# levymsn/CQA-CRCT

Hardware: AMD Instinct MI355X
Metric: QA-pairs/sec training step (whole node) (higher is better)
Workload: dtype bf16; 1 GPU; CRCT fwd+loss+bwd+AdamW, vilbert.json (v_feature_size=2048), batch 80/GPU, 36 visual elems x 2048-d, 20 text tokens, dropout 0.1, L1 regression loss; residual_stream=fp32, global_batch=80, parallelism=dp1, input=resident

## Files before the change

cqa-crct_amd/crct/lib.py:

```python
import ctypes as C
import os

_HERE = os.path.dirname(os.path.abspath(__file__))
LIB_PATH = os.path.join(_HERE, "libcrct_hip.so")

c_i32, c_i64, c_u32, c_u64, c_f32 = C.c_int32, C.c_int64, C.c_uint32, C.c_uint64, C.c_float
ATTN_MAX_LEN = 512
FP8_AMAX_LANES = 64
vp = C.c_void_p


class GemmArgs(C.Structure):
    _fields_ = [("A", vp), ("B", vp), ("C", vp), ("bias", vp), ("preact_out", vp), ("dact_src", vp), ("addend", vp),
                ("lda", c_i64), ("ldb", c_i64), ("ldc", c_i64), ("ld_aux", c_i64), ("ld_add", c_i64),
                ("M", c_i32), ("N", c_i32), ("K", c_i32), ("ta", c_i32), ("tb", c_i32), ("act", c_i32), ("dact", c_i32),
                ("c_is_f32", c_i32), ("accumulate", c_i32), ("tile", c_i32), ("alpha", c_f32), ("drop_thr", c_u32),
                ("drop_scale", c_f32), ("drop_site", c_u32), ("seed", c_u64), ("rowsum_out", vp),
                ("fp8", c_i32), ("scale_a", vp), ("scale_b", vp), ("q_out", vp), ("q_scale", vp), ("q_amax", vp), ("ld_q", c_i64),
                ("site", c_i32), ("split_k", c_i32), ("splitk_ws", vp), ("splitk_cnt", vp), ("addend_f32", c_i32), ("c_cached", c_i32)]


class GemmLnAddend(C.Structure):
    _fields_ = [("mean", vp), ("rstd", vp), ("gamma", vp), ("beta", vp)]

# ... 6 lines not shown
SITE_NAMES = ["none", "t.qkv", "t.out", "t.ffn_up", "t.ffn_down", "v.qkv", "v.out", "v.ffn_up", "v.ffn_down",
              "c.qkv_t", "c.qkv_v", "c.out_t", "c.out_v", "img_emb", "head"]
KIND_NAMES = ["fwd", "dgrad", "wgrad"]
CLASS_NAMES = ["S.w", "S.n", "S.nl", "M.w", "M.n", "M.nl", "L.w", "L.n", "L.nl"]


class HeadArgs(C.Structure):
    _fields_ = [("pooled_t", vp), ("pooled_v", vp), ("fus_h", vp), ("w_cls", vp), ("b_cls", vp), ("w_f6", vp), ("b_f6", vp),
                ("R", vp), ("labels", vp), ("logits", vp), ("reg", vp), ("stats", vp), ("scratch", vp),
                ("d_pooled_t", vp), ("d_pooled_v", vp), ("d_fus_h", vp),
                ("d_w_cls", vp), ("d_b_cls", vp), ("d_w_f6", vp), ("d_b_f6", vp), ("g_nsp_dev", vp), ("g_reg_dev", vp),
                ("g_loss_dev", vp), ("B", c_i32), ("Hb", c_i32), ("fusion_sum", c_i32), ("use_l1", c_i32), ("kind_l1", c_i32),
                ("tol_margin", c_f32), ("nsp_coeff", c_f32), ("reg_coeff", c_f32), ("grad_scale", c_f32),
                ("drop_thr", c_u32), ("drop_scale", c_f32), ("drop_site", c_u32), ("seed", c_u64)]


CE_CLASSES = 65
DATASET_KINDS = {"plotqa": 0, "dvqa": 1, "figure_qa": 2}
REGRESSOR_KINDS = {"plotqa": 0, "none": 1, "ce": 2}


class Variant(C.Structure):
    _fields_ = [("dataset", c_i32), ("regressor", c_i32), ("n_values", c_i32), ("values", c_f32 * CE_CLASSES)]


class HeadVariantArgs(C.Structure):
    _fields_ = [("h", HeadArgs), ("variant", Variant), ("snap", c_i32), ("ce_scratch", vp)]


EVAL_TOTAL, EVAL_BREAKDOWN, EVAL_HISTOGRAM, EVAL_ERRORS, EVAL_TABLE_WORDS = 0, 12, 192, 205, 206


class EvalScoreArgs(C.Structure):
    _fields_ = [("logits", vp), ("reg_out", vp), ("reg_err", vp), ("reg_terr", vp), ("num_ans", vp), ("forced", vp), ("labels", vp),
                ("gt_id", vp), ("needs_reg", vp), ("tolerance", vp), ("cats", vp), ("answers", vp), ("sel_out", vp), ("sel_err", vp),
                ("sel_terr", vp), ("flags", vp), ("prob0", vp), ("tables", vp), ("N", c_i64), ("Q", c_i32), ("mode", c_i32),
                ("with_histogram", c_i32)]


class ModelDims(C.Structure):
    _fields_ = [("vocab", c_i32), ("n_pos", c_i32), ("n_types", c_i32), ("H", c_i32), ("L", c_i32), ("heads", c_i32), ("I", c_i32),
                ("Fv", c_i32), ("Hv", c_i32), ("Lv", c_i32), ("v_heads", c_i32), ("Iv", c_i32), ("Hb", c_i32), ("b_heads", c_i32),
                ("n_color", c_i32), ("n_conn", c_i32), ("v_biatt", c_i32 * 32), ("t_biatt", c_i32 * 32),
                ("fusion_sum", c_i32), ("with_coattention", c_i32),
                ("p_hidden", c_f32), ("p_attn", c_f32), ("p_v_hidden", c_f32), ("p_v_attn", c_f32), ("p_cls", c_f32)]


class Batch(C.Structure):
    _fields_ = [("tokens", vp), ("segments", vp), ("loc", vp), ("text_keymask", vp), ("image_feat", vp), ("image_loc", vp),
                ("image_target", vp), ("image_keymask", vp), ("R", vp), ("labels", vp),
                ("B", c_i32), ("T", c_i32), ("V", c_i32),
                ("sep_indices", vp), ("hist_len", vp), ("image_mask", vp), ("sep_stride", c_i32), ("image_feat_bf16", c_i32)]


class LnFwdArgs(C.Structure):
    _fields_ = [("x", vp), ("gamma", vp), ("beta", vp), ("y", vp), ("mean", vp), ("rstd", vp), ("M", c_i32), ("H", c_i32),
                ("eps", c_f32), ("drop_thr", c_u32), ("drop_scale", c_f32), ("drop_site", c_u32), ("seed", c_u64),
                ("q_out", vp), ("q_scale", vp), ("q_amax", vp), ("x_f32", c_i32), ("y_f32", vp)]


class LnBwdArgs(C.Structure):
    _fields_ = [("dy", vp), ("x", vp), ("mean", vp), ("rstd", vp), ("gamma", vp), ("dx", vp), ("dx_lin", vp), ("partials", vp),
                ("M", c_i32), ("H", c_i32), ("post_thr", c_u32), ("post_scale", c_f32), ("post_site", c_u32),
                ("lin_thr", c_u32), ("lin_scale", c_f32), ("lin_site", c_u32), ("seed", c_u64),
                ("q_out", vp), ("q_scale", vp), ("q_amax", vp), ("x_f32", c_i32)]


class AmpState(C.Structure):
    _fields_ = [("grad_scale", vp), ("found_inf", vp), ("step", vp)]


class AttnQuant(C.Structure):
    _fields_ = [("ctx_q", vp), ("ctx_scale", vp), ("ctx_amax", vp), ("dq_q", vp), ("dk_q", vp), ("dv_q", vp),
                ("dq_scale", vp), ("dq_amax", vp), ("dkv_scale", vp), ("dkv_amax", vp),
                ("row_lse", vp), ("ctx", vp), ("ld_ctx", c_i64)]


class Fp8Shadow(C.Structure):
    _fields_ = [("q", vp), ("seg_slot", vp), ("scale", vp), ("amax", vp), ("qt", vp), ("seg_in", vp), ("seg_t_base", vp), ("seg_t_ld", vp)]


class StepCfg(C.Structure):
    _fields_ = [("training", c_i32), ("use_l1", c_i32), ("kind_l1", c_i32), ("tol_margin", c_f32), ("nsp_coeff", c_f32),
                ("reg_coeff", c_f32), ("grad_scale", c_f32), ("seed", c_u64), ("g_nsp_dev", vp), ("g_reg_dev", vp), ("g_loss_dev", vp),
                ("seg_ready_events", vp), ("seg_done_events", vp),
                ("fp8", c_i32), ("params_fp8", vp), ("fp8_w_scale", vp), ("fp8_act_scale", vp), ("fp8_act_amax", vp),
                ("fp8_bwd", c_i32), ("fp8_wgrad", c_i32), ("params_fp8_t", vp), ("fp8_grad_scale", vp), ("fp8_grad_amax", vp),
                ("seg_enqueued", vp), ("seg_enqueued_user", vp), ("seg_done_mask", vp), ("wgrad_overwrite", c_i32), ("grads_bf16", vp),
                ("residual_fp32", c_i32)]


class InputGrads(C.Structure):
    _fields_ = [("d_image_feat", vp), ("d_image_loc", vp), ("d_areas", vp), ("d_txt_loc", vp), ("d_text_emb", vp)]


class OutputGrads(C.Structure):
    _fields_ = [("d_seq_t", vp), ("d_seq_v", vp)]


class ScoreGrads(C.Structure):
    _fields_ = [("d_logits", vp), ("d_value", vp)]


SEG_ENQUEUED_FN =C.CFUNCTYPE(None, C.c_int, vp)


_u8 = [c_u32, c_f32, c_u32, c_u64]
PROTOTYPES = {
    "crct_last_error": (C.c_char_p, []),
    "crct_abi_version": (C.c_int, []),
    "crct_gemm_bf16": (C.c_int, [C.POINTER(GemmArgs), vp]),
    "crct_gemm_bf16_grouped": (C.c_int, [C.POINTER(GemmArgs), C.c_int, vp]),
    "crct_gemm_bf16_ln_addend": (C.c_int, [C.POINTER(GemmArgs), C.POINTER(GemmLnAddend), vp]),
    "crct_gemm_bf16_grouped_ln_addend": (C.c_int, [C.POINTER(GemmArgs), C.POINTER(GemmLnAddend), C.c_int, vp]),
    "crct_gemm_pick_tile": (C.c_int, [C.c_int, C.c_int]),
    "crct_gemm_group_max_workgroups": (C.c_int, [C.c_int]),
    "crct_gemm_group_target_workgroups": (C.c_int, [C.c_int]),
    "crct_gemm_group_concat": (C.c_int, [C.c_int]),
    "crct_embed_scatter_split": (None, [C.c_int]),
    "crct_gemm_force_generic": (C.c_int, [C.c_int]),
    "crct_prof_enable": (C.c_int, [C.c_int]),
    "crct_prof_reset": (C.c_int, []),
    "crct_prof_read": (C.c_int, [C.c_int, C.POINTER(C.c_long), C.POINTER(C.c_double), C.POINTER(C.c_double)]),
    "crct_prof_read_site": (C.c_int, [C.c_int, C.c_int, C.POINTER(C.c_long), C.POINTER(C.c_double), C.POINTER(C.c_double), C.POINTER(C.c_int)]),
    "crct_prof_stamp_count": (C.c_int, []),
    "crct_prof_stamp_read": (C.c_int, [C.c_int, C.POINTER(vp), C.POINTER(C.c_double), C.POINTER(C.c_double)]),
    "crct_engine_streams": (C.c_int, [vp, C.POINTER(vp)]),
    "crct_launch_log_enable": (C.c_int, [C.c_int]),
    "crct_launch_log_count": (C.c_int, []),
    "crct_launch_log_read": (C.c_int, [C.c_int, C.POINTER(LaunchRec)]),
    "crct_gemm_splitk_ws_elems": (c_i64, [C.c_int, C.c_int, C.c_int]),
    "crct_gemm_splitk_tickets": (C.c_int, [C.c_int, C.c_int]),
    "crct_engine_set_site_policy": (C.c_int, [vp, C.c_int, C.c_int, C.c_int, C.c_int, C.c_int]),
    "crct_layernorm_fwd": (C.c_int, [vp, vp, vp, vp, vp, vp, C.c_int, C.c_int, c_f32] + _u8 + [vp]),
    "crct_layernorm_bwd_blocks": (C.c_int, [C.c_int]),
    "crct_layernorm_bwd": (C.c_int, [vp] * 11 + [C.c_int, C.c_int, C.c_int, c_u32, c_f32, c_u32, c_u32, c_f32, c_u32, c_u64, vp]),
    "crct_layernorm_bwd_rows": (C.c_int, [vp] * 8 + [C.c_int, C.c_int, c_u32, c_f32, c_u32, c_u32, c_f32, c_u32, c_u64, vp]),
    "crct_layernorm_bwd_finalize": (C.c_int, [vp] * 4 + [C.c_int, C.c_int, C.c_int, vp]),
    "crct_colsum_blocks": (C.c_int, [C.c_int]),
    "crct_colsum_bf16": (C.c_int, [vp, c_i64, vp, vp, C.c_int, C.c_int, C.c_int, vp]),
    "crct_build_keymasks": (C.c_int, [vp, vp, C.c_int, vp, vp, vp, C.c_int, C.c_int, C.c_int, vp]),
    "crct_softmax_rows_f32_bf16": (C.c_int, [vp, vp, C.c_int, C.c_int, vp]),
    "crct_softmax_rows_bf16_bf16": (C.c_int, [vp, vp, C.c_int, C.c_int, vp]),
    "crct_layernorm_fwd_q": (C.c_int, [vp, vp, vp, vp, vp, vp, C.c_int, C.c_int, c_f32] + _u8 + [vp, vp, vp, vp]),
    "crct_layernorm_bwd_rows_args": (C.c_int, [C.POINTER(LnBwdArgs), vp]),
    "crct_layernorm_fwd_args": (C.c_int, [C.POINTER(LnFwdArgs), vp]),
    "crct_fp8_transpose_weights": (C.c_int, [vp] * 6 + [C.c_int, c_i64, C.c_int, vp]),
    "crct_fp8_quantize_bf16": (C.c_int, [vp, vp, vp, vp, c_i64, vp]),
    "crct_fp8_update_scales": (C.c_int, [vp, vp, C.c_int, C.c_int, vp, c_f32, vp]),
    "crct_fp8_quantize_weights": (C.c_int, [vp] * 7 + [c_i64, vp, vp, C.c_int, vp]),
    "crct_gemm_group_wgrad_config": (C.c_int, [C.c_int]),
    "crct_engine_set_wgrad_flush": (C.c_int, [vp, C.c_int]),
    "crct_engine_set_ln_addend": (C.c_int, [vp, C.c_int]),
    "crct_engine_set_wgrad_workgroups": (C.c_int, [vp, C.c_int, C.c_int]),
    "crct_gemm_class_config": (C.c_int, [C.c_int, C.c_int]),
    "crct_gemm_fp8_scaled_mfma": (C.c_int, [C.c_int]),
    "crct_ghost_collective": (C.c_int, [vp, c_i64, C.c_int, C.c_int, C.c_double, vp]),
    "crct_cast_f32_bf16": (C.c_int, [vp, vp, c_i64, vp]),
    "crct_cast_bf16_f32": (C.c_int, [vp, vp, c_i64, vp]),
    "crct_cast_runs_f32_bf16": (C.c_int, [vp, vp, vp, vp, vp, vp, c_i64, vp]),
    "crct_cast_runs_bf16_f32": (C.c_int, [vp, vp, vp, vp, vp, vp, c_i64, vp]),
    "crct_attention_fwd": (C.c_int, [vp] * 5 + [C.c_int] * 5 + [c_i64] * 4 + _u8 + [vp]),
    "crct_attention_probs": (C.c_int, [vp] * 4 + [C.c_int] * 5 + [c_i64] * 2 + _u8 + [vp]),
    "crct_attention_bwd": (C.c_int, [vp] * 8 + [C.c_int] * 5 + [c_i64] * 7 + _u8 + [vp]),
    "crct_attention_fwd_q": (C.c_int, [vp] * 5 + [C.c_int] * 5 + [c_i64] * 4 + _u8 + [vp, vp]),
    "crct_attention_bwd_q": (C.c_int, [vp] * 8 + [C.c_int] * 5 + [c_i64] * 7 + _u8 + [vp, vp]),
    "crct_attention_quant_ok": (C.c_int, [C.c_int] * 3),
    "crct_attention_force_valu": (None, [C.c_int]),
    "crct_attention_force_long": (None, [C.c_int]),
    "crct_attention_force_split": (None, [C.c_int]),
    "crct_embed_text_fwd": (C.c_int, [vp] * 14 + [C.c_int] * 4 + [c_f32] + _u8 + [vp]),
    "crct_embed_text_bwd_indexed": (C.c_int, [vp] * 16 + [C.c_int] * 4 + _u8 + [vp, vp, C.c_int, vp, C.c_int, vp]),
    "crct_embed_image_fwd": (C.c_int, [vp] * 12 + [C.c_int] * 2 + [c_f32] + _u8 + [vp]),
    "crct_embed_image_bwd": (C.c_int, [vp] * 15 + [C.c_int] * 2 + _u8 + [vp, vp, C.c_int, vp]),
    "crct_embed_image_var_fwd": (C.c_int, [vp] * 14 + [C.c_int] * 2 + [c_f32] + _u8 + [vp]),
    "crct_embed_image_var_bwd": (C.c_int, [vp] * 16 + [C.c_int] * 2 + _u8 + [vp, vp, C.c_int, vp]),
    "crct_head_loss": (C.c_int, [C.POINTER(HeadArgs), vp]),
    "crct_head_loss_variant": (C.c_int, [C.POINTER(HeadVariantArgs), vp]),
    "crct_head_loss_scores": (C.c_int, [C.POINTER(HeadArgs), C.POINTER(ScoreGrads), vp]),
    "crct_head_loss_variant_scores": (C.c_int, [C.POINTER(HeadVariantArgs), C.POINTER(ScoreGrads), vp]),
    "crct_eval_select": (C.c_int, [vp, vp, vp, vp, vp, vp, C.c_int, c_i64, vp, vp, vp, vp, vp, vp]),
    "crct_eval_score": (C.c_int, [C.POINTER(EvalScoreArgs), vp]),
    "crct_adamw_plan": (c_i64, [vp, C.c_int, vp, vp, c_i64]),
    "crct_adamw_step": (C.c_int, [vp] * 11 + [c_i64, c_f32, c_f32, c_f32, C.c_int, vp, vp, vp, C.c_int, C.c_int, vp, vp]),
    "crct_adamw_advance": (C.c_int, [vp, vp, vp]),
    "crct_grad_sumsq": (C.c_int, [vp] * 6 + [c_i64, vp, C.c_int, C.c_int, vp]),
    "crct_grad_norm_finalize": (C.c_int, [vp, vp, c_i64, C.c_int, C.c_int, c_f32, vp, vp, vp, vp, vp]),
    "crct_scale_runs": (C.c_int, [vp] * 6 + [c_i64, C.c_int, vp]),
    "crct_engine_create": (vp, [C.POINTER(ModelDims), C.c_char_p, vp, vp, C.c_int, C.c_int, C.c_int, C.c_int]),
    "crct_engine_create_variant": (vp, [C.POINTER(ModelDims), C.c_char_p, vp, vp, C.c_int, C.c_int, C.c_int, C.c_int, C.POINTER(Variant)]),
    "crct_engine_set_areas": (C.c_int, [vp, vp]),
    "crct_engine_set_input_grads": (C.c_int, [vp, C.POINTER(InputGrads)]),
    "crct_embed_input_grad": (C.c_int, [vp] * 11 + [C.c_int] * 2 + _u8 + [vp]),
    "crct_softmax_bwd_rows": (C.c_int, [vp, C.c_int, vp, vp, C.c_int, C.c_int, vp]),
    "crct_layernorm_rows_f32": (C.c_int, [vp, C.c_int, vp, vp, vp, vp, vp, C.c_int, C.c_int, vp]),
    "crct_hidden_grad_add": (C.c_int, [vp, vp, c_f32, c_i64, vp]),
    "crct_engine_sequence_outputs": (C.c_int, [vp, vp, vp, C.c_int, C.c_int, C.c_int, vp, vp, vp]),
    "crct_engine_set_output_grads": (C.c_int, [vp, C.POINTER(OutputGrads)]),
    "crct_engine_set_score_grads": (C.c_int, [vp, C.POINTER(ScoreGrads)]),
    "crct_engine_set_trainable": (C.c_int, [vp, vp, C.c_int]),
    "crct_engine_backward_plan": (C.c_int, [vp, vp, C.c_int]),
    "crct_engine_destroy": (None, [vp]),
    "crct_engine_workspace_bytes": (C.c_size_t, [vp]),
    "crct_engine_num_segments": (C.c_int, [vp]),
    "crct_engine_segment_range": (C.c_int, [vp, C.c_int, C.POINTER(c_i64), C.POINTER(c_i64)]),
    "crct_engine_forward": (C.c_int, [vp, vp, vp, C.POINTER(Batch), C.POINTER(StepCfg), vp, vp, vp, vp, vp]),
    "crct_engine_backward": (C.c_int, [vp, vp, vp, C.POINTER(Batch), C.POINTER(StepCfg), vp, vp, vp, vp, vp, C.c_int, vp]),
    "crct_engine_set_streams": (C.c_int, [vp, C.c_int, C.c_int]),
    "crct_engine_aux_stream": (vp, [vp, vp, C.POINTER(C.c_int)]),
    "crct_event_create": (vp, []),
    "crct_event_destroy": (None, [vp]),
    "crct_event_record": (C.c_int, [vp, vp]),
    "crct_stream_wait_event": (C.c_int, [vp, vp]),
    "crct_event_synchronize": (C.c_int, [vp]),
    "crct_event_query": (C.c_int, [vp]),
    "crct_engine_wgrad_owned": (C.c_int, [vp, vp, vp, C.c_int]),
    "crct_engine_fp8_sites": (C.c_int, [vp]),
    "crct_engine_fp8_grad_sites": (C.c_int, [vp]),
    "crct_engine_fp8_weights": (C.c_int, [vp, vp, vp, C.c_int]),
    "crct_zero_runs": (C.c_int, [vp, vp, vp, vp, vp, c_i64, vp]),
    "crct_engine_attention_probs": (c_i64, [vp, vp, vp, vp, C.c_int, C.c_int, C.c_int, vp, c_i64, vp]),
    "crct_engine_tap": (c_i64, [vp, vp, C.c_char_p, C.c_int, C.c_int, C.c_int, vp, c_i64, vp]),
}

_lib = None


def load():
    global _lib
    if _lib is not None:
        return _lib
    if not os.path.exists(LIB_PATH):
        raise RuntimeError("libcrct_hip.so is missing (%s): run `python -c 'import __graft_entry__ as g; g.build()'` "
                           "-- there is no CPU fallback for the CRCT step" % LIB_PATH)
    import torch
    lib = C.CDLL(LIB_PATH)
    for name, (res, args) in PROTOTYPES.items():
        fn = getattr(lib, name)
        fn.restype = res
        fn.argtypes = args
    _lib = lib
    return lib


def check(rc, what=""):
    if rc != 0:
        raise RuntimeError("libcrct_hip %s failed (%d): %s" % (what, rc, load().crct_last_error().decode()))


def drop_threshold(p):
    t = float(p) * 4294967296.0
    if t <= 0.0:
        return 0
    return min(int(t), 4294967295)


def ptr(t):
    return None if t is None else t.data_ptr()


def current_stream():
    import torch
    return torch.cuda.current_stream().cuda_stream
```

cqa-crct_amd/csrc/crct_internal.h:

```cpp
#pragma once
#include <hip/hip_runtime.h>
#include <hip/hip_ext.h>
#include "../../include/crct_hip.h"

void crct_set_error(const char* fmt, ...);
#define CRCT_CHECK_HIP(expr)                                                          \
  do {                                                                                \
    hipError_t _e = (expr);                                                           \
    if (_e != hipSuccess) {                                                           \
      crct_set_error("%s:%d: %s -> %s", __FILE__, __LINE__, #expr, hipGetErrorString(_e)); \
      return 1;                                                                       \
    }                                                                                 \
  } while (0)
#define CRCT_REQUIRE(cond, ...)                 \
  do {                                          \
    if (!(cond)) {                              \
      crct_set_error(__VA_ARGS__);              \
      return 2;                                 \
    }                                           \
  } while (0)

bool crct_gemm_config_built(int id);
int crct_gemm_fp8_wgrad_step_config(int asked);
hipError_t crct_gemm_launch(const CrctGemmArgs& g, const CrctGemmLnAddend* ln, hipStream_t s);
struct CrctGemmGroup {
  const CrctGemmArgs* gs;
  const CrctGemmLnAddend* ln;
  int n;
  const uint8_t* keep;
  int target_wgs;
};
hipError_t crct_gemm_launch_grouped(const CrctGemmGroup& grp, hipStream_t s);
int crct_streams_place(hipStream_t main, hipStream_t out[4], int* n_classes);

#define CRCT_LN_BWD_MAX_BLOCKS 256

bool crct_stamp_begin(hipStream_t s, hipEvent_t* start, hipEvent_t* stop);
void crct_stamp_adopt(hipStream_t s, hipEvent_t start, hipEvent_t stop);
void crct_stamp_enable(int on);
void crct_stamp_reset(void);
#ifdef CRCT_GEMM_LAB
bool crct_lab_skip(const void* kern, hipStream_t s);
#endif
hipError_t crct_lds_limit_raise(const void* kern, size_t bytes);
class CrctDeviceScope {
 public:
  CrctDeviceScope();
  ~CrctDeviceScope();
  CrctDeviceScope(const CrctDeviceScope&) = delete;
  CrctDeviceScope& operator=(const CrctDeviceScope&) = delete;
 private:
  int outer_;
};
template <class K>
inline hipError_t crct_lds_limit(K kern, size_t bytes) {
  return bytes <= 64 * 1024 ? hipSuccess : crct_lds_limit_raise(reinterpret_cast<const void*>(kern), bytes);
}
template <class K, class... A>
inline void crct_launch(K kern, dim3 grid, dim3 block, size_t lds, hipStream_t s, A... a) {
#ifdef CRCT_GEMM_LAB
  if (crct_lab_skip((const void*)kern, s)) return;
#endif
  hipEvent_t e0, e1;
  if (crct_stamp_begin(s, &e0, &e1)) hipExtLaunchKernelGGL(kern, grid, block, (uint32_t)lds, s, e0, e1, 0u, a...);
  else hipLaunchKernelGGL(kern, grid, block, lds, s, a...);
}
```

cqa-crct_amd/csrc/engine.cpp:

```cpp
#include <math.h>
#include <stdarg.h>
#include <stdio.h>
#include <stdlib.h>
#include <string.h>

#include <algorithm>
#include <string>
#include <unordered_map>
#include <unordered_set>
#include <functional>
#include <vector>

#include "crct_internal.h"

typedef unsigned short bf16_t;
enum { ACT_NONE = 0, ACT_GELU = 1, ACT_RELU = 2, ACT_LEAKY = 3, ACT_TANH = 4 };

static thread_local char g_err[1024] = "";
void crct_set_error(const char* fmt, ...) {
  va_list ap;
  va_start(ap, fmt);
  vsnprintf(g_err, sizeof(g_err), fmt, ap);
  va_end(ap);
}
// ... 12 lines not shown
  CRCT_REQUIRE(!a.ta || a.M % 8 == 0, "%s: transposed A needs M %% 8 == 0 (M=%d)%s", who, a.M, of);
  CRCT_REQUIRE(!a.tb || a.N % 8 == 0, "%s: transposed B needs N %% 8 == 0 (N=%d)%s", who, a.N, of);
  CRCT_REQUIRE(a.tile < 0 || crct_gemm_config_built(a.tile), "%s: configuration %d is not built%s", who, a.tile, of);
  CRCT_REQUIRE(!(a.c_cached && a.accumulate), "%s: c_cached with accumulate is not supported (c_cached is a plain fp32 store)%s", who, of);
  CRCT_REQUIRE(!ln || (a.addend && a.addend_f32 && ln->mean && ln->rstd && ln->gamma && ln->beta),
               "%s: a LayerNorm addend needs the fp32 addend it normalises (addend, addend_f32) and mean, rstd, gamma, beta%s", who, of);
  return 0;
}

extern "C" int crct_gemm_bf16_ln_addend(const CrctGemmArgs* a, const CrctGemmLnAddend* ln, crct_stream_t stream) {
  CRCT_REQUIRE(a != nullptr, "gemm: null args");
  if (int r = gemm_check(*a, ln, "gemm", -1)) return r;
  CRCT_CHECK_HIP(crct_gemm_launch(*a, ln, (hipStream_t)stream));
  return 0;
}
extern "C" int crct_gemm_bf16(const CrctGemmArgs* a, crct_stream_t stream) { return crct_gemm_bf16_ln_addend(a, nullptr, stream); }

static int gemm_grouped_checked(const CrctGemmGroup& grp, crct_stream_t stream) {
  CRCT_REQUIRE(grp.gs != nullptr && grp.n >= 1, "gemm_grouped: bad arguments");
  for (int i = 0; i < grp.n; ++i)
    if (int r = gemm_check(grp.gs[i], grp.ln && grp.ln[i].mean ? &grp.ln[i] : nullptr, "gemm_grouped", i)) return r;
  CRCT_CHECK_HIP(crct_gemm_launch_grouped(grp, (hipStream_t)stream));
  return 0;
}
extern "C" int crct_gemm_bf16_grouped_ln_addend(const CrctGemmArgs* a, const CrctGemmLnAddend* ln, int n, crct_stream_t stream) {
  return gemm_grouped_checked(CrctGemmGroup{a, ln, n, nullptr, -1}, stream);
}
extern "C" int crct_gemm_bf16_grouped(const CrctGemmArgs* a, int n, crct_stream_t stream) { return crct_gemm_bf16_grouped_ln_addend(a, nullptr, n, stream); }

namespace {

inline size_t align_up(size_t v, size_t a) { return (v + a - 1) / a * a; }
inline uint32_t thr_of(float p) {
  double t = (double)p * 4294967296.0;
  if (t <= 0.0) return 0u;
  if (t >= 4294967295.0) return 4294967295u;
  return (uint32_t)t;
}

struct Arena {
  size_t top = 0;
  size_t take(size_t bytes) { size_t o = top; top = align_up(top + bytes, 256); return o; }
};

struct Drop { uint32_t thr = 0; float scale = 1.f; uint32_t site = 0; };

struct LinearP { int64_t w = -1, b = -1; int in = 0, out = 0; int site = 0; int parts = 1; };
struct LnP { int64_t g = -1, b = -1; };
struct FfnP { LinearP up, down; LnP ln; };
struct ProjP { LinearP dense; LnP ln; };
struct SelfLayerP { LinearP qkv; ProjP proj; FfnP ffn; int H, heads; float p_attn, p_hid; uint32_t site; };
struct ConnLayerP { LinearP qkv1, qkv2; ProjP proj_v, proj_t; FfnP ffn_v, ffn_t; uint32_t site; };

constexpr size_t NONE = (size_t)-1;
struct Act { size_t x = 0, q = NONE; int site = -1; size_t x32 = NONE; size_t s = NONE, mean = NONE, rstd = NONE; LnP ln; };
struct GradQ { size_t q = NONE; int site = -1; };
struct FfnA {
  size_t u, h, s, y, y32, mean, rstd, hq, yq; int site_h, site_y; int g_dl, g_du;
  Act out(const LnP& ln) const { return {y, yq, site_y, y32, s, mean, rstd, ln}; }
};
struct ProjA {
  size_t s, a, a32, mean, rstd, aq; int site_a; int g_dl;
  Act out(const LnP& ln) const { return {a, aq, site_a, a32, s, mean, rstd, ln}; }
};
struct SelfLayerA { size_t qkv, ctx, ctxq, lse; int site_ctx, g_dqkv; ProjA proj; FfnA ffn; };
struct ConnLayerA { size_t qkv1, qkv2, ctx1, ctx2, ctx1q, ctx2q, lse1, lse2; int site_ctx1, site_ctx2, g_dqkv1, g_dqkv2; ProjA proj_v, proj_t; FfnA ffn_v, ffn_t; };
struct StreamScratch { size_t dy[2], dres_a, dlin_a, dres_b, dlin_b, gc, du, dctx, dqkv, part_a, part_b, dlq_a, dlq_b, duq, dqkvq; };

struct Step { char kind; int idx; };
struct StepIn { Act t, v; };
struct Tap { std::string name; size_t off; char stream; int width = 0; };
struct SegPlan { bool runs = true, dx_t = true, dx_v = true; int dropped = 0; };

}

struct crct_engine {
  CrctModelDims d;
  std::unordered_map<std::string, int64_t> off, size;
  int maxB, maxT, maxV;
  std::vector<Step> sched;
  std::vector<SelfLayerP> tl, vl;
  std::vector<ConnLayerP> cl;
  std::vector<SelfLayerA> tla, vla;
  std::vector<ConnLayerA> cla;
  struct { int64_t word, pos, type, wloc, bloc; LnP ln; } et;
  struct { LinearP img; int64_t color, wloc, bloc; LnP ln; LinearP areas; } ev;
  CrctVariant var = {CRCT_DATASET_PLOTQA, CRCT_REGRESSOR_PLOTQA, 0, {}};
  bool feat = true;
  const float* areas = nullptr;
  CrctInputGrads ig = {nullptr, nullptr, nullptr, nullptr, nullptr};
  size_t ws_ig = 0;
  bool emb_own_t = true, emb_own_v = true;
  CrctOutputGrads og = {nullptr, nullptr};
  int fwd_r32 = -1;
  CrctScoreGrads sg = {nullptr, nullptr};
  bool ig_text() const { return ig.d_txt_loc || ig.d_text_emb; }
  bool ig_vis() const { return ig.d_image_feat || ig.d_image_loc || ig.d_areas; }
  size_t ws_base() const { return ln_addend ? ws_core : ws_two_output; }
  void ws_update() { ws_bytes = ws_base() + (ig.d_image_feat ? ws_ig : 0); }
  struct { size_t sum, y, mean, rstd, yq; int site; } eta;
  struct { size_t soft, lin, sum, y, mean, rstd, yq; int site; } eva;
  LinearP t_pool, v_pool, cls, tp[4], vp[4], fu[4];
  struct { size_t pooled_t, pooled_v, t[3], v[3], cat, f[3], scratch, ce, d_pt, d_pv, g[10]; } ha;
  StreamScratch st, sv;
  StreamScratch st2, sv2;
  size_t partials[2], colsum_part[4];
  size_t embed_rows[2], embed_idx[2];
  size_t km_t = 0, km_v = 0;
  struct SitePolicy { int cfg = -1, split_k = 0; };
  SitePolicy policy[CRCT_SITE_COUNT][3][2];
  size_t sk_ws[2] = {0, 0}, sk_cnt[2] = {0, 0};
  size_t sk_ws_elems[2] = {0, 0};
  int sk_tickets = 0;
  std::unordered_map<int64_t, int> wq_slot;
  int32_t* word_index = nullptr;
  std::vector<std::pair<int64_t, int64_t>> wq_list;
  int n_sites = 0;
  int n_gsites = 0;
  size_t ws_bytes = 0;
  bool use_vis_stream = true, use_wgrad_stream = true, streams_forced = false;
  int wgrad_target = 96, wgrad_target_rows = 3000;
  int ln_addend = 1;
  size_t ws_core = 0, ws_two_output = 0;
  int wgrad_flush = 1;
  bool one_wgrad_stream = false;
  int first_conn = -1;
  hipStream_t side[3] = {nullptr, nullptr, nullptr};
  hipStream_t aux = nullptr;
  hipStream_t placed_for = nullptr;
  bool placed = false;
  int queue_classes = 0;
  std::vector<hipEvent_t> evpool;
  size_t evnext = 0;
  std::vector<std::pair<int64_t, int64_t>> seg_range;
  std::unordered_map<int64_t, int64_t> wgrad_owned;
  std::unordered_map<int64_t, int> wgrad_pass;
  void wgrad_pass_begin() { wgrad_pass.clear(); }
  std::vector<int64_t> param_off;
  std::unordered_set<int64_t> nograd;
  std::vector<SegPlan> plan;
  bool grad_at(int64_t o) const { return nograd.empty() || !nograd.count(o); }
  bool w_grad(const LinearP& l) const {
    for (int k = 0; k < l.parts; ++k) if (grad_at(l.w + k * ((int64_t)l.in * l.out / l.parts))) return true;
    return false;
  }
  bool b_grad(const LinearP& l) const {
    for (int k = 0; k < l.parts; ++k) if (grad_at(l.b + k * (l.out / l.parts))) return true;
    return false;
  }
  bool drops_wgrad(const LinearP& l, bool with_bias) const { return !nograd.empty() && !w_grad(l) && !(with_bias && b_grad(l)); }
  std::vector<Tap> taps;
  std::vector<StepIn> in;
  int cur_t = 0, cur_v = 0;
  bool bad = false;
  int64_t P(const std::string& k) {
    auto it = off.find(k);
    if (it == off.end()) { crct_set_error("engine: parameter '%s' missing from the layout", k.c_str()); bad = true; return 0; }
    return it->second;
  }
};

namespace {

LinearP linear_p(crct_engine* e, const std::string& name, int in, int out, int site = CRCT_SITE_HEAD) {
  LinearP l;
  l.w = e->P(name + ".weight"); l.b = e->P(name + ".bias"); l.in = in; l.out = out; l.site = site;
  return l;
}
LnP ln_p(crct_engine* e, const std::string& name) {
  LnP l; l.g = e->P(name + ".weight"); l.b = e->P(name + ".bias"); return l;
}
LinearP fused3(crct_engine* e, const std::string& a, const std::string& b, const std::string& c, int in, int out, int site) {
  LinearP l = linear_p(e, a, in, 3 * out, site);
  l.parts = 3;
  const int64_t wsz = (int64_t)in * out;
  if (e->P(b + ".weight") != l.w + wsz || e->P(c + ".weight") != l.w + 2 * wsz || e->P(b + ".bias") != l.b + out ||
      e->P(c + ".bias") != l.b + 2 * out) {
    crct_set_error("engine: %s / %s / %s must be adjacent in the flat layout (fused QKV)", a.c_str(), b.c_str(), c.c_str());
    e->bad = true;
  }
  return l;
}

static_assert(CRCT_SITE_T_OUT == CRCT_SITE_T_QKV + 1 && CRCT_SITE_T_FFN_UP == CRCT_SITE_T_QKV + 2 && CRCT_SITE_T_FFN_DN == CRCT_SITE_T_QKV + 3 &&
              CRCT_SITE_V_OUT == CRCT_SITE_V_QKV + 1 && CRCT_SITE_V_FFN_UP == CRCT_SITE_V_QKV + 2 && CRCT_SITE_V_FFN_DN == CRCT_SITE_V_QKV + 3,
              "the GEMM sites of a self-attention layer are consecutive");
SelfLayerP self_layer_p(crct_engine* e, const std::string& p, int H, int I, int heads, float p_attn, float p_hid, uint32_t drop_site, int gemm_site) {
  SelfLayerP l;
  l.H = H; l.heads = heads; l.p_attn = p_attn; l.p_hid = p_hid; l.site = drop_site;
  l.qkv = fused3(e, p + "attention.self.query", p + "attention.self.key", p + "attention.self.value", H, H, gemm_site);
  l.proj.dense = linear_p(e, p + "attention.output.dense", H, H, gemm_site + 1);
  l.proj.ln = ln_p(e, p + "attention.output.LayerNorm");
  l.ffn.up = linear_p(e, p + "intermediate.dense", H, I, gemm_site + 2);
  l.ffn.down = linear_p(e, p + "output.dense", I, H, gemm_site + 3);
  l.ffn.ln = ln_p(e, p + "output.LayerNorm");
  return l;
}
template <class F> void each_encoder_linear(const crct_engine* e, F f) {
  for (const std::vector<SelfLayerP>* stack : {&e->tl, &e->vl})
    for (const SelfLayerP& l : *stack) { f(l.qkv); f(l.ffn.up); f(l.ffn.down); f(l.proj.dense); }
  for (const ConnLayerP& l : e->cl) {
    f(l.qkv1); f(l.qkv2); f(l.ffn_v.up); f(l.ffn_v.down); f(l.ffn_t.up); f(l.ffn_t.down); f(l.proj_v.dense); f(l.proj_t.dense);
  }
}

FfnA ffn_a(Arena& ar, size_t M, int H, int I, int& sites, int& gsites) {
  FfnA a;
  a.g_dl = gsites++; a.g_du = gsites++;
  a.u = ar.take(M * I * 2); a.h = ar.take(M * I * 2); a.s = ar.take(M * H * 4); a.y = ar.take(M * H * 2); a.y32 = NONE;
  a.mean = ar.take(M * 4); a.rstd = ar.take(M * 4);
  a.hq = ar.take(M * I); a.yq = ar.take(M * H);
  a.site_h = sites++; a.site_y = sites++;
  return a;
}
ProjA proj_a(Arena& ar, size_t M, int H, int& sites, int& gsites) {
  ProjA a;
  a.g_dl = gsites++;
  a.s = ar.take(M * H * 4); a.a = ar.take(M * H * 2); a.a32 = NONE; a.mean = ar.take(M * 4); a.rstd = ar.take(M * 4);
  a.aq = ar.take(M * H);
  a.site_a = sites++;
  return a;
}
SelfLayerA self_layer_a(Arena& ar, size_t M, int H, int I, int heads, int& sites, int& gsites) {
  SelfLayerA a;
  a.qkv = ar.take(M * 3 * H * 2); a.ctx = ar.take(M * H * 2); a.ctxq = ar.take(M * H); a.lse = ar.take(M * heads * 4);
  a.site_ctx = sites++; a.g_dqkv = gsites++;
  a.proj = proj_a(ar, M, H, sites, gsites); a.ffn = ffn_a(ar, M, H, I, sites, gsites);
  return a;
}
StreamScratch scratch_a(Arena& ar, size_t M, int H, int I, int Hb) {
  StreamScratch s;
  const int Hm = H > Hb ? H : Hb;
  s.dy[0] = ar.take(M * H * 2); s.dy[1] = ar.take(M * H * 2);
  s.dres_a = ar.take(M * H * 2); s.dlin_a = ar.take(M * H * 2); s.dres_b = ar.take(M * H * 2); s.dlin_b = ar.take(M * H * 2);
  s.gc = ar.take(M * H * 2); s.du = ar.take(M * (size_t)I * 2); s.dctx = ar.take(M * (size_t)Hm * 2);
  s.dqkv = ar.take(M * (size_t)3 * Hm * 2);
  s.part_a = ar.take((size_t)3 * 4 * CRCT_LN_BWD_MAX_BLOCKS * H * 4);
  s.part_b = ar.take((size_t)3 * 4 * CRCT_LN_BWD_MAX_BLOCKS * H * 4);
  s.dlq_a = ar.take(M * H); s.dlq_b = ar.take(M * H); s.duq = ar.take(M * (size_t)I);
  s.dqkvq = ar.take(M * (size_t)3 * Hm);
  return s;
}

hipEvent_t ev_new(crct_engine* e) {
  if (e->evnext == e->evpool.size()) {
    hipEvent_t ev = nullptr;
    const unsigned flags = hipEventDisableTiming | hipEventDisableSystemFence;
    if (hipEventCreateWithFlags(&ev, flags) != hipSuccess) return nullptr;
    e->evpool.push_back(ev);
  }
  return e->evpool[e->evnext++];
}
int order_streams(crct_engine* e, hipStream_t from, hipStream_t to) {
  if (from == to) return 0;
  hipEvent_t ev = ev_new(e);
  if (!ev || hipEventRecord(ev, from) != hipSuccess || hipStreamWaitEvent(to, ev, 0) != hipSuccess) {
    crct_set_error("engine: event ordering between internal streams failed");
    return 1;
  }
  return 0;
}

struct WgQ8 { GradQ dy; Act x; };
struct Q8 { uint8_t* q = nullptr; const float* scale = nullptr; float* amax = nullptr; };

struct Run {
  crct_engine* e;
  const float* p32; const bf16_t* p16; float* g32; char* ws; hipStream_t s;
  const CrctBatch* b; const CrctStepCfg* c;
  hipStream_t sw;
  size_t partials, colsum_part, colsum_part_w;
  int which = 0;
  int phase = 1;
  int rc = 0;
  bool sw_dirty = false;
  const StreamScratch* sets[2] = {nullptr, nullptr};
  hipEvent_t set_free[2] = {nullptr, nullptr};
  int parity = 0;
  const StreamScratch& layer_begin() {
    if (!rc && sw != s && set_free[parity]) {
      if (hipStreamWaitEvent(s, set_free[parity], 0) != hipSuccess) { crct_set_error("engine: stream wait failed"); rc = 1; }
      set_free[parity] = nullptr;
    }
    return *sets[parity];
  }
  void layer_end() {
    flush_wgrads();
    if (!rc && sw != s && sw_dirty) {
      hipEvent_t ev = ev_new(e);
      if (!ev || hipEventRecord(ev, sw) != hipSuccess) { crct_set_error("engine: event record failed"); rc = 1; }
      set_free[parity] = ev;
    }
    parity ^= 1;
  }
  std::vector<CrctGemmArgs> pending;
  bool defer_wgrad = true;
  struct FinJob { const float* part; float* dg; float* db; float* dlb; int M, H; };
  std::vector<FinJob> pending_fin;
  int tick = 0, ordered_tick = -1;
  void wgrad_after_main() {
    if (rc || sw == s) return;
    sw_dirty = true;
    if (ordered_tick == tick) return;
    fail(order_streams(e, s, sw));
    ordered_tick = tick;
  }
  void main_after_wgrad() {
    flush_wgrads();
    if (!rc && sw != s && sw_dirty) { fail(order_streams(e, sw, s)); sw_dirty = false; }
  }

  template <class T> T* W(size_t o) const { return reinterpret_cast<T*>(ws + o); }
  bf16_t* A(size_t o) const { return W<bf16_t>(o); }
  float* F(size_t o) const { return W<float>(o); }
  const float* P(int64_t o) const { return p32 + o; }
  const bf16_t* PB(int64_t o) const { return p16 + o; }
  float* G(int64_t o) const { return g32 + o; }
  Drop drop(float p, uint32_t site) const {
    Drop d; d.site = site;
    if (c->training && p > 0.f) { d.thr = thr_of(p); d.scale = 1.0f / (1.0f - p); }
    return d;
  }
  void fail(int r) { if (!rc && r) rc = r; }

  struct Opt {
    void* preact = nullptr; const void* dact_src = nullptr; int dact = 0; int act = 0;
    const void* addend = nullptr; int64_t ld_aux = 0, ld_add = 0; Drop drop; bool f32 = false; bool acc = false;
    bool add_f32 = false, c_cached = false;
    CrctGemmLnAddend ln = {nullptr, nullptr, nullptr, nullptr};
  };
  void cross_sync(Run& V) {
    if (!rc) fail(order_streams(e, V.s, s));
    if (!V.rc) V.fail(order_streams(e, s, V.s));
  }
  int f8() const { return (c->fp8 && c->params_fp8 && c->fp8_w_scale && c->fp8_act_scale && c->fp8_act_amax) ? c->fp8 : 0; }
  bool f8_lin(const LinearP& l) const { return f8() && e->wq_slot.count(l.w) != 0; }
  int f8b() const { return (c->fp8 && c->fp8_bwd && c->params_fp8_t && c->fp8_w_scale && c->fp8_grad_scale && c->fp8_grad_amax) ? c->fp8_bwd : 0; }
  bool f8b_lin(const LinearP& l) const { return f8b() && e->wq_slot.count(l.w) != 0; }
  const float* ascale(int site) const { return c->fp8_act_scale + site; }
  float* aamax(int site) const { return c->fp8_act_amax + (int64_t)site * CRCT_FP8_AMAX_LANES; }
  const float* gscale(int g) const { return c->fp8_grad_scale + g; }
  float* gamax(int g) const { return c->fp8_grad_amax + (int64_t)g * CRCT_FP8_AMAX_LANES; }
  Q8 q8(const Act& a) const { return a.site < 0 ? Q8() : Q8{W<uint8_t>(a.q), ascale(a.site), aamax(a.site)}; }
  Q8 q8(const GradQ& g) const { return g.site < 0 ? Q8() : Q8{W<uint8_t>(g.q), gscale(g.site), gamax(g.site)}; }

  enum Dir { FWD = CRCT_KIND_FWD, DGRAD = CRCT_KIND_DGRAD, WGRAD = CRCT_KIND_WGRAD };
  CrctGemmArgs gemm_args(Dir dir, const LinearP& l, int M, const void* a, int64_t lda, const void* x, int64_t ldx, void* C, int64_t ldc,
                         const Opt& o, const Q8& a8 = Q8(), const Q8& x8 = Q8(), const Q8& out = Q8()) const {
    const bool q = a8.q != nullptr;
    CrctGemmArgs g;
    memset(&g, 0, sizeof(g));
    g.A = q ? a8.q : a; g.C = C; g.ldc = ldc;
    if (dir == WGRAD) {
      g.B = q ? x8.q : x; g.M = l.out; g.N = l.in; g.K = M; g.ta = 1; g.tb = 1; g.lda = lda; g.ldb = ldx;
    } else {
      const bool fwd = dir == FWD;
      g.M = M; g.N = fwd ? l.out : l.in; g.K = fwd ? l.in : l.out;
      g.lda = q ? g.K : lda; g.ldb = q ? g.K : l.in; g.tb = !fwd && !q;
      if (q) g.B = reinterpret_cast<const uint8_t*>(fwd ? c->params_fp8 : c->params_fp8_t) + l.w;
      else g.B = PB(l.w);
      if (fwd) g.bias = P(l.b);
    }
    g.preact_out = o.preact; g.dact_src = o.dact_src; g.addend = o.addend; g.ld_aux = o.ld_aux; g.ld_add = o.ld_add;
    g.act = o.act; g.dact = o.dact; g.c_is_f32 = o.f32; g.accumulate = o.acc; g.addend_f32 = o.add_f32; g.c_cached = o.c_cached;
    g.alpha = 1.0f; g.drop_thr = o.drop.thr; g.drop_scale = o.drop.scale; g.drop_site = o.drop.site; g.seed = c->seed; g.site = l.site;
    if (q) {
      g.fp8 = dir == FWD ? 1 : (dir == DGRAD ? 1 | 2 | 8 : 1 | 2);
      g.scale_a = a8.scale; g.scale_b = dir == WGRAD ? x8.scale : c->fp8_w_scale + e->wq_slot.at(l.w);
    }
    if (out.q) {
      g.q_out = out.q; g.q_scale = out.scale; g.q_amax = out.amax; g.ld_q = g.N;
      if (dir == DGRAD) g.fp8 |= 4;
    }
    g.tile = -1;
    if (l.site > 0 && l.site < CRCT_SITE_COUNT) {
      const crct_engine::SitePolicy& pol = e->policy[l.site][dir][phase];
      if (pol.cfg >= 0) g.tile = pol.cfg;
      if (dir != WGRAD && !q && pol.split_k > 1 && crct_gemm_splitk_ws_elems(g.M, g.N, pol.split_k) <= (int64_t)e->sk_ws_elems[which] &&
          crct_gemm_splitk_tickets(g.M, g.N) <= e->sk_tickets) {
        g.split_k = pol.split_k; g.splitk_ws = F(e->sk_ws[which]); g.splitk_cnt = W<uint32_t>(e->sk_cnt[which]);
      }
    }
    return g;
  }
  void launch(const CrctGemmArgs& g, const CrctGemmLnAddend* ln = nullptr) {
    ++tick;
    fail(crct_gemm_bf16_ln_addend(&g, ln && ln->mean ? ln : nullptr, s));
  }

  Act lin_fwd(const Act& x, int64_t ldx, const LinearP& l, int M, Act y, int64_t ldy, const Opt& o) {
    const bool q = f8_lin(l) && x.site >= 0;
    if (!q) y.site = -1;
    if (rc) return y;
    launch(gemm_args(FWD, l, M, A(x.x), ldx, nullptr, 0, A(y.x), ldy, o, q && f8() == 1 ? q8(x) : Q8(), Q8(), q8(y)), &o.ln);
    return y;
  }
  GradQ lin_dgrad(const void* dy, int64_t lddy, const LinearP& l, int M, void* dx, int64_t lddx, const Opt& o, const GradQ& dyq = GradQ(),
                  GradQ out = GradQ()) {
    const bool q = f8b_lin(l) && dyq.site >= 0;
    if (!q) out.site = -1;
    if (rc) return out;
    launch(gemm_args(DGRAD, l, M, dy, lddy, nullptr, 0, dx, lddx, o, q && f8b() == 1 ? q8(dyq) : Q8(), Q8(), q8(out)));
    return out;
  }
  void lin_wgrad(const void* dy, int64_t lddy, const void* x, int64_t ldx, const LinearP& l, int M, bool with_bias = false, const WgQ8& w8 = WgQ8()) {
    if (rc) return;
    const bool keep = !e->drops_wgrad(l, with_bias);
    if (!keep && !defer_wgrad) return;
    const bool f8w = f8b() == 1 && c->fp8_wgrad && defer_wgrad && f8_lin(l) && w8.dy.site >= 0 && w8.x.site >= 0 &&
                     l.in % 16 == 0 && l.out % 16 == 0 && lddy % 16 == 0 && ldx % 16 == 0;
    const bool fold = !f8w && with_bias && M % 64 == 0 && l.in % 8 == 0 && l.out % 8 == 0 && lddy % 8 == 0 && ldx % 8 == 0;
    if (with_bias && !fold && keep) bias_grad(dy, lddy, l, M);
    if (rc) return;
    Opt o; o.f32 = true; o.acc = true;
    CrctGemmArgs g = gemm_args(WGRAD, l, M, dy, lddy, x, ldx, G(l.w), l.in, o, f8w ? q8(w8.dy) : Q8(), f8w ? q8(w8.x) : Q8());
    if (keep && c->wgrad_overwrite && e->wgrad_owned.count(l.w)) {
      if (++e->wgrad_pass[l.w] > 1) { rc = 1; crct_set_error("engine_backward: weight gradient at offset %lld is produced twice in one pass but is listed as owned", (long long)l.w); return; }
      g.accumulate = 0;
      if (c->grads_bf16) {
        if (l.in % 8 != 0 || l.w % 8 != 0) { rc = 1; crct_set_error("engine_backward: owned weight gradient at offset %lld (in = %d) cannot be written as bf16 rows", (long long)l.w, l.in); return; }
        g.C = reinterpret_cast<bf16_t*>(c->grads_bf16) + l.w; g.c_is_f32 = 0;
      }
    }
    if (fold) g.rowsum_out = G(l.b);
    if (f8w) {
      if (!keep) return;
      g.tile = crct_gemm_fp8_wgrad_step_config(g.tile);
      pending_f8.push_back(g);
      return;
    }
    if (!defer_wgrad) { launch(g); return; }
    pending.push_back(g);
    pending_keep.push_back(keep);
    if (pending.size() == 8) flush_wgrads();
  }
  std::vector<CrctGemmArgs> pending_f8;
  std::vector<uint8_t> pending_keep;
  void flush_wgrads() {
    if (!pending.empty() && std::find(pending_keep.begin(), pending_keep.end(), 1) == pending_keep.end()) { pending.clear(); pending_keep.clear(); }
    if (rc || (pending.empty() && pending_f8.empty() && pending_fin.empty() && pending_bias.empty())) return;
    if (sw == s) ++tick;
    wgrad_after_main();
    for (const BiasJob& j : pending_bias)
      if (!rc) fail(crct_colsum_bf16(j.dy, j.lddy, j.db, F(sw != s ? colsum_part_w : colsum_part), j.M, j.N, 1, sw));
    pending_bias.clear();
    for (const FinJob& f : pending_fin)
      if (!rc) fail(crct_layernorm_bwd_finalize(f.part, f.dg, f.db, f.dlb, f.M, f.H, 1, sw));
    pending_fin.clear();
    const int target = (sw != s && !pending.empty() && pending[0].K <= e->wgrad_target_rows && !e->one_wgrad_stream) ? e->wgrad_target : 0;
    for (size_t i = 0; i < pending.size() && !rc; i += 8) {
      const int ng = (int)std::min<size_t>(8, pending.size() - i);
      const uint8_t* kp = pending_keep.data() + i;
      fail(gemm_grouped_checked(CrctGemmGroup{pending.data() + i, nullptr, ng, std::find(kp, kp + ng, 0) == kp + ng ? nullptr : kp, target}, sw));
    }
    pending.clear();
    pending_keep.clear();
    for (size_t i = 0; i < pending_f8.size() && !rc; i += 8)
      fail(crct_gemm_bf16_grouped(pending_f8.data() + i, (int)std::min<size_t>(8, pending_f8.size() - i), sw));
    pending_f8.clear();
  }
  struct BiasJob { const void* dy; int64_t lddy; float* db; int M, N; };
  std::vector<BiasJob> pending_bias;
  void bias_grad(const void* dy, int64_t lddy, const LinearP& l, int M) {
    if (rc) return;
    if (defer_wgrad) { pending_bias.push_back(BiasJob{dy, lddy, G(l.b), M, l.out}); return; }
    wgrad_after_main();
    if (rc) return;
    fail(crct_colsum_bf16(dy, lddy, G(l.b), F(sw != s ? colsum_part_w : colsum_part), M, l.out, 1, sw));
  }
  void ln_fwd(size_t x, const LnP& ln, const Act& y, size_t mean, size_t rstd, int M, int H) {
    if (rc) return;
    ++tick;
    CrctLnFwdArgs a = {A(x), P(ln.g), P(ln.b), A(y.x), F(mean), F(rstd), M, H, 1e-12f, 0, 1.f, 0, c->seed, nullptr, nullptr, nullptr, 0, nullptr};
    if (r32()) { a.x_f32 = 1; if (!e->ln_addend) a.y_f32 = F(y.x32); }
    if (f8()) { a.q_out = W<uint8_t>(y.q); a.q_scale = ascale(y.site); a.q_amax = aamax(y.site); }
    fail(crct_layernorm_fwd_args(&a, s));
  }
  bool r32() const { return c->residual_fp32 != 0; }
  void residual(Opt& o, const Act& x, int64_t ld) const {
    o.ld_add = ld;
    if (r32()) {
      o.f32 = true; o.c_cached = true;
      if (e->ln_addend && x.s != NONE) {
        o.addend = F(x.s); o.add_f32 = true;
        o.ln = CrctGemmLnAddend{F(x.mean), F(x.rstd), P(x.ln.g), P(x.ln.b)};
        return;
      }
      if (!e->ln_addend && x.x32 != NONE) { o.addend = F(x.x32); o.add_f32 = true; return; }
    }
    o.addend = A(x.x);
  }
  size_t ln_bwd(size_t dy, size_t x, size_t mean, size_t rstd, const LnP& ln, const LinearP& lin, size_t dres, size_t dlin,
                size_t part, int M, int H, const Drop& dr, GradQ& dlq) {
    if (!f8b_lin(lin)) dlq.site = -1;
    if (rc) return dres;
    ++tick;
    CrctLnBwdArgs a = {A(dy), A(x), F(mean), F(rstd), P(ln.g), A(dres), dr.thr ? A(dlin) : nullptr, F(part), M, H,
                       0, 1.f, 0, dr.thr, dr.scale, dr.site, c->seed, nullptr, nullptr, nullptr, r32() ? 1 : 0};
    if (dlq.site >= 0) { const Q8 d8 = q8(dlq); a.q_out = d8.q; a.q_scale = d8.scale; a.q_amax = d8.amax; }
    fail(crct_layernorm_bwd_rows_args(&a, s));
    if (defer_wgrad) pending_fin.push_back(FinJob{F(part), G(ln.g), G(ln.b), G(lin.b), M, H});
    else { wgrad_after_main(); if (!rc) fail(crct_layernorm_bwd_finalize(F(part), G(ln.g), G(ln.b), G(lin.b), M, H, 1, sw)); }
    return dr.thr ? dlin : dres;
  }
  void attn_fwd(const bf16_t* q, int64_t ldq, const bf16_t* k, const bf16_t* v, int64_t ldk, const uint8_t* km, const Act& ctx,
                int64_t ldo, int B, int heads, int Tq, int Tk, int d, const Drop& dr, size_t lse = NONE) {
    if (rc) return;
    ++tick;
    const uint64_t seed = c->seed;
    CrctAttnQuant qz;
    memset(&qz, 0, sizeof(qz));
    if (lse != NONE) qz.row_lse = F(lse);
    if (ctx.site >= 0) { const Q8 c8 = q8(ctx); qz.ctx_q = c8.q; qz.ctx_scale = c8.scale; qz.ctx_amax = c8.amax; }
    fail(crct_attention_fwd_q(q, k, v, km, A(ctx.x), B, heads, Tq, Tk, d, ldq, ldk, ldk, ldo, dr.thr, dr.scale, dr.site, seed, &qz, s));
  }
  void attn_bwd(const bf16_t* q, int64_t ldq, const bf16_t* k, const bf16_t* v, int64_t ldk, const uint8_t* km,
                const bf16_t* dctx, int64_t ldo, bf16_t* dq, int64_t lddq, bf16_t* dk, bf16_t* dv, int64_t lddk, int B,
                int heads, int Tq, int Tk, int d, const Drop& dr, uint8_t* dqq = nullptr, int g_dq = -1, uint8_t* dkq = nullptr,
                uint8_t* dvq = nullptr, int g_dkv = -1, size_t lse = NONE, const bf16_t* ctx = nullptr, int64_t ldc = 0) {
    if (rc) return;
    ++tick;
    const uint64_t seed = c->seed;
    CrctAttnQuant qz;
    memset(&qz, 0, sizeof(qz));
    if (lse != NONE && ctx) { qz.row_lse = F(lse); qz.ctx = ctx; qz.ld_ctx = ldc; }
    if (dqq && g_dq >= 0) { qz.dq_q = dqq; qz.dq_scale = gscale(g_dq); qz.dq_amax = gamax(g_dq); }
    if (dkq && dvq && g_dkv >= 0) { qz.dk_q = dkq; qz.dv_q = dvq; qz.dkv_scale = gscale(g_dkv); qz.dkv_amax = gamax(g_dkv); }
    fail(crct_attention_bwd_q(q, k, v, km, dctx, dq, dk, dv, B, heads, Tq, Tk, d, ldq, ldk, ldk, ldo, lddq, lddk, lddk, dr.thr, dr.scale,
                              dr.site, seed, &qz, s));
  }
  static bool attn_q_ok(int Tq, int Tk, int d) { return crct_attention_quant_ok(Tq, Tk, d) != 0; }
  Act ctx_act(size_t ctx, size_t ctxq, int site, const LinearP& dense, bool aq) const { return {ctx, ctxq, aq && f8_lin(dense) ? site : -1}; }
  Act ffn_h(const FfnP& p, const FfnA& a) const { return {a.h, a.hq, f8_lin(p.up) && f8_lin(p.down) ? a.site_h : -1}; }

  void proj_fwd(const ProjP& p, const ProjA& a, const Act& ctx, const Act& x, int M, const Drop& dr) {
    Opt o; o.drop = dr; residual(o, x, p.dense.out);
    lin_fwd(ctx, p.dense.in, p.dense, M, Act{a.s}, p.dense.out, o);
    ln_fwd(a.s, p.ln, a.out(p.ln), a.mean, a.rstd, M, p.dense.out);
  }
  void proj_bwd(const ProjP& p, const ProjA& a, const Act& ctx, size_t g, const StreamScratch& sc, int M, const Drop& dr) {
    GradQ dlq{sc.dlq_b, a.g_dl};
    const size_t dl = ln_bwd(g, a.s, a.mean, a.rstd, p.ln, p.dense, sc.dres_b, sc.dlin_b, sc.part_b, M, p.dense.out, dr, dlq);
    lin_wgrad(A(dl), p.dense.out, A(ctx.x), p.dense.in, p.dense, M, false, WgQ8{dlq, ctx});
    lin_dgrad(A(dl), p.dense.out, p.dense, M, A(sc.dctx), p.dense.in, Opt(), dlq);
    if (e->wgrad_flush & 2) flush_wgrads();
  }
  void ffn_fwd(const FfnP& p, const FfnA& a, const Act& x, int M, const Drop& dr) {
    Opt o; o.preact = A(a.u); o.ld_aux = p.up.out; o.act = ACT_GELU;
    const Act h = lin_fwd(x, p.up.in, p.up, M, ffn_h(p, a), p.up.out, o);
    Opt o2; o2.drop = dr; residual(o2, x, p.down.out);
    lin_fwd(h, p.down.in, p.down, M, Act{a.s}, p.down.out, o2);
    ln_fwd(a.s, p.ln, a.out(p.ln), a.mean, a.rstd, M, p.down.out);
  }
  void ffn_bwd(const FfnP& p, const FfnA& a, const Act& x, size_t g, size_t gx, const StreamScratch& sc, int M, const Drop& dr) {
    const int H = p.down.out, I = p.up.out;
    GradQ dlq{sc.dlq_a, a.g_dl};
    const size_t dl = ln_bwd(g, a.s, a.mean, a.rstd, p.ln, p.down, sc.dres_a, sc.dlin_a, sc.part_a, M, H, dr, dlq);
    lin_wgrad(A(dl), H, A(a.h), I, p.down, M, false, WgQ8{dlq, ffn_h(p, a)});
    Opt o; o.dact_src = A(a.u); o.dact = ACT_GELU; o.ld_aux = I;
    const GradQ duq = lin_dgrad(A(dl), H, p.down, M, A(sc.du), I, o, dlq, GradQ{sc.duq, f8b_lin(p.up) ? a.g_du : -1});
    lin_wgrad(A(sc.du), I, A(x.x), H, p.up, M, true, WgQ8{duq, x});
    Opt o2; o2.addend = A(sc.dres_a); o2.ld_add = H;
    lin_dgrad(A(sc.du), I, p.up, M, A(gx), H, o2, duq);
    if (e->wgrad_flush & 1) flush_wgrads();
  }

  void self_fwd(const SelfLayerP& p, const SelfLayerA& a, const Act& x, const uint8_t* km, int B, int T) {
    const int M = B * T, H = p.H, d = H / p.heads;
    lin_fwd(x, p.qkv.in, p.qkv, M, Act{a.qkv}, 3 * H, Opt());
    const Act ctx = ctx_act(a.ctx, a.ctxq, a.site_ctx, p.proj.dense, attn_q_ok(T, T, d));
    attn_fwd(A(a.qkv), 3 * H, A(a.qkv) + H, A(a.qkv) + 2 * H, 3 * H, km, ctx, H, B, p.heads, T, T, d, drop(p.p_attn, p.site), a.lse);
    proj_fwd(p.proj, a.proj, ctx, x, M, drop(p.p_hid, p.site + 1));
    ffn_fwd(p.ffn, a.ffn, a.proj.out(p.proj.ln), M, drop(p.p_hid, p.site + 2));
  }
  void self_bwd(const SelfLayerP& p, const SelfLayerA& a, const Act& x, size_t g, size_t gx, const uint8_t* km, int B, int T, bool dx = true) {
    const int M = B * T, H = p.H, d = H / p.heads;
    const StreamScratch& sc = layer_begin();
    ffn_bwd(p.ffn, a.ffn, a.proj.out(p.proj.ln), g, sc.gc, sc, M, drop(p.p_hid, p.site + 2));
    const bool aq = attn_q_ok(T, T, d);
    const bool gq = aq && f8b_lin(p.qkv) && f8_lin(p.qkv);
    const GradQ dqkvq{sc.dqkvq, gq ? a.g_dqkv : -1};
    proj_bwd(p.proj, a.proj, ctx_act(a.ctx, a.ctxq, a.site_ctx, p.proj.dense, aq), sc.gc, sc, M, drop(p.p_hid, p.site + 1));
    uint8_t* dq8 = gq ? W<uint8_t>(sc.dqkvq) : nullptr;
    attn_bwd(A(a.qkv), 3 * H, A(a.qkv) + H, A(a.qkv) + 2 * H, 3 * H, km, A(sc.dctx), H, A(sc.dqkv), 3 * H, A(sc.dqkv) + H,
             A(sc.dqkv) + 2 * H, 3 * H, B, p.heads, T, T, d, drop(p.p_attn, p.site), dq8, a.g_dqkv, gq ? dq8 + H : nullptr,
             gq ? dq8 + 2 * H : nullptr, a.g_dqkv, a.lse, A(a.ctx), H);
    lin_wgrad(A(sc.dqkv), 3 * H, A(x.x), H, p.qkv, M, true, WgQ8{dqkvq, x});
    Opt o; o.addend = A(sc.dres_b); o.ld_add = H;
    if (dx) lin_dgrad(A(sc.dqkv), 3 * H, p.qkv, M, A(gx), H, o, dqkvq);
    layer_end();
  }

  void conn_fwd(Run& V, const ConnLayerP& p, const ConnLayerA& a, const StepIn& x) {
    const CrctModelDims& D = e->d;
    const int B = b->B, Mv = B * b->V, Mt = B * b->T, Hb = D.Hb, d = Hb / D.b_heads;
    V.lin_fwd(x.v, p.qkv1.in, p.qkv1, Mv, Act{a.qkv1}, 3 * Hb, Opt());
    lin_fwd(x.t, p.qkv2.in, p.qkv2, Mt, Act{a.qkv2}, 3 * Hb, Opt());
    cross_sync(V);
    const bool aq = attn_q_ok(b->T, b->V, d) && attn_q_ok(b->V, b->T, d);
    const Act ctx1 = ctx_act(a.ctx1, a.ctx1q, a.site_ctx1, p.proj_t.dense, aq), ctx2 = V.ctx_act(a.ctx2, a.ctx2q, a.site_ctx2, p.proj_v.dense, aq);
    attn_fwd(A(a.qkv2), 3 * Hb, A(a.qkv1) + Hb, A(a.qkv1) + 2 * Hb, 3 * Hb, b->image_keymask, ctx1, Hb, B, D.b_heads,
             b->T, b->V, d, drop(D.p_v_attn, p.site), a.lse1);
    V.attn_fwd(A(a.qkv1), 3 * Hb, A(a.qkv2) + Hb, A(a.qkv2) + 2 * Hb, 3 * Hb, b->text_keymask, ctx2, Hb, B, D.b_heads,
               b->V, b->T, d, drop(D.p_attn, p.site + 1), a.lse2);
    V.proj_fwd(p.proj_v, a.proj_v, ctx2, x.v, Mv, drop(D.p_v_hidden, p.site + 2));
    proj_fwd(p.proj_t, a.proj_t, ctx1, x.t, Mt, drop(D.p_hidden, p.site + 3));
    V.ffn_fwd(p.ffn_v, a.ffn_v, a.proj_v.out(p.proj_v.ln), Mv, drop(D.p_v_hidden, p.site + 4));
    ffn_fwd(p.ffn_t, a.ffn_t, a.proj_t.out(p.proj_t.ln), Mt, drop(D.p_hidden, p.site + 5));
  }
  void conn_bwd(Run& V, const ConnLayerP& p, const ConnLayerA& a, const StepIn& x, size_t gv, size_t gt, size_t gxv, size_t gxt,
                bool dxv = true, bool dxt = true) {
    const CrctModelDims& D = e->d;
    hipEvent_t free_v = V.set_free[V.parity], free_t = set_free[parity];
    const StreamScratch& sv = V.layer_begin(); const StreamScratch& st = layer_begin();
    const int B = b->B, Mv = B * b->V, Mt = B * b->T, Hb = D.Hb, d = Hb / D.b_heads;
    V.ffn_bwd(p.ffn_v, a.ffn_v, a.proj_v.out(p.proj_v.ln), gv, sv.gc, sv, Mv, drop(D.p_v_hidden, p.site + 4));
    ffn_bwd(p.ffn_t, a.ffn_t, a.proj_t.out(p.proj_t.ln), gt, st.gc, st, Mt, drop(D.p_hidden, p.site + 5));
    const bool aq = attn_q_ok(b->T, b->V, d) && attn_q_ok(b->V, b->T, d);
    const bool gq = aq && f8b_lin(p.qkv1) && f8b_lin(p.qkv2) && f8_lin(p.qkv1) && f8_lin(p.qkv2);
    const GradQ dqkvq_v{sv.dqkvq, gq ? a.g_dqkv1 : -1}, dqkvq_t{st.dqkvq, gq ? a.g_dqkv2 : -1};
    V.proj_bwd(p.proj_v, a.proj_v, V.ctx_act(a.ctx2, a.ctx2q, a.site_ctx2, p.proj_v.dense, aq), sv.gc, sv, Mv, drop(D.p_v_hidden, p.site + 2));
    proj_bwd(p.proj_t, a.proj_t, ctx_act(a.ctx1, a.ctx1q, a.site_ctx1, p.proj_t.dense, aq), st.gc, st, Mt, drop(D.p_hidden, p.site + 3));
    if (sw != s && V.sw != V.s) {
      if (free_v && !rc && hipStreamWaitEvent(s, free_v, 0) != hipSuccess) { crct_set_error("engine: stream wait failed"); rc = 1; }
      if (free_t && !V.rc && hipStreamWaitEvent(V.s, free_t, 0) != hipSuccess) { crct_set_error("engine: stream wait failed"); V.rc = 1; }
    } else cross_sync(V);
    uint8_t* tq8 = gq ? W<uint8_t>(st.dqkvq) : nullptr;
    uint8_t* vq8 = gq ? W<uint8_t>(sv.dqkvq) : nullptr;
    attn_bwd(A(a.qkv2), 3 * Hb, A(a.qkv1) + Hb, A(a.qkv1) + 2 * Hb, 3 * Hb, b->image_keymask, A(st.dctx), Hb, A(st.dqkv),
             3 * Hb, A(sv.dqkv) + Hb, A(sv.dqkv) + 2 * Hb, 3 * Hb, B, D.b_heads, b->T, b->V, d, drop(D.p_v_attn, p.site),
             tq8, a.g_dqkv2, gq ? vq8 + Hb : nullptr, gq ? vq8 + 2 * Hb : nullptr, a.g_dqkv1, a.lse1, A(a.ctx1), Hb);
    V.attn_bwd(A(a.qkv1), 3 * Hb, A(a.qkv2) + Hb, A(a.qkv2) + 2 * Hb, 3 * Hb, b->text_keymask, A(sv.dctx), Hb, A(sv.dqkv),
               3 * Hb, A(st.dqkv) + Hb, A(st.dqkv) + 2 * Hb, 3 * Hb, B, D.b_heads, b->V, b->T, d, drop(D.p_attn, p.site + 1),
               vq8, a.g_dqkv1, gq ? tq8 + Hb : nullptr, gq ? tq8 + 2 * Hb : nullptr, a.g_dqkv2, a.lse2, A(a.ctx2), Hb);
    cross_sync(V);
    V.lin_wgrad(A(sv.dqkv), 3 * Hb, A(x.v.x), D.Hv, p.qkv1, Mv, true, WgQ8{dqkvq_v, x.v});
    Opt ov; ov.addend = A(sv.dres_b); ov.ld_add = D.Hv;
    if (dxv) V.lin_dgrad(A(sv.dqkv), 3 * Hb, p.qkv1, Mv, A(gxv), D.Hv, ov, dqkvq_v);
    lin_wgrad(A(st.dqkv), 3 * Hb, A(x.t.x), D.H, p.qkv2, Mt, true, WgQ8{dqkvq_t, x.t});
    Opt ot; ot.addend = A(st.dres_b); ot.ld_add = D.H;
    if (dxt) lin_dgrad(A(st.dqkv), 3 * Hb, p.qkv2, Mt, A(gxt), D.H, ot, dqkvq_t);
    V.layer_end();
    layer_end();
  }

  void embed_text_fwd() {
    const CrctModelDims& D = e->d;
    const Drop dt = drop(D.p_hidden, 1);
    if (!rc) fail(crct_embed_text_fwd(b->tokens, b->segments, b->loc, P(e->et.word), P(e->et.pos), P(e->et.type), P(e->et.wloc),
                                      P(e->et.bloc), P(e->et.ln.g), P(e->et.ln.b), A(e->eta.sum), A(e->eta.y), F(e->eta.mean),
                                      F(e->eta.rstd), b->B, b->T, D.H, D.n_pos, 1e-12f, dt.thr, dt.scale, dt.site, c->seed, s));
    if (!rc && f8()) fail(crct_fp8_quantize_bf16(A(e->eta.y), W<uint8_t>(e->eta.yq), ascale(e->eta.site), aamax(e->eta.site),
                                                 (int64_t)b->B * b->T * D.H, s));
  }
  void embed_image_fwd() {
    const CrctModelDims& D = e->d;
    const int Mv = b->B * b->V;
    const Drop dv = drop(D.p_hidden, 2);
    if (!e->feat) {
      const bool ar = e->areas != nullptr;
      if (!rc) fail(crct_embed_image_var_fwd(b->image_loc, b->image_target, e->areas, P(e->ev.wloc), P(e->ev.bloc), P(e->ev.color),
                                             ar ? P(e->ev.areas.w) : nullptr, ar ? P(e->ev.areas.b) : nullptr, P(e->ev.ln.g), P(e->ev.ln.b),
                                             A(e->eva.sum), A(e->eva.y), F(e->eva.mean), F(e->eva.rstd), Mv, D.Hv, 1e-12f, dv.thr, dv.scale,
                                             dv.site, c->seed, s));
      return;
    }
    if (!rc) fail(b->image_feat_bf16 ? crct_softmax_rows_bf16_bf16(b->image_feat, A(e->eva.soft), Mv, D.Fv, s)
                                     : crct_softmax_rows_f32_bf16((const float*)b->image_feat, A(e->eva.soft), Mv, D.Fv, s));
    lin_fwd(Act{e->eva.soft}, D.Fv, e->ev.img, Mv, Act{e->eva.lin}, D.Hv, Opt());
    if (!rc) fail(crct_embed_image_fwd(A(e->eva.lin), b->image_loc, b->image_target, P(e->ev.wloc), P(e->ev.bloc), P(e->ev.color),
                                       P(e->ev.ln.g), P(e->ev.ln.b), A(e->eva.sum), A(e->eva.y), F(e->eva.mean), F(e->eva.rstd),
                                       Mv, D.Hv, 1e-12f, dv.thr, dv.scale, dv.site, c->seed, s));
    if (!rc && f8()) fail(crct_fp8_quantize_bf16(A(e->eva.y), W<uint8_t>(e->eva.yq), ascale(e->eva.site), aamax(e->eva.site),
                                                 (int64_t)Mv * D.Hv, s));
  }
  void embed_text_bwd(size_t gt) {
    const CrctModelDims& D = e->d;
    const Drop dt = drop(D.p_hidden, 1);
    layer_begin();
    ++tick;
    if (!rc) fail(crct_embed_text_bwd_indexed(A(gt), A(e->eta.sum), F(e->eta.mean), F(e->eta.rstd), b->tokens, b->segments, b->loc,
                                              P(e->et.ln.g), e->grad_at(e->et.word) ? G(e->et.word) : nullptr, G(e->et.pos), G(e->et.type), G(e->et.wloc), G(e->et.bloc),
                                              G(e->et.ln.g), G(e->et.ln.b), F(partials), b->B, b->T, D.H, D.n_pos, dt.thr, dt.scale,
                                              dt.site, c->seed, F(e->embed_rows[0]), W<int32_t>(e->embed_idx[0]), D.n_types, e->word_index,
                                              D.vocab, s));
  }
  void embed_image_bwd(size_t gv) {
    const CrctModelDims& D = e->d;
    const int Mv = b->B * b->V;
    const Drop dv = drop(D.p_hidden, 2);
    const StreamScratch& sc = layer_begin();
    ++tick;
    if (!e->feat) {
      const bool ar = e->areas != nullptr;
      if (!rc) fail(crct_embed_image_var_bwd(A(gv), A(e->eva.sum), F(e->eva.mean), F(e->eva.rstd), b->image_loc, b->image_target, e->areas,
                                             P(e->ev.ln.g), G(e->ev.color), G(e->ev.wloc), G(e->ev.bloc), ar ? G(e->ev.areas.w) : nullptr,
                                             ar ? G(e->ev.areas.b) : nullptr, G(e->ev.ln.g), G(e->ev.ln.b), F(partials), Mv, D.Hv, dv.thr,
                                             dv.scale, dv.site, c->seed, F(e->embed_rows[1]), W<int32_t>(e->embed_idx[1]), D.n_color, s));
      return;
    }
    if (!rc) fail(crct_embed_image_bwd(A(gv), A(e->eva.sum), F(e->eva.mean), F(e->eva.rstd), b->image_loc, b->image_target,
                                       P(e->ev.ln.g), A(sc.gc), G(e->ev.color), G(e->ev.wloc), G(e->ev.bloc), G(e->ev.img.b),
                                       G(e->ev.ln.g), G(e->ev.ln.b), F(partials), Mv, D.Hv, dv.thr, dv.scale, dv.site,
                                       c->seed, F(e->embed_rows[1]), W<int32_t>(e->embed_idx[1]), D.n_color, s));
    lin_wgrad(A(sc.gc), D.Hv, A(e->eva.soft), D.Fv, e->ev.img, Mv);
  }
  void embed_text_input_grads(size_t gt) {
    const CrctModelDims& D = e->d;
    const Drop dt = drop(D.p_hidden, 1);
    ++tick;
    if (!rc) fail(crct_embed_input_grad(A(gt), A(e->eta.sum), F(e->eta.mean), F(e->eta.rstd), P(e->et.ln.g), b->loc, P(e->et.wloc), nullptr,
                                        e->ig.d_txt_loc, nullptr, e->ig.d_text_emb, b->B * b->T, D.H, dt.thr, dt.scale, dt.site, c->seed, s));
  }
  void embed_image_input_grads(size_t gv) {
    const CrctModelDims& D = e->d;
    const int Mv = b->B * b->V;
    const Drop dv = drop(D.p_hidden, 2);
    if (e->ig.d_image_loc || e->ig.d_areas) {
      ++tick;
      if (!rc) fail(crct_embed_input_grad(A(gv), A(e->eva.sum), F(e->eva.mean), F(e->eva.rstd), P(e->ev.ln.g), nullptr, P(e->ev.wloc),
                                          e->ig.d_areas ? P(e->ev.areas.w) : nullptr, e->ig.d_image_loc, e->ig.d_areas, nullptr, Mv, D.Hv,
                                          dv.thr, dv.scale, dv.site, c->seed, s));
    }
    if (!e->ig.d_image_feat) return;
    const StreamScratch& sc = *sets[parity];
    float* g = F(e->ws_base());
    Opt o; o.f32 = true;
    lin_dgrad(A(sc.gc), D.Hv, e->ev.img, Mv, g, D.Fv, o);
    ++tick;
    if (!rc) fail(crct_softmax_bwd_rows(b->image_feat, b->image_feat_bf16, g, e->ig.d_image_feat, Mv, D.Fv, s));
  }

  void pipe_fwd(const LinearP* l, size_t x0, int64_t ldx0, const size_t* acts, size_t out_last, int64_t ld_last, int B) {
    Opt o; o.act = ACT_LEAKY;
    lin_fwd(Act{x0}, ldx0, l[0], B, Act{acts[0]}, l[0].out, o);
    lin_fwd(Act{acts[0]}, l[0].out, l[1], B, Act{acts[1]}, l[1].out, o);
    lin_fwd(Act{acts[1]}, l[1].out, l[2], B, Act{acts[2]}, l[2].out, o);
    lin_fwd(Act{acts[2]}, l[2].out, l[3], B, Act{out_last}, ld_last, Opt());
  }
  void pipe_bwd(const LinearP* l, const bf16_t* x0, int64_t ldx0, const size_t* acts, const bf16_t* du3, int64_t ld3,
                bf16_t* dx0, int64_t lddx0, bool acc0, int B, const size_t* gb) {
    bias_grad(du3, ld3, l[3], B);
    lin_wgrad(du3, ld3, A(acts[2]), l[2].out, l[3], B);
    Opt o; o.dact = ACT_LEAKY; o.dact_src = A(acts[2]); o.ld_aux = l[2].out;
    lin_dgrad(du3, ld3, l[3], B, A(gb[0]), l[2].out, o);
    bias_grad(A(gb[0]), l[2].out, l[2], B);
    lin_wgrad(A(gb[0]), l[2].out, A(acts[1]), l[1].out, l[2], B);
    o.dact_src = A(acts[1]); o.ld_aux = l[1].out;
    lin_dgrad(A(gb[0]), l[2].out, l[2], B, A(gb[1]), l[1].out, o);
    bias_grad(A(gb[1]), l[1].out, l[1], B);
    lin_wgrad(A(gb[1]), l[1].out, A(acts[0]), l[0].out, l[1], B);
    o.dact_src = A(acts[0]); o.ld_aux = l[0].out;
    lin_dgrad(A(gb[1]), l[1].out, l[1], B, A(gb[2]), l[0].out, o);
    bias_grad(A(gb[2]), l[0].out, l[0], B);
    lin_wgrad(A(gb[2]), l[0].out, x0, ldx0, l[0], B);
    if (dx0) { Opt od; od.acc = acc0; lin_dgrad(A(gb[2]), l[0].out, l[0], B, dx0, lddx0, od); }
  }

  void heads_branch_fwd(bool visual, size_t seq) {
    const CrctModelDims& D = e->d;
    const int B = b->B;
    const int64_t ld = visual ? (int64_t)b->V * D.Hv : (int64_t)b->T * D.H;
    Opt orelu; orelu.act = ACT_RELU;
    if (visual) {
      lin_fwd(Act{seq}, ld, e->v_pool, B, Act{e->ha.pooled_v}, D.Hb, orelu);
      if (has_regressor())
        pipe_fwd(e->vp, seq, ld, e->ha.v, e->ha.cat, 512, B);
    } else {
      lin_fwd(Act{seq}, ld, e->t_pool, B, Act{e->ha.pooled_t}, D.Hb, orelu);
      if (has_regressor()) pipe_fwd(e->tp, seq, ld, e->ha.t, e->ha.cat + 256 * sizeof(bf16_t), 512, B);
    }
  }
  bool has_regressor() const { return e->var.regressor != CRCT_REGRESSOR_NONE; }
  bool plain_head() const { return e->var.dataset == CRCT_DATASET_PLOTQA && e->var.regressor == CRCT_REGRESSOR_PLOTQA; }
  int head_loss(const CrctHeadArgs& h, const CrctScoreGrads* scores = nullptr) {
    if (plain_head()) return crct_head_loss_scores(&h, scores, s);
    CrctHeadVariantArgs va;
    memset(&va, 0, sizeof(va));
    va.h = h; va.variant = e->var;
    va.snap = e->var.dataset == CRCT_DATASET_DVQA && e->var.regressor == CRCT_REGRESSOR_PLOTQA && !c->training;
    va.ce_scratch = e->var.regressor == CRCT_REGRESSOR_CE ? F(e->ha.ce) : nullptr;
    return crct_head_loss_variant_scores(&va, scores, s);
  }
  void fill_head_args(CrctHeadArgs& h, float* logits, float* reg, float* stats, bool with_grad) {
    const CrctModelDims& D = e->d;
    memset(&h, 0, sizeof(h));
    h.pooled_t = A(e->ha.pooled_t); h.pooled_v = A(e->ha.pooled_v); h.fus_h = A(e->ha.f[2]);
    h.w_cls = P(e->cls.w); h.b_cls = P(e->cls.b);
    if (has_regressor()) { h.w_f6 = P(e->fu[3].w); h.b_f6 = P(e->fu[3].b); }
    h.R = b->R; h.labels = b->labels; h.logits = logits; h.reg = reg; h.stats = stats; h.scratch = F(e->ha.scratch);
    if (with_grad && g32) {
      h.d_pooled_t = A(e->ha.d_pt); h.d_pooled_v = A(e->ha.d_pv); h.d_fus_h = A(e->ha.g[0]);
      h.d_w_cls = G(e->cls.w); h.d_b_cls = G(e->cls.b);
      if (has_regressor()) { h.d_w_f6 = G(e->fu[3].w); h.d_b_f6 = G(e->fu[3].b); }
    }
    h.g_nsp_dev = c->g_nsp_dev; h.g_reg_dev = c->g_reg_dev; h.g_loss_dev = c->g_loss_dev;
    h.B = b->B; h.Hb = D.Hb; h.fusion_sum = D.fusion_sum; h.use_l1 = c->use_l1; h.kind_l1 = c->kind_l1;
    h.tol_margin = c->tol_margin; h.nsp_coeff = c->nsp_coeff; h.reg_coeff = c->reg_coeff; h.grad_scale = c->grad_scale;
    const Drop dc = drop(D.p_cls, 3);
    h.drop_thr = dc.thr; h.drop_scale = dc.scale; h.drop_site = dc.site; h.seed = c->seed;
  }
  void heads_tail_fwd(float* logits, float* reg, float* stats) {
    const int B = b->B;
    Opt o; o.act = ACT_LEAKY;
    if (has_regressor()) {
      lin_fwd(Act{e->ha.cat}, 512, e->fu[0], B, Act{e->ha.f[0]}, 512, o);
      lin_fwd(Act{e->ha.f[0]}, 512, e->fu[1], B, Act{e->ha.f[1]}, 256, o);
      lin_fwd(Act{e->ha.f[1]}, 256, e->fu[2], B, Act{e->ha.f[2]}, 256, o);
    }
    if (rc) return;
    CrctHeadArgs h;
    fill_head_args(h, logits, reg, stats, false);
    fail(head_loss(h));
  }
  void heads_bwd(Run& V, size_t seq_t, size_t seq_v, size_t gt, size_t gv, float* logits, float* reg, float* stats) {
    const CrctModelDims& D = e->d;
    const int B = b->B;
    const int64_t ldt = (int64_t)b->T * D.H, ldv = (int64_t)b->V * D.Hv;
    const size_t* g = e->ha.g;
    {
      CrctHeadArgs h;
      fill_head_args(h, logits, reg, stats, true);
      if (!rc) fail(head_loss(h, e->sg.d_logits || e->sg.d_value ? &e->sg : nullptr));
    }
    if (rc) return;
    if (!V.rc) V.fail(order_streams(e, s, V.s));
    if (hipMemsetAsync(A(gt), 0, (size_t)B * b->T * D.H * 2, s) != hipSuccess ||
        hipMemsetAsync(V.A(gv), 0, (size_t)B * b->V * D.Hv * 2, V.s) != hipSuccess) { crct_set_error("engine: memset failed"); rc = 1; return; }
    ++tick; ++V.tick;
    bias_grad(A(e->ha.d_pt), D.Hb, e->t_pool, B);
    lin_wgrad(A(e->ha.d_pt), D.Hb, A(seq_t), ldt, e->t_pool, B);
    lin_dgrad(A(e->ha.d_pt), D.Hb, e->t_pool, B, A(gt), ldt, Opt());
    V.bias_grad(V.A(e->ha.d_pv), D.Hb, e->v_pool, B);
    V.lin_wgrad(V.A(e->ha.d_pv), D.Hb, V.A(seq_v), ldv, e->v_pool, B);
    V.lin_dgrad(V.A(e->ha.d_pv), D.Hb, e->v_pool, B, V.A(gv), ldv, Opt());
    if (!has_regressor()) {
      output_grads(V, gt, gv);
      flush_wgrads();
      V.flush_wgrads();
      return;
    }
    bias_grad(A(g[0]), 256, e->fu[2], B);
    lin_wgrad(A(g[0]), 256, A(e->ha.f[1]), 256, e->fu[2], B);
    Opt o; o.dact = ACT_LEAKY; o.dact_src = A(e->ha.f[1]); o.ld_aux = 256;
    lin_dgrad(A(g[0]), 256, e->fu[2], B, A(g[1]), 256, o);
    bias_grad(A(g[1]), 256, e->fu[1], B);
    lin_wgrad(A(g[1]), 256, A(e->ha.f[0]), 512, e->fu[1], B);
    o.dact_src = A(e->ha.f[0]); o.ld_aux = 512;
    lin_dgrad(A(g[1]), 256, e->fu[1], B, A(g[2]), 512, o);
    bias_grad(A(g[2]), 512, e->fu[0], B);
    lin_wgrad(A(g[2]), 512, A(e->ha.cat), 512, e->fu[0], B);
    lin_dgrad(A(g[2]), 512, e->fu[0], B, A(g[3]), 512, Opt());
    if (!rc && !V.rc) V.fail(order_streams(e, s, V.s));
    V.pipe_bwd(e->vp, V.A(seq_v), ldv, e->ha.v, V.A(g[3]), 512, V.A(gv), ldv, true, B, g + 4);
    pipe_bwd(e->tp, A(seq_t), ldt, e->ha.t, A(g[3]) + 256, 512, A(gt), ldt, true, B, g + 7);
    output_grads(V, gt, gv);
    flush_wgrads();
    V.flush_wgrads();
  }
  void output_grads(Run& V, size_t gt, size_t gv) {
    const SegPlan& pl = e->plan[0];
    if (e->og.d_seq_t && pl.dx_t && !rc) {
      fail(crct_hidden_grad_add(A(gt), e->og.d_seq_t, c->grad_scale, (int64_t)b->B * b->T * e->d.H, s));
      ++tick;
    }
    if (e->og.d_seq_v && pl.dx_v && !V.rc) {
      V.fail(crct_hidden_grad_add(V.A(gv), e->og.d_seq_v, c->grad_scale, (int64_t)b->B * b->V * e->d.Hv, V.s));
      ++V.tick;
    }
  }
};

int check_batch(const crct_engine* e, const CrctBatch* b) {
  CRCT_REQUIRE(b && b->B >= 1 && b->T >= 1 && b->V >= 1, "engine: bad batch sizes");
  CRCT_REQUIRE(b->B <= e->maxB && b->T <= e->maxT && b->V <= e->maxV, "engine: batch (B=%d,T=%d,V=%d) exceeds the engine maximum (%d,%d,%d)",
               b->B, b->T, b->V, e->maxB, e->maxT, e->maxV);
  CRCT_REQUIRE(b->tokens && b->segments && b->loc && b->image_feat && b->image_loc && b->image_target && b->R, "engine: null batch pointer");
  CRCT_REQUIRE(b->text_keymask || (b->sep_indices && b->hist_len && b->sep_stride > 0), "engine: text_keymask, or sep_indices + hist_len, is required");
  CRCT_REQUIRE(b->image_keymask || b->image_mask, "engine: image_keymask or image_mask is required");
  return 0;
}

void replan(crct_engine* e) {
  const size_t nseg = e->sched.size() + 2;
  e->plan.assign(nseg, SegPlan());
  e->emb_own_t = e->emb_own_v = true;
  if (e->nograd.empty()) return;
  auto lin = [&](const LinearP& l) { return e->w_grad(l) || e->b_grad(l); };
  auto ln = [&](const LnP& l) { return e->grad_at(l.g) || e->grad_at(l.b); };
  auto proj = [&](const ProjP& p) { return lin(p.dense) || ln(p.ln); };
  auto ffn = [&](const FfnP& p) { return lin(p.up) || lin(p.down) || ln(p.ln); };
  auto drops = [&](const LinearP& l, bool with_bias) { return e->drops_wgrad(l, with_bias) ? 1 : 0; };
  auto self_drops = [&](const SelfLayerP& l) { return drops(l.qkv, true) + drops(l.proj.dense, false) + drops(l.ffn.up, true) + drops(l.ffn.down, false); };
  bool below_t = e->grad_at(e->et.word) || e->grad_at(e->et.pos) || e->grad_at(e->et.type) || e->grad_at(e->et.wloc) ||
                 e->grad_at(e->et.bloc) || ln(e->et.ln);
  bool below_v = (e->feat ? lin(e->ev.img) : lin(e->ev.areas)) || e->grad_at(e->ev.color) || e->grad_at(e->ev.wloc) ||
                 e->grad_at(e->ev.bloc) || ln(e->ev.ln);
  e->emb_own_t = below_t; e->emb_own_v = below_v;
  below_t = below_t || e->ig_text();
  below_v = below_v || e->ig_vis();
  SegPlan& emb = e->plan[nseg - 1];
  emb.runs = below_t || below_v; emb.dx_t = below_t; emb.dx_v = below_v;
  emb.dropped = (e->feat && below_v) ? drops(e->ev.img, false) : 0;
  for (size_t i = 0; i < e->sched.size(); ++i) {
    const Step& st = e->sched[i];
    SegPlan& pl = e->plan[e->sched.size() - i];
    pl.dx_t = below_t; pl.dx_v = below_v;
    if (st.kind == 't' || st.kind == 'v') {
      const SelfLayerP& l = st.kind == 't' ? e->tl[st.idx] : e->vl[st.idx];
      bool& below = st.kind == 't' ? below_t : below_v;
      pl.runs = below || lin(l.qkv) || proj(l.proj) || ffn(l.ffn);
      pl.dropped = pl.runs ? self_drops(l) : 0;
      below = pl.runs;
    } else {
      const ConnLayerP& l = e->cl[st.idx];
      pl.runs = below_t || below_v || lin(l.qkv1) || lin(l.qkv2) || proj(l.proj_v) || proj(l.proj_t) || ffn(l.ffn_v) || ffn(l.ffn_t);
      pl.dropped = !pl.runs ? 0 : drops(l.qkv1, true) + drops(l.qkv2, true) + drops(l.proj_v.dense, false) + drops(l.proj_t.dense, false) +
                                    drops(l.ffn_v.up, true) + drops(l.ffn_v.down, false) + drops(l.ffn_t.up, true) + drops(l.ffn_t.down, false);
      below_t = below_v = pl.runs;
    }
    if (!pl.runs) pl.dx_t = pl.dx_v = false;
  }
  SegPlan& hd = e->plan[0];
  const bool reg = e->var.regressor != CRCT_REGRESSOR_NONE;
  bool own = lin(e->t_pool) || lin(e->v_pool) || lin(e->cls);
  int dropped = drops(e->t_pool, false) + drops(e->v_pool, false);
  for (int j = 0; j < 4 && reg; ++j) {
    own = own || lin(e->tp[j]) || lin(e->vp[j]) || lin(e->fu[j]);
    dropped += drops(e->tp[j], false) + drops(e->vp[j], false) + (j < 3 ? drops(e->fu[j], false) : 0);
  }
  hd.runs = own || below_t || below_v;
  hd.dx_t = hd.runs && below_t; hd.dx_v = hd.runs && below_v;
  hd.dropped = hd.runs ? dropped : 0;
}

}

extern "C" crct_engine_t* crct_engine_create_variant(const CrctModelDims* dims, const char* names, const int64_t* offsets,
                                                     const int64_t* sizes, int n_params, int max_B, int max_T, int max_V,
                                                     const CrctVariant* variant) {
  if (!dims || !names || !offsets || !sizes) { crct_set_error("engine_create: null argument"); return nullptr; }
  if (variant && (variant->dataset < CRCT_DATASET_PLOTQA || variant->dataset > CRCT_DATASET_FIGUREQA ||
                  variant->regressor < CRCT_REGRESSOR_PLOTQA || variant->regressor > CRCT_REGRESSOR_CE ||
                  variant->n_values < 0 || variant->n_values > CRCT_CE_CLASSES)) {
    crct_set_error("engine_create: bad variant (dataset %d, regressor %d, %d values)", variant->dataset, variant->regressor, variant->n_values);
    return nullptr;
  }
  if (variant && variant->regressor == CRCT_REGRESSOR_CE && variant->n_values != CRCT_CE_CLASSES) {
    crct_set_error("engine_create: the CE regressor needs the %d class values", CRCT_CE_CLASSES);
    return nullptr;
  }
  crct_engine* e = new crct_engine();
  e->d = *dims; e->maxB = max_B; e->maxT = max_T; e->maxV = max_V;
  if (variant) e->var = *variant;
  e->feat = e->var.dataset == CRCT_DATASET_PLOTQA;
  const CrctModelDims& D = e->d;
  {
    const char* p = names;
    for (int i = 0; i < n_params; ++i) {
      const char* q = strchr(p, '\n');
      std::string k = q ? std::string(p, q - p) : std::string(p);
      e->off[k] = offsets[i]; e->size[k] = sizes[i];
      e->param_off.push_back(offsets[i]);
      if (!q) break;
      p = q + 1;
    }
  }
  auto fail = [&](const char* msg) -> crct_engine_t* { if (msg) crct_set_error("%s", msg); delete e; return nullptr; };
  if (D.H % D.heads || D.Hv % D.v_heads || D.Hb % D.b_heads) return fail("engine_create: hidden size not a multiple of heads");
  if (D.H % 8 || D.Hv % 8 || D.Hb % 8 || D.I % 8 || D.Iv % 8 || D.Fv % 8) return fail("engine_create: sizes must be multiples of 8");
  if (D.n_conn > 32) return fail("engine_create: more than 32 connection layers");
  {
    int vs = 0, ts = 0;
    for (int c = 0; c < D.n_conn; ++c) {
      for (int i = vs; i < D.v_biatt[c]; ++i) e->sched.push_back({'v', i});
      for (int i = ts; i < D.t_biatt[c]; ++i) e->sched.push_back({'t', i});
      if (D.with_coattention) e->sched.push_back({'c', c});
      vs = D.v_biatt[c]; ts = D.t_biatt[c];
    }
    for (int i = vs; i < D.Lv; ++i) e->sched.push_back({'v', i});
    for (int i = ts; i < D.L; ++i) e->sched.push_back({'t', i});
    for (size_t i = 0; i < e->sched.size() && e->first_conn < 0; ++i)
      if (e->sched[i].kind == 'c') e->first_conn = (int)i;
  }
  char buf[256];
  uint32_t site = 16;
  for (int i = 0; i < D.L; ++i, site += 4) {
    snprintf(buf, sizeof(buf), "bert.encoder.layer.%d.", i);
    e->tl.push_back(self_layer_p(e, buf, D.H, D.I, D.heads, D.p_attn, D.p_hidden, site, CRCT_SITE_T_QKV));
  }
  for (int i = 0; i < D.Lv; ++i, site += 4) {
    snprintf(buf, sizeof(buf), "bert.encoder.v_layer.%d.", i);
    e->vl.push_back(self_layer_p(e, buf, D.Hv, D.Iv, D.v_heads, D.p_v_attn, D.p_v_hidden, site, CRCT_SITE_V_QKV));
  }
  for (int i = 0; i < D.n_conn; ++i) {
    snprintf(buf, sizeof(buf), "bert.encoder.c_layer.%d.", i);
    std::string p(buf);
    ConnLayerP l;
    l.site = site; site += 8;
    l.qkv1 = fused3(e, p + "biattention.query1", p + "biattention.key1", p + "biattention.value1", D.Hv, D.Hb, CRCT_SITE_C_QKV_V);
    l.qkv2 = fused3(e, p + "biattention.query2", p + "biattention.key2", p + "biattention.value2", D.H, D.Hb, CRCT_SITE_C_QKV_T);
    l.proj_v.dense = linear_p(e, p + "biOutput.dense1", D.Hb, D.Hv, CRCT_SITE_C_OUT_V); l.proj_v.ln = ln_p(e, p + "biOutput.LayerNorm1");
    l.proj_t.dense = linear_p(e, p + "biOutput.dense2", D.Hb, D.H, CRCT_SITE_C_OUT_T); l.proj_t.ln = ln_p(e, p + "biOutput.LayerNorm2");
    l.ffn_v.up = linear_p(e, p + "v_intermediate.dense", D.Hv, D.Iv, CRCT_SITE_V_FFN_UP);
    l.ffn_v.down = linear_p(e, p + "v_output.dense", D.Iv, D.Hv, CRCT_SITE_V_FFN_DN); l.ffn_v.ln = ln_p(e, p + "v_output.LayerNorm");
    l.ffn_t.up = linear_p(e, p + "t_intermediate.dense", D.H, D.I, CRCT_SITE_T_FFN_UP);
    l.ffn_t.down = linear_p(e, p + "t_output.dense", D.I, D.H, CRCT_SITE_T_FFN_DN); l.ffn_t.ln = ln_p(e, p + "t_output.LayerNorm");
    e->cl.push_back(l);
  }
  e->et.word = e->P("bert.embeddings.word_embeddings.weight");
  e->et.pos = e->P("bert.embeddings.position_embeddings.weight");
// ... 249 lines not shown
}
extern "C" size_t crct_engine_workspace_bytes(const crct_engine_t* e) { return e ? e->ws_bytes : 0; }
extern "C" int crct_engine_num_segments(const crct_engine_t* e) { return e ? (int)e->seg_range.size() : 0; }
extern "C" int crct_engine_segment_range(const crct_engine_t* e, int seg, int64_t* lo, int64_t* hi) {
  CRCT_REQUIRE(e && seg >= 0 && seg < (int)e->seg_range.size(), "segment_range: bad segment %d", seg);
  *lo = e->seg_range[seg].first; *hi = e->seg_range[seg].second;
  return 0;
}

namespace {

int ensure_streams(crct_engine* e, hipStream_t main) {
  if (!e->placed) {
    e->placed = true;
    e->placed_for = main;
    hipStream_t out[4];
    if (int r = crct_streams_place(main, out, &e->queue_classes)) return r;
    e->side[0] = out[0]; e->side[1] = out[1]; e->aux = out[2]; e->side[2] = out[3];
    const size_t index_bytes = (size_t)2 * e->d.vocab * sizeof(int32_t);
    if (hipMalloc((void**)&e->word_index, index_bytes) != hipSuccess) {
      e->word_index = nullptr;
      (void)hipGetLastError();
      crct_set_error("engine: cannot allocate the word index (%zu bytes)", index_bytes);
      return 1;
    }
    CRCT_CHECK_HIP(hipMemsetAsync(e->word_index, 0, index_bytes, main));
    CRCT_CHECK_HIP(hipStreamSynchronize(main));
  }
  for (int k = 0; k < 3; ++k) {
    const bool need = k == 0 ? e->use_vis_stream : (e->use_wgrad_stream && !(k == 2 && e->one_wgrad_stream));
    if (need && !e->side[k] && hipStreamCreateWithFlags(&e->side[k], hipStreamNonBlocking) != hipSuccess) {
      crct_set_error("engine: cannot create an internal HIP stream");
      return 1;
    }
  }
  return 0;
}

void make_runs(crct_engine* e, const float* p32, const void* p16, float* g32, void* ws, hipStream_t main, const CrctBatch* batch,
               const CrctStepCfg* cfg, Run& Rt, Run& Rv) {
  hipStream_t vis = e->use_vis_stream ? e->side[0] : main;
  Rt = Run{e, p32, (const bf16_t*)p16, g32, (char*)ws, main, batch, cfg, e->use_wgrad_stream ? e->side[1] : main,
           e->partials[0], e->colsum_part[0], e->colsum_part[2]};
  Rv = Run{e, p32, (const bf16_t*)p16, g32, (char*)ws, vis, batch, cfg, e->use_wgrad_stream ? e->side[e->one_wgrad_stream ? 1 : 2] : vis,
           e->partials[1], e->colsum_part[1], e->colsum_part[3]};
  Rt.sets[0] = &e->st; Rt.sets[1] = &e->st2;
  Rv.sets[0] = &e->sv; Rv.sets[1] = &e->sv2;
  Rt.which = 0; Rv.which = 1;
}

int reset_tickets(crct_engine* e, void* ws, hipStream_t s) {
  bool any = false;
  for (int a = 1; a < CRCT_SITE_COUNT && !any; ++a)
    for (int k = 0; k < 2; ++k)
      for (int ph = 0; ph < 2; ++ph) any = any || e->policy[a][k][ph].split_k > 1;
  if (!any) return 0;
  CRCT_CHECK_HIP(hipMemsetAsync((char*)ws + e->sk_cnt[0], 0, (size_t)2 * e->sk_tickets * 4, s));
  return 0;
}

}

extern "C" int crct_engine_forward(crct_engine_t* e, const float* params_f32, const void* params_bf16, const CrctBatch* batch,
                                   const CrctStepCfg* cfg, void* workspace, float* logits, float* reg, float* stats,
                                   crct_stream_t stream) {
  CRCT_REQUIRE(e && params_f32 && params_bf16 && cfg && workspace && logits && reg && stats, "engine_forward: null argument");
  if (int r = check_batch(e, batch)) return r;
  CRCT_REQUIRE(!cfg->fp8 || (e->feat && e->var.regressor == CRCT_REGRESSOR_PLOTQA),
               "engine_forward: the fp8 step is built for the PlotQA model only, not for the dvqa / figure_qa variants");
  if (int r = ensure_streams(e, (hipStream_t)stream)) return r;
  e->evnext = 0;
  e->fwd_r32 = cfg->residual_fp32 != 0;
  CrctDeviceScope on_device;
  CrctBatch bl = *batch;
  if (!bl.text_keymask || !bl.image_keymask) {
    uint8_t* kt = bl.text_keymask ? nullptr : (uint8_t*)workspace + e->km_t;
    uint8_t* kv = bl.image_keymask ? nullptr : (uint8_t*)workspace + e->km_v;
    if (int r = crct_build_keymasks(bl.sep_indices, bl.hist_len, bl.sep_stride, bl.image_mask, kt, kv, bl.B, bl.T, bl.V, stream)) return r;
    if (kt) bl.text_keymask = kt;
    if (kv) bl.image_keymask = kv;
  }
  batch = &bl;
  Run Rt, Rv;
  make_runs(e, params_f32, params_bf16, nullptr, workspace, (hipStream_t)stream, batch, cfg, Rt, Rv);
  if (int r = reset_tickets(e, workspace, (hipStream_t)stream)) return r;
  Rv.fail(order_streams(e, Rt.s, Rv.s));
  const int nseg = (int)e->seg_range.size();
  auto wait_params = [&](Run& R, int seg) {
    if (!cfg->seg_ready_events || R.rc) return;
#ifdef CRCT_GEMM_LAB
    static const bool lab_no_wait = getenv("CRCT_LAB_NO_PARAM_WAIT") != nullptr;
    if (lab_no_wait) return;
#endif
    hipEvent_t ev = (hipEvent_t)cfg->seg_ready_events[seg];
    if (ev && hipStreamWaitEvent(R.s, ev, 0) != hipSuccess) { crct_set_error("engine: wait on a parameter-ready event failed"); R.rc = 1; }
  };
  wait_params(Rt, nseg - 1);
  wait_params(Rv, nseg - 1);
  Rt.embed_text_fwd();
  Rv.embed_image_fwd();
  for (size_t i = 0; i < e->sched.size(); ++i) {
    const Step& st = e->sched[i];
    const StepIn& x = e->in[i];
    const int seg = (int)(e->sched.size() - i);
    Rt.phase = (e->first_conn < 0 || (int)i < e->first_conn) ? 0 : 1;
    if (st.kind != 'v') wait_params(Rt, seg);
    if (st.kind != 't') wait_params(Rv, seg);
    if (st.kind == 't') Rt.self_fwd(e->tl[st.idx], e->tla[st.idx], x.t, batch->text_keymask, batch->B, batch->T);
    else if (st.kind == 'v') Rv.self_fwd(e->vl[st.idx], e->vla[st.idx], x.v, batch->image_keymask, batch->B, batch->V);
    else Rt.conn_fwd(Rv, e->cl[st.idx], e->cla[st.idx], x);
  }
  Rt.phase = 1;
  wait_params(Rt, 0);
  wait_params(Rv, 0);
  Rt.heads_branch_fwd(false, e->in.back().t.x);
  Rv.heads_branch_fwd(true, e->in.back().v.x);
  Rt.fail(order_streams(e, Rv.s, Rt.s));
  Rt.heads_tail_fwd(logits, reg, stats);
  return Rt.rc ? Rt.rc : Rv.rc;
}

extern "C" int crct_engine_backward(crct_engine_t* e, const float* params_f32, const void* params_bf16, const CrctBatch* batch,
                                    const CrctStepCfg* cfg, void* workspace, float* grads_f32, float* logits, float* reg,
                                    float* stats, int seg, crct_stream_t stream) {
  CRCT_REQUIRE(e && params_f32 && params_bf16 && cfg && workspace && grads_f32 && logits && reg && stats, "engine_backward: null argument");
  CRCT_REQUIRE(batch && batch->labels, "engine_backward: labels are required (training step)");
  if (int r = check_batch(e, batch)) return r;
  CRCT_REQUIRE(!e->ig.d_areas || e->areas, "engine_backward: d_areas is requested (crct_engine_set_input_grads) but the batch has no areas (crct_engine_set_areas)");
  if (int r = ensure_streams(e, (hipStream_t)stream)) return r;
  e->evnext = 0;
  CrctDeviceScope on_device;
  CrctBatch bl = *batch;
  if (!bl.text_keymask) bl.text_keymask = (const uint8_t*)workspace + e->km_t;
  if (!bl.image_keymask) bl.image_keymask = (const uint8_t*)workspace + e->km_v;
  batch = &bl;
  Run Rt, Rv;
  make_runs(e, params_f32, params_bf16, grads_f32, workspace, (hipStream_t)stream, batch, cfg, Rt, Rv);
  const int nseg = (int)e->seg_range.size();
  const int s0 = seg < 0 ? 0 : seg, s1 = seg < 0 ? nseg : seg + 1;
  CRCT_REQUIRE(s1 <= nseg, "engine_backward: bad segment %d", seg);
  if (s0 == 0) e->wgrad_pass_begin();
  if (seg >= 0 && !e->plan[seg].runs) return 0;
  if (int r = reset_tickets(e, workspace, (hipStream_t)stream)) return r;
  Rv.fail(order_streams(e, Rt.s, Rv.s));
  int ev_from = s0;
  for (int sgi = s0; sgi < s1 && !Rt.rc && !Rv.rc; ++sgi) {
    const bool in_sched = sgi != 0 && sgi != nseg - 1;
    const size_t si = in_sched ? e->sched.size() - (size_t)sgi : 0;
    Rt.phase = (in_sched && (e->first_conn < 0 || (int)si < e->first_conn)) ? 0 : 1;
    const SegPlan& pl = e->plan[sgi];
    if (!pl.runs) {
    } else if (sgi == 0) {
      e->cur_t = 0; e->cur_v = 0;
      Rt.heads_bwd(Rv, e->in.back().t.x, e->in.back().v.x, e->st.dy[0], e->sv.dy[0], logits, reg, stats);
    } else if (sgi == nseg - 1) {
      if (pl.dx_t && e->emb_own_t) Rt.embed_text_bwd(e->st.dy[e->cur_t]);
      if (pl.dx_t && e->ig_text()) Rt.embed_text_input_grads(e->st.dy[e->cur_t]);
      if (pl.dx_v && (e->emb_own_v || e->ig.d_image_feat)) Rv.embed_image_bwd(e->sv.dy[e->cur_v]);
      if (pl.dx_v && e->ig_vis()) Rv.embed_image_input_grads(e->sv.dy[e->cur_v]);
    } else {
      const Step& st = e->sched[si];
      const StepIn& x = e->in[si];
      const size_t gt = e->st.dy[e->cur_t], gxt = e->st.dy[e->cur_t ^ 1], gv = e->sv.dy[e->cur_v], gxv = e->sv.dy[e->cur_v ^ 1];
      if (st.kind == 't') Rt.self_bwd(e->tl[st.idx], e->tla[st.idx], x.t, gt, gxt, batch->text_keymask, batch->B, batch->T, pl.dx_t);
      else if (st.kind == 'v') Rv.self_bwd(e->vl[st.idx], e->vla[st.idx], x.v, gv, gxv, batch->image_keymask, batch->B, batch->V, pl.dx_v);
      else Rt.conn_bwd(Rv, e->cl[st.idx], e->cla[st.idx], x, gv, gt, gxv, gxt, pl.dx_v, pl.dx_t);
      if (st.kind != 'v') e->cur_t ^= 1;
      if (st.kind != 't') e->cur_v ^= 1;
    }
    if (seg < 0 && cfg->seg_done_events && !Rt.rc && !Rv.rc) {
      Rt.flush_wgrads();
      Rv.flush_wgrads();
      hipStream_t ss[4] = {Rt.s, Rt.sw, Rv.s, Rv.sw};
      for (int sg = ev_from; sg <= sgi; ++sg) {
        if (cfg->seg_done_mask && !cfg->seg_done_mask[sg]) continue;
        for (int k = 0; k < 4; ++k) {
          hipEvent_t ev = (hipEvent_t)cfg->seg_done_events[4 * sg + k];
          if (ev && hipEventRecord(ev, ss[k]) != hipSuccess) { crct_set_error("engine_backward: cannot record a segment event"); Rt.rc = 1; }
        }
        if (cfg->seg_enqueued && !Rt.rc) cfg->seg_enqueued(sg, cfg->seg_enqueued_user);
      }
    }
    ev_from = sgi + 1;
  }
  Rt.main_after_wgrad();
  Rv.main_after_wgrad();
  Rt.fail(order_streams(e, Rv.s, Rt.s));
  return Rt.rc ? Rt.rc : Rv.rc;
}

extern "C" int crct_engine_wgrad_owned(crct_engine_t* e, int64_t* offsets, int64_t* numels, int cap) {
  if (!e) return -1;
  std::vector<std::pair<int64_t, int64_t>> v(e->wgrad_owned.begin(), e->wgrad_owned.end());
  std::sort(v.begin(), v.end());
  int n = 0;
  for (const auto& kv : v) {
    if (offsets && numels && n < cap) { offsets[n] = kv.first; numels[n] = kv.second; }
    ++n;
  }
  return n;
}

extern "C" int crct_engine_fp8_sites(const crct_engine_t* e) { return e ? e->n_sites : 0; }
extern "C" int crct_engine_fp8_grad_sites(const crct_engine_t* e) { return e ? e->n_gsites : 0; }
extern "C" int crct_engine_fp8_weights(const crct_engine_t* e, int64_t* offsets, int64_t* numels, int cap) {
  if (!e) return -1;
  const int n = (int)e->wq_list.size();
  for (int i = 0; i < n && i < cap && offsets && numels; ++i) { offsets[i] = e->wq_list[i].first; numels[i] = e->wq_list[i].second; }
  return n;
}

extern "C" int crct_engine_set_streams(crct_engine_t* e, int use_visual_stream, int use_wgrad_streams) {
  if (!e) return 1;
  e->use_vis_stream = use_visual_stream != 0;
  e->use_wgrad_stream = use_wgrad_streams != 0;
  e->one_wgrad_stream = use_wgrad_streams == 2;
  e->streams_forced = true;
  return 0;
}

extern "C" void* crct_event_create(void) {
  hipEvent_t ev = nullptr;
  const unsigned flags = hipEventDisableTiming | hipEventDisableSystemFence;
  if (hipEventCreateWithFlags(&ev, flags) != hipSuccess) { crct_set_error("event_create: hipEventCreateWithFlags failed"); return nullptr; }
  return ev;
}
extern "C" void crct_event_destroy(void* ev) { if (ev) (void)hipEventDestroy((hipEvent_t)ev); }
extern "C" int crct_event_record(void* ev, crct_stream_t stream) {
  CRCT_REQUIRE(ev, "event_record: null event");
  CRCT_CHECK_HIP(hipEventRecord((hipEvent_t)ev, (hipStream_t)stream));
  return 0;
}
extern "C" int crct_stream_wait_event(crct_stream_t stream, void* ev) {
  CRCT_REQUIRE(ev, "stream_wait_event: null event");
  CRCT_CHECK_HIP(hipStreamWaitEvent((hipStream_t)stream, (hipEvent_t)ev, 0));
  return 0;
}
extern "C" int crct_event_query(void* ev) {
  if (!ev) return -1;
  const hipError_t r = hipEventQuery((hipEvent_t)ev);
  if (r == hipSuccess) return 1;
  if (r == hipErrorNotReady) { (void)hipGetLastError(); return 0; }
  crct_set_error("event_query: %s", hipGetErrorString(r));
  return -1;
}
extern "C" int crct_event_synchronize(void* ev) {
  CRCT_REQUIRE(ev, "event_synchronize: null event");
  CRCT_CHECK_HIP(hipEventSynchronize((hipEvent_t)ev));
  return 0;
}

extern "C" crct_stream_t crct_engine_aux_stream(crct_engine_t* e, crct_stream_t main_stream, int* queue_classes) {
  if (!e) return nullptr;
  if (ensure_streams(e, (hipStream_t)main_stream)) return nullptr;
  if (queue_classes) *queue_classes = e->queue_classes;
  return e->aux;
}

extern "C" int crct_engine_streams(crct_engine_t* e, crct_stream_t out[4]) {
  if (!e || !out) return 1;
  out[0] = e->side[0]; out[1] = e->side[1]; out[2] = e->side[2]; out[3] = e->aux;
  return 0;
}

extern "C" int crct_engine_set_wgrad_workgroups(crct_engine_t* e, int target_wgs, int max_rows) {
  if (!e) return 1;
  e->wgrad_target = target_wgs > 0 ? target_wgs : 0;
  e->wgrad_target_rows = max_rows;
  return 0;
}
extern "C" int crct_engine_set_wgrad_flush(crct_engine_t* e, int mode) {
  if (!e) return 1;
  e->wgrad_flush = mode;
  return 0;
}

extern "C" int crct_engine_set_ln_addend(crct_engine_t* e, int on) {
  if (!e) return 1;
  e->ln_addend = on != 0;
  e->ws_update();
  return 0;
}

extern "C" int crct_engine_set_site_policy(crct_engine_t* e, int site, int kind, int phase, int cfg, int split_k) {
  CRCT_REQUIRE(e && site > 0 && site < CRCT_SITE_COUNT && kind >= CRCT_KIND_FWD && kind <= CRCT_KIND_WGRAD && phase <= 1,
               "set_site_policy: bad site / kind / phase (%d, %d, %d)", site, kind, phase);
  CRCT_REQUIRE(cfg == -1 || crct_gemm_config_built(cfg), "set_site_policy: configuration %d is not built", cfg);
  CRCT_REQUIRE(split_k >= 0 && split_k <= 4, "set_site_policy: split_k %d out of range", split_k);
  for (int ph = 0; ph < 2; ++ph)
    if (phase < 0 || phase == ph) { e->policy[site][kind][ph].cfg = cfg; e->policy[site][kind][ph].split_k = split_k; }
  return 0;
}

extern "C" int64_t crct_engine_tap(crct_engine_t* e, const void* workspace, const char* name, int B, int T, int V, void* out,
                                   int64_t cap, crct_stream_t stream) {
  if (!e || !name) return -1;
  auto copy = [&](const Tap& t) -> int64_t {
    const int64_t n = t.stream == 't' ? (int64_t)B * T * (t.width ? t.width : e->d.H) : (int64_t)B * V * (t.width ? t.width : e->d.Hv);
    if (n > cap) { crct_set_error("tap: buffer too small"); return -1; }
    if (hipMemcpyAsync(out, (const char*)workspace + t.off, (size_t)n * 2, hipMemcpyDeviceToDevice, (hipStream_t)stream) != hipSuccess) return -1;
    return n;
  };
  if (!strcmp(name, "grad.t")) return copy(Tap{name, e->st.dy[e->cur_t], 't'});
  if (!strcmp(name, "grad.v")) return copy(Tap{name, e->sv.dy[e->cur_v], 'v'});
  for (const Tap& t : e->taps)
    if (t.name == name) return copy(t);
  crct_set_error("tap: unknown activation '%s'", name);
  return -1;
}

extern "C" int64_t crct_engine_attention_probs(crct_engine_t* e, const CrctBatch* batch, const CrctStepCfg* cfg, const void* workspace, int kind,
                                               int index, int direction, float* out, int64_t cap, crct_stream_t stream) {
  if (!e || !cfg || !workspace || !out) { crct_set_error("engine_attention_probs: null argument"); return -1; }
  if (check_batch(e, batch)) return -1;
  const CrctModelDims& D = e->d;
  const char* ws = (const char*)workspace;
  const uint8_t* km_t = batch->text_keymask ? batch->text_keymask : (const uint8_t*)ws + e->km_t;
  const uint8_t* km_v = batch->image_keymask ? batch->image_keymask : (const uint8_t*)ws + e->km_v;
  const int B = batch->B, T = batch->T, V = batch->V;
  const bf16_t* q = nullptr;
  const bf16_t* k = nullptr;
  const uint8_t* km = nullptr;
  int heads = 0, Tq = 0, Tk = 0, H = 0;
  float p = 0.f;
  uint32_t site = 0;
  if (kind == 0 || kind == 1) {
    const std::vector<SelfLayerP>& lp = kind == 0 ? e->tl : e->vl;
    const std::vector<SelfLayerA>& la = kind == 0 ? e->tla : e->vla;
    if (index < 0 || index >= (int)lp.size()) { crct_set_error("engine_attention_probs: %s layer %d out of range [0,%d)", kind == 0 ? "text" : "visual", index, (int)lp.size()); return -1; }
    if (direction != 0) { crct_set_error("engine_attention_probs: direction %d belongs to connection layers (kind 2)", direction); return -1; }
    H = lp[index].H; heads = lp[index].heads; Tq = Tk = kind == 0 ? T : V;
    q = (const bf16_t*)(ws + la[index].qkv); k = q + H;
    km = kind == 0 ? km_t : km_v;
    p = lp[index].p_attn; site = lp[index].site;
  } else if (kind == 2) {
    if (index < 0 || index >= (int)e->cl.size() || !D.with_coattention) { crct_set_error("engine_attention_probs: connection layer %d out of range [0,%d)", index, D.with_coattention ? (int)e->cl.size() : 0); return -1; }
    if (direction != 0 && direction != 1) { crct_set_error("engine_attention_probs: direction %d must be 0 (text over visual) or 1 (visual over text)", direction); return -1; }
    const ConnLayerA& a = e->cla[index];
    H = D.Hb; heads = D.b_heads;
    const bf16_t* qkv1 = (const bf16_t*)(ws + a.qkv1);
    const bf16_t* qkv2 = (const bf16_t*)(ws + a.qkv2);
    if (direction == 0) { q = qkv2; k = qkv1 + H; km = km_v; Tq = T; Tk = V; p = D.p_v_attn; site = e->cl[index].site; }
    else { q = qkv1; k = qkv2 + H; km = km_t; Tq = V; Tk = T; p = D.p_attn; site = e->cl[index].site + 1; }
  } else {
    crct_set_error("engine_attention_probs: unknown kind %d (0 text, 1 visual, 2 connection layer)", kind);
    return -1;
  }
  const int64_t n = (int64_t)B * heads * Tq * Tk;
  if (n > cap) { crct_set_error("engine_attention_probs: %lld elements do not fit the buffer of %lld", (long long)n, (long long)cap); return -1; }
  Drop dr;
  if (cfg->training && p > 0.f) { dr.thr = thr_of(p); dr.scale = 1.0f / (1.0f - p); }
  if (crct_attention_probs(q, k, km, out, B, heads, Tq, Tk, H / heads, 3 * H, 3 * H, dr.thr, dr.scale, site, cfg->seed, stream)) return -1;
  return n;
}
```

cqa-crct_amd/csrc/rowops.hip:

```cpp
#include <type_traits>

#include "common.hip.h"
#include "crct_internal.h"

namespace {

constexpr int ROWS_PER_BLOCK = 4;

template <int NCH>
struct Row {
  float v[NCH][8];
};

template <int NCH>
__device__ __forceinline__ void row_load_bf16(Row<NCH>& r, const bf16_t* p, int H, int lane) {
  uint4 u[NCH];
#pragma unroll
  for (int i = 0; i < NCH; ++i) u[i] = *reinterpret_cast<const uint4*>(p + min((lane + 64 * i) * 8, H - 8));
#pragma unroll
  for (int i = 0; i < NCH; ++i) {
    const uint32_t m = (lane + 64 * i) * 8 < H ? 0xffffffffu : 0u;
    const uint32_t x = u[i].x & m, y = u[i].y & m, z = u[i].z & m, w = u[i].w & m;
    r.v[i][0] = bf2f((bf16_t)(x & 0xffff)); r.v[i][1] = bf2f((bf16_t)(x >> 16));
    r.v[i][2] = bf2f((bf16_t)(y & 0xffff)); r.v[i][3] = bf2f((bf16_t)(y >> 16));
// ... 417 lines not shown
    for (int u = 0; u < 4; ++u) m[u] = __ballot(v[u] == id);
  };
  int cnt = own ? 1 : 0;
  if (own && l > r)
    for (int base = (r + 1) & ~63; base <= l; base += 256) {
      unsigned long long m[4];
      hits4(base, m);
      cnt += __builtin_popcountll(m[0]) + __builtin_popcountll(m[1]) + __builtin_popcountll(m[2]) + __builtin_popcountll(m[3]);
    }
  if (lane == 0) { s_cnt[w] = cnt; s_last[w] = l; }
  __syncthreads();
  if (own && cnt <= WORD_HEAVY) {
    Row<NCH> acc;
    row_zero(acc);
    row_add_f32(acc, rows + (long)r * H, H, lane);
    if (cnt > 1)
      for (int base = (r + 1) & ~63; base <= l; base += 256) {
        unsigned long long m[4];
        hits4(base, m);
#pragma unroll
        for (int u = 0; u < 4; ++u)
          while (m[u]) {
            const int j = base + 64 * u + __builtin_ctzll(m[u]);
            m[u] &= m[u] - 1;
            row_add_f32(acc, rows + (long)j * H, H, lane);
          }
      }
    row_add_f32(acc, table + (long)id * H, H, lane);
    row_store_f32(acc, table + (long)id * H, H, lane);
  }
  if (own && lane == 0) { first[id] = 0; last[id] = 0; }
  for (int k = 0; k < ROWS_PER_BLOCK; ++k) {
    const int n = s_cnt[k];
    if (n <= WORD_HEAVY) continue;
    const int rk = blk * ROWS_PER_BLOCK + k, idk = (int)ids[rk], lk = s_last[k];
    if (w == k) {
      int at = 0;
      if (lane == 0) list[0] = rk;
      at = 1;
      for (int base = (rk + 1) & ~63; base <= lk; base += 256) {
        unsigned long long m[4];
        hits4(base, m);
#pragma unroll
        for (int u = 0; u < 4; ++u) {
          if ((m[u] >> lane) & 1ull) list[at + __builtin_popcountll(m[u] & ((1ull << lane) - 1ull))] = base + 64 * u + lane;
          at += __builtin_popcountll(m[u]);
        }
      }
    }
    __syncthreads();
    Row<NCH> a0, a1, a2, a3;
    row_zero(a0); row_zero(a1); row_zero(a2); row_zero(a3);
    int e = w * 4;
    for (; e + 3 < n; e += 16) {
      const int j0 = list[e], j1 = list[e + 1], j2 = list[e + 2], j3 = list[e + 3];
      row_add_f32(a0, rows + (long)j0 * H, H, lane);
      row_add_f32(a1, rows + (long)j1 * H, H, lane);
      row_add_f32(a2, rows + (long)j2 * H, H, lane);
      row_add_f32(a3, rows + (long)j3 * H, H, lane);
    }
    if (e < n) row_add_f32(a0, rows + (long)list[e] * H, H, lane);
    if (e + 1 < n) row_add_f32(a1, rows + (long)list[e + 1] * H, H, lane);
    if (e + 2 < n) row_add_f32(a2, rows + (long)list[e + 2] * H, H, lane);
#pragma unroll
    for (int i = 0; i < NCH; ++i)
#pragma unroll
      for (int j = 0; j < 8; ++j) a0.v[i][j] = (a0.v[i][j] + a1.v[i][j]) + (a2.v[i][j] + a3.v[i][j]);
    row_store_f32(a0, part + (long)w * H, H, lane);
    __syncthreads();
    if (w == k) {
      Row<NCH> t, u;
      row_load_f32(t, part, H, lane);
      row_load_f32(u, part + H, H, lane);
#pragma unroll
      for (int i = 0; i < NCH; ++i)
#pragma unroll
        for (int j = 0; j < 8; ++j) t.v[i][j] += u.v[i][j];
      row_load_f32(u, part + 2 * (long)H, H, lane);
      Row<NCH> v;
      row_load_f32(v, part + 3 * (long)H, H, lane);
#pragma unroll
      for (int i = 0; i < NCH; ++i)
#pragma unroll
        for (int j = 0; j < 8; ++j) t.v[i][j] += u.v[i][j] + v.v[i][j];
      row_add_f32(t, table + (long)idk * H, H, lane);
      row_store_f32(t, table + (long)idk * H, H, lane);
    }
    __syncthreads();
  }
}

template <int NCH>
__global__ __launch_bounds__(256) void word_scatter_kernel(const float* __restrict__ rows, const int64_t* __restrict__ ids, int M, int H,
                                                           float* __restrict__ table, int* __restrict__ first, int* __restrict__ last) {
  extern __shared__ __attribute__((aligned(16))) char smem[];
  word_scatter_indexed_body<NCH>(rows, ids, M, H, table, first, last, blockIdx.x, smem);
}
template <int NCH>
__global__ __launch_bounds__(256) void embed_scatter_kernel(const float* __restrict__ rows, const int* __restrict__ idx, int M, int H,
                                                            float* __restrict__ d_pos, int n0, const int* __restrict__ idx1,
                                                            float* __restrict__ d_type, int n_gather, const int64_t* __restrict__ ids,
                                                            float* __restrict__ d_word, int* __restrict__ w_first, int* __restrict__ w_last) {
  extern __shared__ __attribute__((aligned(16))) char smem[];
  if ((int)blockIdx.x < n_gather) gather_sum_body(rows, idx, M, H, d_pos, n0, idx1, d_type, blockIdx.x, smem);
  else word_scatter_indexed_body<NCH>(rows, ids, M, H, d_word, w_first, w_last, (int)blockIdx.x - n_gather, smem);
}

struct LnFwdP {
  const bf16_t* x; const float* gamma; const float* beta; bf16_t* y; float* mean_o; float* rstd_o; int M, H; float eps;
  uint32_t thr; float scale; uint32_t site; uint64_t seed; uint8_t* q_out; const float* q_scale; float* q_amax;
  int x_f32; float* y_f32;
};
template <int NCH>
__device__ __forceinline__ void ln_fwd_body(const LnFwdP& a, const int blk, const int nblk) {
  const int lane = threadIdx.x & 63, wave = threadIdx.x >> 6;
  const int M = a.M, H = a.H;
  Row<NCH> g, b;
  row_load_f32(g, a.gamma, H, lane);
  row_load_f32(b, a.beta, H, lane);
  const float qs = a.q_out ? a.q_scale[0] : 0.f;
  float amax = 0.f;
  const long stride = (long)nblk * ROWS_PER_BLOCK;
  for (long row = (long)blk * ROWS_PER_BLOCK + wave; row < M; row += stride) {
    Row<NCH> r;
    if (a.x_f32) row_load_f32(r, reinterpret_cast<const float*>(a.x) + row * H, H, lane);
    else row_load_bf16(r, a.x + row * H, H, lane);
    float mean, rstd;
    row_stats(r, H, lane, a.eps, mean, rstd);
    row_normalize(r, g, b, H, lane, mean, rstd, row, a.thr, a.scale, a.site, a.seed);
    row_store_bf16(r, a.y + row * H, H, lane);
    if (a.y_f32) row_store_f32_nt(r, a.y_f32 + row * H, H, lane);
    if (a.q_out) amax = amax_join(amax, row_store_fp8(r, a.q_out + row * H, H, lane, qs));
    if (lane == 0) { a.mean_o[row] = mean; a.rstd_o[row] = rstd; }
  }
  if (a.q_out && a.q_amax) {
    amax = amax_wave(amax);
    if (lane == 0) amax_update(a.q_amax, amax);
  }
}
template <int NCH>
__global__ __launch_bounds__(256) void ln_fwd_kernel(const bf16_t* x, const float* gamma, const float* beta, bf16_t* y, float* mean_o, float* rstd_o, int M, int H,
                                                       float eps, uint32_t thr, const LnFwdP a_in) {
  LnFwdP a = a_in;
  a.x = x; a.gamma = gamma; a.beta = beta; a.y = y; a.mean_o = mean_o; a.rstd_o = rstd_o; a.M = M; a.H = H; a.eps = eps; a.thr = thr;
  ln_fwd_body<NCH>(a, blockIdx.x, gridDim.x);
}
#define LN_FWD_HOT(p) (p).x, (p).gamma, (p).beta, (p).y, (p).mean_o, (p).rstd_o, (p).M, (p).H, (p).eps, (p).thr,

struct LnBwdP {
  const bf16_t* dy; const bf16_t* x; const float* mean; const float* rstd; const float* gamma; bf16_t* dx; bf16_t* dxl;
  float* partials; int M, H; uint32_t post_thr; float post_scale; uint32_t post_site; uint32_t lin_thr; float lin_scale;
  uint32_t lin_site; uint64_t seed;
  uint8_t* q_out; const float* q_scale; float* q_amax;
};
template <int NCH, bool COMBINE, bool X32>
__device__ __forceinline__ void ln_bwd_body(const LnBwdP& a, const int blk, const int nblk) {
  const bf16_t* __restrict__ dy_p = a.dy; const bf16_t* __restrict__ x_p = a.x;
  const float* __restrict__ mean_p = a.mean; const float* __restrict__ rstd_p = a.rstd; const float* __restrict__ gamma = a.gamma;
  bf16_t* __restrict__ dx_p = a.dx; bf16_t* __restrict__ dxl_p = a.dxl; float* __restrict__ partials = a.partials;
  const int M = a.M, H = a.H;
  const uint32_t post_thr = a.post_thr, post_site = a.post_site, lin_thr = a.lin_thr, lin_site = a.lin_site;
  const float post_scale = a.post_scale, lin_scale = a.lin_scale;
  const uint64_t seed = a.seed;
  const int lane = threadIdx.x & 63, wave = threadIdx.x >> 6;
  Row<NCH> adg, adb, adl, g;
  row_zero(adg); row_zero(adb); row_zero(adl);
  row_load_f32(g, gamma, H, lane);
  const float qs = a.q_out ? a.q_scale[0] : 0.f;
  float q_amax = 0.f;
  const long stride = (long)nblk * ROWS_PER_BLOCK;
  long row = (long)blk * ROWS_PER_BLOCK + wave;
  RawRow<NCH> dy_n;
  typename std::conditional<X32, RawRowF<NCH>, RawRow<NCH>>::type x_n;
  const float* __restrict__ x32_p = reinterpret_cast<const float*>(a.x);
  float mean_n = 0.f, rstd_n = 0.f;
  if (row < M) {
    row_fetch_bf16(dy_n, dy_p + row * H, H, lane);
    if constexpr (X32) row_fetch_f32(x_n, x32_p + row * H, H, lane);
    else row_fetch_bf16(x_n, x_p + row * H, H, lane);
    mean_n = mean_p[row]; rstd_n = rstd_p[row];
  }
  for (; row < M; row += stride) {
    Row<NCH> dy, x;
    const float mean = mean_n, rstd = rstd_n;
    row_unpack_bf16(dy, dy_n, H, lane);
    if constexpr (X32) row_unpack_f32(x, x_n, H, lane);
    else row_unpack_bf16(x, x_n, H, lane);
    if (row + stride < M) {
      row_fetch_bf16(dy_n, dy_p + (row + stride) * H, H, lane);
      if constexpr (X32) row_fetch_f32(x_n, x32_p + (row + stride) * H, H, lane);
      else row_fetch_bf16(x_n, x_p + (row + stride) * H, H, lane);
      mean_n = mean_p[row + stride]; rstd_n = rstd_p[row + stride];
    }
    row_apply_dropmask(dy, H, lane, row, post_thr, post_scale, post_site, seed);
    row_ln_bwd(dy, x, g, H, lane, mean, rstd, adg, adb);
    row_store_bf16(dy, dx_p + row * H, H, lane);
    if (dxl_p) {
      row_apply_dropmask(dy, H, lane, row, lin_thr, lin_scale, lin_site, seed);
      row_store_bf16(dy, dxl_p + row * H, H, lane);
    }
    if (a.q_out) q_amax = amax_join(q_amax, row_store_bf8(dy, a.q_out + row * H, H, lane, qs));
    row_acc(adl, dy);
  }
  if (a.q_out && a.q_amax) {
    q_amax = amax_wave(q_amax);
    if (lane == 0) amax_update(a.q_amax, q_amax);
  }
  if constexpr (COMBINE) {
    extern __shared__ __attribute__((aligned(16))) float ln_lds[];
    row_store_f32(adg, ln_lds + (0 * ROWS_PER_BLOCK + wave) * H, H, lane);
    row_store_f32(adb, ln_lds + (1 * ROWS_PER_BLOCK + wave) * H, H, lane);
    row_store_f32(adl, ln_lds + (2 * ROWS_PER_BLOCK + wave) * H, H, lane);
    __syncthreads();
    const int H4 = H >> 2;
    for (int i = threadIdx.x; i < 3 * H4; i += 256) {
      const int q = i / H4, c = (i - q * H4) << 2;
      const float* src = ln_lds + (long)q * ROWS_PER_BLOCK * H + c;
      const float4 a = *reinterpret_cast<const float4*>(src), b = *reinterpret_cast<const float4*>(src + H);
      const float4 d = *reinterpret_cast<const float4*>(src + 2 * H), e = *reinterpret_cast<const float4*>(src + 3 * H);
      *reinterpret_cast<float4*>(partials + ((long)q * nblk + blk) * H + c) =
          make_float4((a.x + b.x) + (d.x + e.x), (a.y + b.y) + (d.y + e.y), (a.z + b.z) + (d.z + e.z), (a.w + b.w) + (d.w + e.w));
    }
  } else {
    const long nr = (long)nblk * ROWS_PER_BLOCK, pr = (long)blk * ROWS_PER_BLOCK + wave;
    row_store_f32(adg, partials + (0 * nr + pr) * H, H, lane);
    row_store_f32(adb, partials + (1 * nr + pr) * H, H, lane);
    row_store_f32(adl, partials + (2 * nr + pr) * H, H, lane);
  }
}

template <int NCH, bool COMBINE, bool X32 = false>
__global__ __launch_bounds__(256) void ln_bwd_kernel(const bf16_t* dy, const bf16_t* x, const float* mean, const float* rstd, const float* gamma, int M, int H,
                                                       bf16_t* dx, bf16_t* dxl, const LnBwdP a_in) {
  LnBwdP a = a_in;
  a.dy = dy; a.x = x; a.mean = mean; a.rstd = rstd; a.gamma = gamma; a.M = M; a.H = H; a.dx = dx; a.dxl = dxl;
  ln_bwd_body<NCH, COMBINE, X32>(a, blockIdx.x, gridDim.x);
}
#define LN_BWD_HOT(p) (p).dy, (p).x, (p).mean, (p).rstd, (p).gamma, (p).M, (p).H, (p).dx, (p).dxl,

struct FinalizeArgs {
  float* out[10];
  int stride[10];
  int Q, nblk, H, accumulate;
  const float* partials;
};
__global__ __launch_bounds__(256) void finalize_partials_kernel(const FinalizeArgs a) {
  __shared__ float4 red[32][9];
  const int q = blockIdx.y;
  float* o = a.out[q];
  if (!o) return;
  const int cl = threadIdx.x & 7, rg = threadIdx.x >> 3;
  const int c = blockIdx.x * 32 + cl * 4;
  float4 s = make_float4(0.f, 0.f, 0.f, 0.f);
  if (c < a.H) {
    const float* p = a.partials + ((long)q * a.nblk) * a.H + c;
    float4 acc[8];
#pragma unroll
    for (int u = 0; u < 8; ++u) acc[u] = s;
    int b = rg;
    for (; b + 224 < a.nblk; b += 256) {
      float4 x[8];
#pragma unroll
      for (int u = 0; u < 8; ++u) x[u] = *reinterpret_cast<const float4*>(p + (long)(b + 32 * u) * a.H);
#pragma unroll
      for (int u = 0; u < 8; ++u) { acc[u].x += x[u].x; acc[u].y += x[u].y; acc[u].z += x[u].z; acc[u].w += x[u].w; }
    }
    for (; b + 96 < a.nblk; b += 128) {
      float4 x[4];
#pragma unroll
      for (int u = 0; u < 4; ++u) x[u] = *reinterpret_cast<const float4*>(p + (long)(b + 32 * u) * a.H);
#pragma unroll
      for (int u = 0; u < 4; ++u) { acc[u].x += x[u].x; acc[u].y += x[u].y; acc[u].z += x[u].z; acc[u].w += x[u].w; }
    }
    for (; b < a.nblk; b += 32) {
      const float4 x0 = *reinterpret_cast<const float4*>(p + (long)b * a.H);
      acc[0].x += x0.x; acc[0].y += x0.y; acc[0].z += x0.z; acc[0].w += x0.w;
    }
    s.x = ((acc[0].x + acc[1].x) + (acc[2].x + acc[3].x)) + ((acc[4].x + acc[5].x) + (acc[6].x + acc[7].x));
    s.y = ((acc[0].y + acc[1].y) + (acc[2].y + acc[3].y)) + ((acc[4].y + acc[5].y) + (acc[6].y + acc[7].y));
    s.z = ((acc[0].z + acc[1].z) + (acc[2].z + acc[3].z)) + ((acc[4].z + acc[5].z) + (acc[6].z + acc[7].z));
    s.w = ((acc[0].w + acc[1].w) + (acc[2].w + acc[3].w)) + ((acc[4].w + acc[5].w) + (acc[6].w + acc[7].w));
  }
  red[rg][cl] = s;
  __syncthreads();
  if (rg == 0 && c < a.H) {
    float4 t = make_float4(0.f, 0.f, 0.f, 0.f);
#pragma unroll
    for (int k = 0; k < 32; ++k) { const float4 r = red[k][cl]; t.x += r.x; t.y += r.y; t.z += r.z; t.w += r.w; }
    const float tv[4] = {t.x, t.y, t.z, t.w};
#pragma unroll
    for (int j = 0; j < 4; ++j) {
      if (c + j < a.H) {
        const long oi = (long)(c + j) * a.stride[q];
        o[oi] = a.accumulate ? o[oi] + tv[j] : tv[j];
      }
    }
  }
}

__global__ __launch_bounds__(256) void colsum_kernel(const bf16_t* __restrict__ x, long ld, float* __restrict__ partials, int M, int N) {
  const int nb = gridDim.y;
  const int c = (blockIdx.x * 256 + threadIdx.x) * 4;
  if (c >= N) return;
  float s[4][4];
#pragma unroll
  for (int u = 0; u < 4; ++u)
#pragma unroll
    for (int j = 0; j < 4; ++j) s[u][j] = 0.f;
  const bf16_t* p = x + c;
  int r = blockIdx.y;
  for (; r + 3 * nb < M; r += 4 * nb) {
    uint2 v[4];
#pragma unroll
    for (int u = 0; u < 4; ++u) v[u] = *reinterpret_cast<const uint2*>(p + (long)(r + u * nb) * ld);
#pragma unroll
    for (int u = 0; u < 4; ++u) {
      s[u][0] += bf2f((bf16_t)(v[u].x & 0xffff)); s[u][1] += bf2f((bf16_t)(v[u].x >> 16));
      s[u][2] += bf2f((bf16_t)(v[u].y & 0xffff)); s[u][3] += bf2f((bf16_t)(v[u].y >> 16));
    }
  }
  for (; r < M; r += nb) {
    const uint2 v = *reinterpret_cast<const uint2*>(p + (long)r * ld);
    s[0][0] += bf2f((bf16_t)(v.x & 0xffff)); s[0][1] += bf2f((bf16_t)(v.x >> 16));
    s[0][2] += bf2f((bf16_t)(v.y & 0xffff)); s[0][3] += bf2f((bf16_t)(v.y >> 16));
  }
  float4 o;
  o.x = (s[0][0] + s[1][0]) + (s[2][0] + s[3][0]); o.y = (s[0][1] + s[1][1]) + (s[2][1] + s[3][1]);
  o.z = (s[0][2] + s[1][2]) + (s[2][2] + s[3][2]); o.w = (s[0][3] + s[1][3]) + (s[2][3] + s[3][3]);
  *reinterpret_cast<float4*>(partials + (long)blockIdx.y * N + c) = o;
}

template <bool IN_BF16>
__device__ __forceinline__ float4 softmax_load4(const void* xr, int c) {
  if constexpr (!IN_BF16) return *reinterpret_cast<const float4*>(reinterpret_cast<const float*>(xr) + c);
  else {
    const uint2 u = *reinterpret_cast<const uint2*>(reinterpret_cast<const bf16_t*>(xr) + c);
    return make_float4(bf2f((bf16_t)(u.x & 0xffff)), bf2f((bf16_t)(u.x >> 16)), bf2f((bf16_t)(u.y & 0xffff)), bf2f((bf16_t)(u.y >> 16)));
  }
}
template <bool IN_BF16>
__global__ __launch_bounds__(256) void softmax_rows_kernel(const void* __restrict__ x, bf16_t* __restrict__ y, int M, int F) {
  const int lane = threadIdx.x & 63, wave = threadIdx.x >> 6;
  for (long row = (long)blockIdx.x * ROWS_PER_BLOCK + wave; row < M; row += (long)gridDim.x * ROWS_PER_BLOCK) {
    const void* xr = IN_BF16 ? (const void*)(reinterpret_cast<const bf16_t*>(x) + row * F) : (const void*)(reinterpret_cast<const float*>(x) + row * F);
    float mx = -INFINITY;
    for (int c = lane * 4; c < F; c += 256) {
      const float4 v = softmax_load4<IN_BF16>(xr, c);
      mx = fmaxf(fmaxf(mx, fmaxf(v.x, v.y)), fmaxf(v.z, v.w));
    }
    mx = wave_max(mx);
    float s = 0.f;
    for (int c = lane * 4; c < F; c += 256) {
      const float4 v = softmax_load4<IN_BF16>(xr, c);
      s += expf(v.x - mx) + expf(v.y - mx) + expf(v.z - mx) + expf(v.w - mx);
// ... 390 lines not shown
        d = fmaf(expf(v.x - mx) * inv, gg.x, d); d = fmaf(expf(v.y - mx) * inv, gg.y, d);
        d = fmaf(expf(v.z - mx) * inv, gg.z, d); d = fmaf(expf(v.w - mx) * inv, gg.w, d);
      }
      d = wave_sum(d);
      for (int c = lane * 4; c < F; c += 256) {
        const float4 v = softmax_load4<IN_BF16>(xr, c);
        const float4 gg = *reinterpret_cast<const float4*>(gr + c);
        *reinterpret_cast<float4*>(dr + c) = make_float4(expf(v.x - mx) * inv * (gg.x - d), expf(v.y - mx) * inv * (gg.y - d),
                                                         expf(v.z - mx) * inv * (gg.z - d), expf(v.w - mx) * inv * (gg.w - d));
      }
    }
  }
}

template <int NCH, bool S_BF16>
__global__ __launch_bounds__(256) void ln_rows_f32_kernel(const void* __restrict__ s_p, const float* __restrict__ mean_p,
                                                          const float* __restrict__ rstd_p, const float* __restrict__ gamma,
                                                          const float* __restrict__ beta, float* __restrict__ y, int M, int H) {
  const int lane = threadIdx.x & 63, wave = threadIdx.x >> 6;
  Row<NCH> g, b;
  row_load_f32(g, gamma, H, lane);
  row_load_f32(b, beta, H, lane);
  for (long row = (long)blockIdx.x * ROWS_PER_BLOCK + wave; row < M; row += (long)gridDim.x * ROWS_PER_BLOCK) {
    Row<NCH> r;
    if constexpr (S_BF16) row_load_bf16(r, reinterpret_cast<const bf16_t*>(s_p) + row * H, H, lane);
    else row_load_f32(r, reinterpret_cast<const float*>(s_p) + row * H, H, lane);
    row_normalize(r, g, b, H, lane, mean_p[row], rstd_p[row], row, 0u, 1.f, 0u, 0ull);
    row_store_f32(r, y + row * H, H, lane);
  }
}

__device__ __forceinline__ float grad_add1(float x, float c, float g) {
#pragma clang fp contract(off)
  const float p = c * g;
  return x + p;
}
__global__ __launch_bounds__(256) void hidden_grad_add_kernel(bf16_t* __restrict__ x, const float* __restrict__ g, float c, long n) {
  long i = ((long)blockIdx.x * blockDim.x + threadIdx.x) * 8;
  const long stride = (long)gridDim.x * blockDim.x * 8;
  for (; i + 8 <= n; i += stride) {
    const uint4 u = *reinterpret_cast<const uint4*>(x + i);
    const float4 a = *reinterpret_cast<const float4*>(g + i), b = *reinterpret_cast<const float4*>(g + i + 4);
    uint4 o;
    o.x = pack2bf(grad_add1(bf2f((bf16_t)(u.x & 0xffff)), c, a.x), grad_add1(bf2f((bf16_t)(u.x >> 16)), c, a.y));
    o.y = pack2bf(grad_add1(bf2f((bf16_t)(u.y & 0xffff)), c, a.z), grad_add1(bf2f((bf16_t)(u.y >> 16)), c, a.w));
    o.z = pack2bf(grad_add1(bf2f((bf16_t)(u.z & 0xffff)), c, b.x), grad_add1(bf2f((bf16_t)(u.z >> 16)), c, b.y));
    o.w = pack2bf(grad_add1(bf2f((bf16_t)(u.w & 0xffff)), c, b.z), grad_add1(bf2f((bf16_t)(u.w >> 16)), c, b.w));
    *reinterpret_cast<uint4*>(x + i) = o;
  }
  if (i < n && i + 8 > n)
    for (long j = i; j < n; ++j) x[j] = f2bf(grad_add1(bf2f(x[j]), c, g[j]));
}

inline int nch_for(int H) { return (H / 8 + 63) / 64; }
#ifndef CRCT_LN_FWD_GRID_CAP
#define CRCT_LN_FWD_GRID_CAP 2048
#endif
inline int row_grid(long M, int cap) {
  long g = (M + ROWS_PER_BLOCK - 1) / ROWS_PER_BLOCK;
  return (int)(g < 1 ? 1 : (g > cap ? cap : g));
}

#define DISPATCH_NCH(H, ...)                                           \
  switch (nch_for(H)) {                                                \
    case 1: { constexpr int NCH = 1; __VA_ARGS__; } break;             \
    case 2: { constexpr int NCH = 2; __VA_ARGS__; } break;             \
    case 3: { constexpr int NCH = 3; __VA_ARGS__; } break;             \
    case 4: { constexpr int NCH = 4; __VA_ARGS__; } break;             \
    default: crct_set_error("row width %d > 2048 unsupported", H); return 2; \
  }

int launch_finalize(const FinalizeArgs& fa, hipStream_t s) {
  crct_launch(finalize_partials_kernel, dim3((fa.H + 31) / 32, fa.Q), dim3(256), 0, s, fa);
  return hipGetLastError() == hipSuccess ? 0 : 1;
}

}

extern "C" {

static LnFwdP ln_fwd_problem(const CrctLnFwdArgs& a) {
  return LnFwdP{(const bf16_t*)a.x, a.gamma, a.beta, (bf16_t*)a.y, a.mean, a.rstd, a.M, a.H, a.eps, a.drop_thr, a.drop_scale,
                a.drop_site, a.seed, (uint8_t*)a.q_out, a.q_scale, a.q_amax, a.x_f32, a.y_f32};
}
static int ln_fwd_check(const CrctLnFwdArgs& a) {
  CRCT_REQUIRE(a.H % 8 == 0 && a.H > 0, "layernorm: H=%d must be a positive multiple of 8", a.H);
  CRCT_REQUIRE(!a.q_out || a.q_scale, "layernorm_fwd: q_out needs q_scale");
  return 0;
}
static int ln_fwd_launch(const CrctLnFwdArgs& a, hipStream_t s) {
  if (int r = ln_fwd_check(a)) return r;
  if (a.M <= 0) return 0;
  const LnFwdP p = ln_fwd_problem(a);
  DISPATCH_NCH(a.H, crct_launch((ln_fwd_kernel<NCH>), dim3(row_grid(a.M, CRCT_LN_FWD_GRID_CAP)), dim3(256), 0, s, LN_FWD_HOT(p) p));
  CRCT_CHECK_HIP(hipGetLastError());
  return 0;
}

int crct_layernorm_fwd(const void* x, const float* gamma, const float* beta, void* y, float* mean, float* rstd,
                       int M, int H, float eps, uint32_t drop_thr, float drop_scale, uint32_t drop_site,
                       uint64_t seed, crct_stream_t stream) {
  const CrctLnFwdArgs a = {x, gamma, beta, y, mean, rstd, M, H, eps, drop_thr, drop_scale, drop_site, seed, nullptr, nullptr, nullptr, 0, nullptr};
  return ln_fwd_launch(a, (hipStream_t)stream);
}
int crct_layernorm_fwd_args(const CrctLnFwdArgs* a, crct_stream_t stream) {
  CRCT_REQUIRE(a, "layernorm_fwd_args: null argument");
  return ln_fwd_launch(*a, (hipStream_t)stream);
}

int crct_layernorm_fwd_q(const void* x, const float* gamma, const float* beta, void* y, float* mean, float* rstd,
                         int M, int H, float eps, uint32_t drop_thr, float drop_scale, uint32_t drop_site,
                         uint64_t seed, void* q_out, const float* q_scale, float* q_amax, crct_stream_t stream) {
  CRCT_REQUIRE(q_out && q_scale, "layernorm_fwd_q: q_out and q_scale are required");
  const CrctLnFwdArgs a = {x, gamma, beta, y, mean, rstd, M, H, eps, drop_thr, drop_scale, drop_site, seed, q_out, q_scale, q_amax, 0, nullptr};
  return ln_fwd_launch(a, (hipStream_t)stream);
}

int crct_layernorm_rows_f32(const void* s, int s_is_bf16, const float* mean, const float* rstd, const float* gamma, const float* beta,
                            float* y_f32, int M, int N, crct_stream_t stream) {
  CRCT_REQUIRE(s && mean && rstd && gamma && beta && y_f32, "layernorm_rows_f32: null argument");
  CRCT_REQUIRE(N % 8 == 0 && N > 0, "layernorm_rows_f32: N=%d must be a positive multiple of 8", N);
  CRCT_REQUIRE((((uintptr_t)s | (uintptr_t)gamma | (uintptr_t)beta | (uintptr_t)y_f32) & 15) == 0, "layernorm_rows_f32: 16-byte aligned buffers");
  if (M <= 0) return 0;
  hipStream_t st = (hipStream_t)stream;
  const dim3 grid(row_grid(M, CRCT_LN_FWD_GRID_CAP));
  if (s_is_bf16) { DISPATCH_NCH(N, crct_launch((ln_rows_f32_kernel<NCH, true>), grid, dim3(256), 0, st, s, mean, rstd, gamma, beta, y_f32, M, N)); }
  else { DISPATCH_NCH(N, crct_launch((ln_rows_f32_kernel<NCH, false>), grid, dim3(256), 0, st, s, mean, rstd, gamma, beta, y_f32, M, N)); }
  CRCT_CHECK_HIP(hipGetLastError());
  return 0;
}

int crct_hidden_grad_add(void* x_bf16, const float* g_f32, float c, int64_t n, crct_stream_t stream) {
  CRCT_REQUIRE(x_bf16 && g_f32, "hidden_grad_add: null argument");
  CRCT_REQUIRE((((uintptr_t)x_bf16 | (uintptr_t)g_f32) & 15) == 0, "hidden_grad_add: 16-byte aligned buffers");
  if (n <= 0) return 0;
  long blocks = (n / 8 + 255) / 256;
  if (blocks > 4096) blocks = 4096;
  if (blocks < 1) blocks = 1;
  crct_launch(hidden_grad_add_kernel, dim3((int)blocks), dim3(256), 0, (hipStream_t)stream, (bf16_t*)x_bf16, g_f32, c, (long)n);
  CRCT_CHECK_HIP(hipGetLastError());
  return 0;
}

static int embed_bwd_blocks(long M) {
  return row_grid(M, CRCT_LN_BWD_MAX_BLOCKS);
}
int crct_layernorm_bwd_blocks(int M) {
  return row_grid(M, CRCT_LN_BWD_MAX_BLOCKS);
}

static bool ln_bwd_combines(int H) {
  return (size_t)3 * ROWS_PER_BLOCK * H * 4 <= 64 * 1024;
}
static LnBwdP ln_bwd_problem(const CrctLnBwdArgs& a) {
  return LnBwdP{(const bf16_t*)a.dy, (const bf16_t*)a.x, a.mean, a.rstd, a.gamma, (bf16_t*)a.dx, (bf16_t*)a.dx_lin, a.partials,
                a.M, a.H, a.post_thr, a.post_scale, a.post_site, a.lin_thr, a.lin_scale, a.lin_site, a.seed,
                (uint8_t*)a.q_out, a.q_scale, a.q_amax};
}
static int ln_bwd_launch(const CrctLnBwdArgs& a, hipStream_t s) {
  CRCT_REQUIRE(a.H % 8 == 0 && a.H > 0, "layernorm_bwd: H=%d must be a positive multiple of 8", a.H);
  if (a.M <= 0) return 0;
  const int nb = crct_layernorm_bwd_blocks(a.M);
  const LnBwdP p = ln_bwd_problem(a);
  if (a.x_f32) {
    if (ln_bwd_combines(a.H)) {
      DISPATCH_NCH(a.H, crct_launch((ln_bwd_kernel<NCH, true, true>), dim3(nb), dim3(256), (size_t)3 * ROWS_PER_BLOCK * a.H * 4, s, LN_BWD_HOT(p) p));
    } else {
      DISPATCH_NCH(a.H, crct_launch((ln_bwd_kernel<NCH, false, true>), dim3(nb), dim3(256), 0, s, LN_BWD_HOT(p) p));
    }
  } else if (ln_bwd_combines(a.H)) {
    DISPATCH_NCH(a.H, crct_launch((ln_bwd_kernel<NCH, true>), dim3(nb), dim3(256), (size_t)3 * ROWS_PER_BLOCK * a.H * 4, s, LN_BWD_HOT(p) p));
  } else {
    DISPATCH_NCH(a.H, crct_launch((ln_bwd_kernel<NCH, false>), dim3(nb), dim3(256), 0, s, LN_BWD_HOT(p) p));
  }
  CRCT_CHECK_HIP(hipGetLastError());
  return 0;
}
int crct_layernorm_bwd_rows(const void* dy, const void* x, const float* mean, const float* rstd, const float* gamma,
                            void* dx, void* dx_lin, float* partials, int M, int H, uint32_t post_thr, float post_scale,
                            uint32_t post_site, uint32_t lin_thr, float lin_scale, uint32_t lin_site, uint64_t seed,
                            crct_stream_t stream) {
  const CrctLnBwdArgs a = {dy, x, mean, rstd, gamma, dx, dx_lin, partials, M, H, post_thr, post_scale, post_site, lin_thr, lin_scale,
                           lin_site, seed, nullptr, nullptr, nullptr, 0};
  return ln_bwd_launch(a, (hipStream_t)stream);
}
int crct_layernorm_bwd_rows_args(const CrctLnBwdArgs* a, crct_stream_t stream) {
  CRCT_REQUIRE(a && (!a->q_out || a->q_scale), "layernorm_bwd_rows_args: bad arguments");
  return ln_bwd_launch(*a, (hipStream_t)stream);
}
int crct_layernorm_bwd_finalize(const float* partials, float* dgamma, float* dbeta, float* dbias_lin, int M, int H,
                                int accumulate, crct_stream_t stream) {
  if (M <= 0) return 0;
  FinalizeArgs fa = {};
  fa.out[0] = dgamma; fa.out[1] = dbeta; fa.out[2] = dbias_lin;
  fa.stride[0] = fa.stride[1] = fa.stride[2] = 1;
  fa.Q = 3; fa.nblk = crct_layernorm_bwd_blocks(M) * (ln_bwd_combines(H) ? 1 : ROWS_PER_BLOCK);
  fa.H = H; fa.accumulate = accumulate; fa.partials = partials;
  return launch_finalize(fa, (hipStream_t)stream);
}

int crct_layernorm_bwd(const void* dy, const void* x, const float* mean, const float* rstd, const float* gamma,
                       void* dx, void* dx_lin, float* dgamma, float* dbeta, float* dbias_lin, float* partials,
                       int M, int H, int accumulate, uint32_t post_thr, float post_scale, uint32_t post_site,
                       uint32_t lin_thr, float lin_scale, uint32_t lin_site, uint64_t seed, crct_stream_t stream) {
  if (int r = crct_layernorm_bwd_rows(dy, x, mean, rstd, gamma, dx, dx_lin, partials, M, H, post_thr, post_scale, post_site,
                                      lin_thr, lin_scale, lin_site, seed, stream)) return r;
  return crct_layernorm_bwd_finalize(partials, dgamma, dbeta, dbias_lin, M, H, accumulate, stream);
}

int crct_colsum_blocks(int M) { int b = (M + 7) / 8; return b < 1 ? 1 : (b > 64 ? 64 : b); }

int crct_colsum_bf16(const void* x, int64_t ld, float* out, float* partials, int M, int N, int accumulate,
                     crct_stream_t stream) {
  CRCT_REQUIRE(N % 4 == 0 && ld % 4 == 0, "colsum: N=%d and ld must be multiples of 4", N);
  if (N <= 0) return 0;
  hipStream_t s = (hipStream_t)stream;
  const int nb = crct_colsum_blocks(M);
  crct_launch(colsum_kernel, dim3((N / 4 + 255) / 256, nb), dim3(256), 0, s, (const bf16_t*)x, (long)ld, partials, M, N);
  CRCT_CHECK_HIP(hipGetLastError());
  FinalizeArgs fa = {};
  fa.out[0] = out; fa.stride[0] = 1; fa.Q = 1; fa.nblk = nb; fa.H = N; fa.accumulate = accumulate; fa.partials = partials;
  return launch_finalize(fa, s);
}

int crct_softmax_rows_f32_bf16(const float* x, void* y, int M, int F, crct_stream_t stream) {
  CRCT_REQUIRE(F % 4 == 0, "softmax_rows: F=%d must be a multiple of 4", F);
  if (M <= 0) return 0;
  crct_launch(softmax_rows_kernel<false>, dim3(row_grid(M, 4096)), dim3(256), 0, (hipStream_t)stream, (const void*)x, (bf16_t*)y, M, F);
  CRCT_CHECK_HIP(hipGetLastError());
  return 0;
}

int crct_softmax_rows_bf16_bf16(const void* x, void* y, int M, int F, crct_stream_t stream) {
  CRCT_REQUIRE(F % 4 == 0, "softmax_rows: F=%d must be a multiple of 4", F);
  if (M <= 0) return 0;
  crct_launch(softmax_rows_kernel<true>, dim3(row_grid(M, 4096)), dim3(256), 0, (hipStream_t)stream, x, (bf16_t*)y, M, F);
  CRCT_CHECK_HIP(hipGetLastError());
  return 0;
}

__global__ __launch_bounds__(256) void build_keymasks_kernel(const int64_t* __restrict__ sep_indices, const int64_t* __restrict__ hist_len,
                                                             int sep_stride, const int64_t* __restrict__ image_mask,
                                                             uint8_t* __restrict__ km_t, uint8_t* __restrict__ km_v, int B, int T, int V) {
  const int i = blockIdx.x * 256 + threadIdx.x;
  if (km_t && i < B * T) {
    const int b = i / T, t = i % T;
    long h = hist_len[b];
    h = h < 0 ? 0 : (h >= sep_stride ? sep_stride - 1 : h);
    km_t[i] = (long)t < sep_indices[(long)b * sep_stride + h] + 1 ? 1 : 0;
  }
  if (km_v && i < B * V) km_v[i] = image_mask[i] != 0 ? 1 : 0;
}

extern "C" int crct_build_keymasks(const int64_t* sep_indices, const int64_t* hist_len, int sep_stride, const int64_t* image_mask,
                                   uint8_t* km_t, uint8_t* km_v, int B, int T, int V, crct_stream_t stream) {
  CRCT_REQUIRE(B > 0 && T > 0 && V > 0, "build_keymasks: bad sizes");
  CRCT_REQUIRE(!km_t || (sep_indices && hist_len && sep_stride > 0), "build_keymasks: sep_indices / hist_len are required for the text mask");
  CRCT_REQUIRE(!km_v || image_mask, "build_keymasks: image_mask is required for the visual mask");
  if (!km_t && !km_v) return 0;
  const int n = B * (T > V ? T : V);
  crct_launch(build_keymasks_kernel, dim3((n + 255) / 256), dim3(256), 0, (hipStream_t)stream, sep_indices, hist_len, sep_stride,
                     image_mask, km_t, km_v, B, T, V);
  CRCT_CHECK_HIP(hipGetLastError());
  return 0;
}

}

namespace {
__global__ __launch_bounds__(256) void fp8_quantize_bf16_kernel(const bf16_t* __restrict__ x, uint8_t* __restrict__ q,
                                                                const float* __restrict__ scale, float* __restrict__ amax_out, long n) {
  const float qs = scale[0];
  float amax = 0.f;
  for (long i = ((long)blockIdx.x * 256 + threadIdx.x) * 8; i + 8 <= n; i += (long)gridDim.x * 256 * 8) {
    const uint4 u = *reinterpret_cast<const uint4*>(x + i);
    const uint32_t w[4] = {u.x, u.y, u.z, u.w};
    float v[8];
#pragma unroll
    for (int j = 0; j < 4; ++j) { v[2 * j] = bf2f((bf16_t)(w[j] & 0xffff)); v[2 * j + 1] = bf2f((bf16_t)(w[j] >> 16)); }
#pragma unroll
    for (int j = 0; j < 8; ++j) amax = amax_join(amax, v[j]);
    *reinterpret_cast<uint2*>(q + i) = pack8_fp8(v, qs);
  }
  if (amax_out) {
    amax = amax_wave(amax);
    if ((threadIdx.x & 63) == 0) amax_update(amax_out, amax);
  }
}
template <int MODE>
__global__ __launch_bounds__(256) void fp8_weights_kernel(const float* __restrict__ p, uint8_t* __restrict__ q,
                                                          const int64_t* __restrict__ seg_off, const int64_t* __restrict__ seg_len,
                                                          const int32_t* __restrict__ seg_slot, const int32_t* __restrict__ blk_seg,
                                                          const int64_t* __restrict__ blk_off, const float* __restrict__ scale,
                                                          float* __restrict__ amax, int n_blk) {
  for (int blk = blockIdx.x; blk < n_blk; blk += gridDim.x) {
    const int sgi = blk_seg[blk], slot = seg_slot[sgi];
    if (slot < 0) continue;
    const int64_t off = blk_off[blk], base = seg_off[sgi] + off;
    int64_t n = seg_len[sgi] - off;
    if (n > 4096) n = 4096;
    const float qs = MODE == 1 ? scale[slot] : 0.f;
    float am = 0.f;
    for (int64_t i = (int64_t)threadIdx.x * 4; i + 4 <= n; i += 1024) {
      const float4 v = *reinterpret_cast<const float4*>(p + base + i);
      if (MODE == 0) am = amax_join(amax_join(am, amax_pair(v.x, v.y)), amax_pair(v.z, v.w));
      else {
        uint32_t w = 0;
        w = __builtin_amdgcn_cvt_pk_fp8_f32(f8_clamp(v.x * qs), f8_clamp(v.y * qs), w, false);
        w = __builtin_amdgcn_cvt_pk_fp8_f32(f8_clamp(v.z * qs), f8_clamp(v.w * qs), w, true);
        *reinterpret_cast<uint32_t*>(q + base + i) = w;
      }
    }
    if (MODE == 0) {
      am = amax_wave(am);
      if ((threadIdx.x & 63) == 0) amax_update(amax + (long)slot * CRCT_FP8_AMAX_LANES, am);
    }
  }
}
__global__ __launch_bounds__(256) void fp8_transpose_kernel(const uint8_t* __restrict__ q, uint8_t* __restrict__ qt,
                                                            const int64_t* __restrict__ w_off, const int32_t* __restrict__ w_out,
                                                            const int32_t* __restrict__ w_in, const int64_t* __restrict__ tile_begin, int n_w,
                                                            long n_tiles) {
  __shared__ uint8_t t[64][80];
  for (long bid = blockIdx.x; bid < n_tiles; bid += gridDim.x) {
  int lo = 0, hi = n_w - 1;
  while (lo < hi) {
    const int mid = (lo + hi + 1) >> 1;
    if (tile_begin[mid] <= bid) lo = mid; else hi = mid - 1;
  }
  const int wi = lo;
  const int out = w_out[wi], in = w_in[wi];
  const int tiles_in = (in + 63) / 64;
  const long tl = bid - tile_begin[wi];
  const int r0 = (int)(tl / tiles_in) * 64, c0 = (int)(tl % tiles_in) * 64;
  const uint8_t* src = q + w_off[wi];
  uint8_t* dst = qt + w_off[wi];
  {
    const int r = threadIdx.x >> 2, ch = (threadIdx.x & 3) * 16;
    uint4 v = make_uint4(0, 0, 0, 0);
    if (r0 + r < out && c0 + ch < in) v = *reinterpret_cast<const uint4*>(src + (long)(r0 + r) * in + c0 + ch);
    *reinterpret_cast<uint4*>(&t[r][ch]) = v;
// ... 335 lines not shown
```

include/crct_hip.h:

```cpp
#ifndef CRCT_HIP_H
#define CRCT_HIP_H
#include <stddef.h>
#include <stdint.h>

#ifdef __cplusplus
extern "C" {
#endif

typedef void* crct_stream_t;

enum { CRCT_ACT_NONE = 0, CRCT_ACT_GELU = 1, CRCT_ACT_RELU = 2, CRCT_ACT_LEAKY = 3, CRCT_ACT_TANH = 4 };

const char* crct_last_error(void);
int crct_abi_version(void);

typedef struct CrctGemmArgs {
  const void* A; const void* B; void* C;
  const float* bias;
  void* preact_out;
  const void* dact_src;
  const void* addend;
  int64_t lda, ldb, ldc, ld_aux, ld_add;
  int32_t M, N, K;
  int32_t ta, tb;
// ... 246 lines not shown
  const float* d_value;
} CrctScoreGrads;
int crct_head_loss_scores(const CrctHeadArgs* args, const CrctScoreGrads* scores, crct_stream_t stream);
int crct_head_loss_variant_scores(const CrctHeadVariantArgs* args, const CrctScoreGrads* scores, crct_stream_t stream);

int crct_eval_select(const float* logits, const float* reg_out, const float* reg_err, const float* reg_terr,
                     const int64_t* num_ans, const int64_t* forced_answers, int Q, int64_t N, float* prob0,
                     int64_t* answers, float* sel_out, float* sel_err, float* sel_terr, crct_stream_t stream);

enum { CRCT_EVAL_TOTAL = 0, CRCT_EVAL_BREAKDOWN = 12, CRCT_EVAL_HISTOGRAM = 192, CRCT_EVAL_ERRORS = 205, CRCT_EVAL_TABLE_WORDS = 206 };
typedef struct CrctEvalScoreArgs {
  const float* logits;
  const float* reg_out; const float* reg_err; const float* reg_terr;
  const int64_t* num_ans;
  const int64_t* forced;
  const int64_t* labels;
  const int64_t* gt_id;
  const uint8_t* needs_reg;
  const float* tolerance;
  const int32_t* cats;
  int64_t* answers;
  float* sel_out; float* sel_err; float* sel_terr;
  uint8_t* flags;
  float* prob0;
  int64_t* tables;
  int64_t N;
  int32_t Q, mode, with_histogram;
} CrctEvalScoreArgs;
int crct_eval_score(const CrctEvalScoreArgs* args, crct_stream_t stream);

typedef struct CrctAmpState { const float* grad_scale; const float* found_inf; const int32_t* step; } CrctAmpState;
int crct_adamw_advance(int32_t* step_dev, const float* found_inf_dev, crct_stream_t stream);
typedef struct CrctFp8Shadow {
  void* q; const int32_t* seg_slot; const float* scale; float* amax;
  void* qt; const int32_t* seg_in; const int64_t* seg_t_base; const int32_t* seg_t_ld;
} CrctFp8Shadow;
int64_t crct_adamw_plan(const int64_t* seg_len, int n_seg, int32_t* blk_seg, int64_t* blk_off, int64_t cap);
int crct_adamw_step(float* p, float* g, float* m, float* v, void* p_bf16,
                    const int64_t* seg_off, const int64_t* seg_len, const float* seg_lr, const float* seg_wd,
                    const int32_t* blk_seg, const int64_t* blk_off, int64_t n_blk,
                    float beta1, float beta2, float eps, int step, const float* inv_scale_dev, const CrctAmpState* amp,
                    const CrctFp8Shadow* fp8_shadow, int max_workgroups, int zero_grads, const void* g_bf16, crct_stream_t stream);

int crct_grad_sumsq(const float* g_f32, const void* g_bf16, const int64_t* seg_off, const int64_t* seg_len, const int32_t* blk_seg,
                    const int64_t* blk_off, int64_t n_blk, float* partials, int norm_kind, int max_workgroups, crct_stream_t stream);
int crct_grad_norm_finalize(const float* partials, const int32_t* blk_seg, int64_t n_blk, int n_seg, int norm_kind, float max_norm,
                            const float* grad_scale_dev, const float* mul_dev, float* out, float* seg_norm, crct_stream_t stream);
int crct_scale_runs(float* g_f32, const float* coef_dev, const int64_t* seg_off, const int64_t* seg_len, const int32_t* blk_seg,
                    const int64_t* blk_off, int64_t n_blk, int max_workgroups, crct_stream_t stream);

typedef struct CrctAttnQuant {
  void* ctx_q; const float* ctx_scale; float* ctx_amax;
  void* dq_q; void* dk_q; void* dv_q;
  const float* dq_scale; float* dq_amax; const float* dkv_scale; float* dkv_amax;
  float* row_lse; const void* ctx; int64_t ld_ctx;
} CrctAttnQuant;
int crct_attention_quant_ok(int Tq, int Tk, int d);
int crct_attention_fwd_q(const void* q, const void* k, const void* v, const uint8_t* keymask, void* ctx,
                         int B, int heads, int Tq, int Tk, int d, int64_t ldq, int64_t ldk, int64_t ldv, int64_t ldo,
                         uint32_t drop_thr, float drop_scale, uint32_t drop_site, uint64_t seed, const CrctAttnQuant* quant,
                         crct_stream_t stream);
int crct_attention_bwd_q(const void* q, const void* k, const void* v, const uint8_t* keymask,
                         const void* dctx, void* dq, void* dk, void* dv,
                         int B, int heads, int Tq, int Tk, int d,
                         int64_t ldq, int64_t ldk, int64_t ldv, int64_t ldo, int64_t lddq, int64_t lddk, int64_t lddv,
                         uint32_t drop_thr, float drop_scale, uint32_t drop_site, uint64_t seed, const CrctAttnQuant* quant,
                         crct_stream_t stream);

typedef struct CrctModelDims {
  int32_t vocab, n_pos, n_types, H, L, heads, I;
  int32_t Fv, Hv, Lv, v_heads, Iv, Hb, b_heads, n_color;
  int32_t n_conn;
  int32_t v_biatt[32], t_biatt[32];
  int32_t fusion_sum, with_coattention;
  float p_hidden, p_attn, p_v_hidden, p_v_attn, p_cls;
} CrctModelDims;

typedef struct crct_engine crct_engine_t;

crct_engine_t* crct_engine_create(const CrctModelDims* dims, const char* names, const int64_t* offsets,
                                  const int64_t* sizes, int n_params, int max_B, int max_T, int max_V);
crct_engine_t* crct_engine_create_variant(const CrctModelDims* dims, const char* names, const int64_t* offsets,
                                          const int64_t* sizes, int n_params, int max_B, int max_T, int max_V,
                                          const CrctVariant* variant);
int crct_engine_set_areas(crct_engine_t*, const float* areas);
typedef struct {
  float* d_image_feat;
  float* d_image_loc;
  float* d_areas;
  float* d_txt_loc;
  float* d_text_emb;
} CrctInputGrads;
int crct_engine_set_input_grads(crct_engine_t*, const CrctInputGrads* req);
typedef struct {
  const float* d_seq_t;
  const float* d_seq_v;
} CrctOutputGrads;
int crct_engine_sequence_outputs(crct_engine_t*, const float* params_f32, const void* workspace, int B, int T, int V,
                                 float* seq_t, float* seq_v, crct_stream_t stream);
int crct_engine_set_output_grads(crct_engine_t*, const CrctOutputGrads* req);
int crct_engine_set_score_grads(crct_engine_t*, const CrctScoreGrads* req);
int crct_engine_set_trainable(crct_engine_t*, const uint8_t* flags, int n);
int crct_engine_backward_plan(const crct_engine_t*, int32_t* plan, int cap_segments);
void crct_engine_destroy(crct_engine_t*);
size_t crct_engine_workspace_bytes(const crct_engine_t*);
int crct_engine_num_segments(const crct_engine_t*);
int crct_engine_segment_range(const crct_engine_t*, int seg, int64_t* lo, int64_t* hi);

typedef struct CrctBatch {
  const int64_t* tokens; const int64_t* segments; const float* loc; const uint8_t* text_keymask;
  const void* image_feat;
  const float* image_loc; const int64_t* image_target; const uint8_t* image_keymask;
  const float* R; const int64_t* labels;
  int32_t B, T, V;
  const int64_t* sep_indices; const int64_t* hist_len; const int64_t* image_mask;
  int32_t sep_stride;
  int32_t image_feat_bf16;
} CrctBatch;

typedef struct CrctStepCfg {
  int32_t training;
  int32_t use_l1, kind_l1;
  float tol_margin, nsp_coeff, reg_coeff, grad_scale;
  uint64_t seed;
  const float* g_nsp_dev;
  const float* g_reg_dev;
  const float* g_loss_dev;
  const void* const* seg_ready_events;
  const void* const* seg_done_events;
  int32_t fp8;
  const void* params_fp8; const float* fp8_w_scale; const float* fp8_act_scale; float* fp8_act_amax;
  int32_t fp8_bwd; int32_t fp8_wgrad;
  const void* params_fp8_t; const float* fp8_grad_scale; float* fp8_grad_amax;
  void (*seg_enqueued)(int seg, void* user);
  void* seg_enqueued_user;
  const int32_t* seg_done_mask;
  int32_t wgrad_overwrite;
  void* grads_bf16;
  int32_t residual_fp32;
} CrctStepCfg;

int crct_engine_forward(crct_engine_t*, const float* params_f32, const void* params_bf16,
                        const CrctBatch* batch, const CrctStepCfg* cfg, void* workspace,
                        float* logits, float* reg, float* stats, crct_stream_t stream);
int crct_engine_backward(crct_engine_t*, const float* params_f32, const void* params_bf16,
                         const CrctBatch* batch, const CrctStepCfg* cfg, void* workspace,
                         float* grads_f32, float* logits, float* reg, float* stats, int seg,
                         crct_stream_t stream);
int crct_engine_set_streams(crct_engine_t*, int use_visual_stream, int use_wgrad_streams);
crct_stream_t crct_engine_aux_stream(crct_engine_t*, crct_stream_t main_stream, int* queue_classes);
int crct_engine_streams(crct_engine_t*, crct_stream_t out[4]);
int crct_engine_set_wgrad_flush(crct_engine_t* e, int mode);
int crct_engine_set_ln_addend(crct_engine_t* e, int on);
int crct_engine_set_wgrad_workgroups(crct_engine_t* e, int target_wgs, int max_rows);
int crct_engine_set_site_policy(crct_engine_t*, int site, int kind, int phase, int cfg, int split_k);
int crct_engine_wgrad_owned(crct_engine_t*, int64_t* offsets, int64_t* numels, int cap);
int crct_zero_runs(float* base, const int64_t* off, const int64_t* len, const int32_t* blk_seg, const int64_t* blk_off,
                   int64_t n_blk, crct_stream_t stream);
int crct_engine_fp8_sites(const crct_engine_t*);
int crct_engine_fp8_grad_sites(const crct_engine_t*);
int crct_engine_fp8_weights(const crct_engine_t*, int64_t* offsets, int64_t* numels, int cap);
void* crct_event_create(void);
void crct_event_destroy(void* ev);
int crct_event_record(void* ev, crct_stream_t stream);
int crct_stream_wait_event(crct_stream_t stream, void* ev);
int crct_event_synchronize(void* ev);
int crct_event_query(void* ev);

int64_t crct_engine_tap(crct_engine_t*, const void* workspace, const char* name, int B, int T, int V,
                        void* out, int64_t cap, crct_stream_t stream);

int64_t crct_engine_attention_probs(crct_engine_t*, const CrctBatch* batch, const CrctStepCfg* cfg,
                                    const void* workspace, int kind, int index, int direction,
                                    float* out, int64_t cap, crct_stream_t stream);

#ifdef __cplusplus
}
#endif
#endif
```

Baseline: 11360 QA-pairs/s.

## Restrict last-layer backward to pooled rows when sequence gradients are unused

```diff
diff --git a/cqa-crct_amd/crct/lib.py b/cqa-crct_amd/crct/lib.py
--- a/cqa-crct_amd/crct/lib.py
+++ b/cqa-crct_amd/crct/lib.py
@@ -182,6 +182,7 @@
     "crct_gemm_group_wgrad_config": (C.c_int, [C.c_int]),
     "crct_engine_set_wgrad_flush": (C.c_int, [vp, C.c_int]),
     "crct_engine_set_ln_addend": (C.c_int, [vp, C.c_int]),
+    "crct_engine_set_sparse_tail": (C.c_int, [vp, C.c_int]),
     "crct_engine_set_wgrad_workgroups": (C.c_int, [vp, C.c_int, C.c_int]),
     "crct_gemm_class_config": (C.c_int, [C.c_int, C.c_int]),
     "crct_gemm_fp8_scaled_mfma": (C.c_int, [C.c_int]),
diff --git a/cqa-crct_amd/csrc/crct_internal.h b/cqa-crct_amd/csrc/crct_internal.h
--- a/cqa-crct_amd/csrc/crct_internal.h
+++ b/cqa-crct_amd/csrc/crct_internal.h
@@ -34,6 +34,7 @@
 int crct_streams_place(hipStream_t main, hipStream_t out[4], int* n_classes);
 
 #define CRCT_LN_BWD_MAX_BLOCKS 256
+int crct_layernorm_bwd_rows_pitch(const CrctLnBwdArgs* a, int pitch, hipStream_t stream);
 
 bool crct_stamp_begin(hipStream_t s, hipEvent_t* start, hipEvent_t* stop);
 void crct_stamp_adopt(hipStream_t s, hipEvent_t start, hipEvent_t stop);
diff --git a/cqa-crct_amd/csrc/engine.cpp b/cqa-crct_amd/csrc/engine.cpp
--- a/cqa-crct_amd/csrc/engine.cpp
+++ b/cqa-crct_amd/csrc/engine.cpp
@@ -188,6 +188,8 @@
   std::vector<Tap> taps;
   std::vector<StepIn> in;
   int cur_t = 0, cur_v = 0;
+  bool tail_t = false, tail_v = false;
+  int sparse_tail = 1;
   bool bad = false;
   int64_t P(const std::string& k) {
     auto it = off.find(k);
@@ -439,10 +441,29 @@
     launch(gemm_args(DGRAD, l, M, dy, lddy, nullptr, 0, dx, lddx, o, q && f8b() == 1 ? q8(dyq) : Q8(), Q8(), q8(out)));
     return out;
   }
-  void lin_wgrad(const void* dy, int64_t lddy, const void* x, int64_t ldx, const LinearP& l, int M, bool with_bias = false, const WgQ8& w8 = WgQ8()) {
+  void lin_wgrad(const void* dy, int64_t lddy, const void* x, int64_t ldx, const LinearP& l, int M, bool with_bias = false, const WgQ8& w8 = WgQ8(),
+                 int pitch = 1) {
     if (rc) return;
     const bool keep = !e->drops_wgrad(l, with_bias);
     if (!keep && !defer_wgrad) return;
+    if (pitch > 1) {
+      if (with_bias && keep) bias_grad(dy, lddy * pitch, l, M);
+      if (rc) return;
+      Opt o; o.f32 = true; o.acc = true;
+      CrctGemmArgs g = gemm_args(WGRAD, l, M, dy, lddy * pitch, x, ldx * pitch, G(l.w), l.in, o);
+      if (!wgrad_owner(g, l, keep)) return;
+      if (!defer_wgrad) { launch(g); return; }
+      pending_rows.push_back(g);
+      pending_rows_keep.push_back(keep);
+      const int Md = M * pitch;
+      CrctGemmArgs d = gemm_args(WGRAD, l, Md, dy, lddy, x, ldx, g.C, l.in, o);
+      d.c_is_f32 = g.c_is_f32; d.accumulate = g.accumulate;
+      if (with_bias && Md % 64 == 0 && l.in % 8 == 0 && l.out % 8 == 0 && lddy % 8 == 0 && ldx % 8 == 0) d.rowsum_out = G(l.b);
+      pending.push_back(d);
+      pending_keep.push_back(0);
+      if (pending.size() == 8) flush_wgrads();
+      return;
+    }
     const bool f8w = f8b() == 1 && c->fp8_wgrad && defer_wgrad && f8_lin(l) && w8.dy.site >= 0 && w8.x.site >= 0 &&
                      l.in % 16 == 0 && l.out % 16 == 0 && lddy % 16 == 0 && ldx % 16 == 0;
     const bool fold = !f8w && with_bias && M % 64 == 0 && l.in % 8 == 0 && l.out % 8 == 0 && lddy % 8 == 0 && ldx % 8 == 0;
@@ -450,14 +471,7 @@
     if (rc) return;
     Opt o; o.f32 = true; o.acc = true;
     CrctGemmArgs g = gemm_args(WGRAD, l, M, dy, lddy, x, ldx, G(l.w), l.in, o, f8w ? q8(w8.dy) : Q8(), f8w ? q8(w8.x) : Q8());
-    if (keep && c->wgrad_overwrite && e->wgrad_owned.count(l.w)) {
-      if (++e->wgrad_pass[l.w] > 1) { rc = 1; crct_set_error("engine_backward: weight gradient at offset %lld is produced twice in one pass but is listed as owned", (long long)l.w); return; }
-      g.accumulate = 0;
-      if (c->grads_bf16) {
-        if (l.in % 8 != 0 || l.w % 8 != 0) { rc = 1; crct_set_error("engine_backward: owned weight gradient at offset %lld (in = %d) cannot be written as bf16 rows", (long long)l.w, l.in); return; }
-        g.C = reinterpret_cast<bf16_t*>(c->grads_bf16) + l.w; g.c_is_f32 = 0;
-      }
-    }
+    if (!wgrad_owner(g, l, keep)) return;
     if (fold) g.rowsum_out = G(l.b);
     if (f8w) {
       if (!keep) return;
@@ -470,11 +484,24 @@
     pending_keep.push_back(keep);
     if (pending.size() == 8) flush_wgrads();
   }
+  bool wgrad_owner(CrctGemmArgs& g, const LinearP& l, bool keep) {
+    if (!(keep && c->wgrad_overwrite && e->wgrad_owned.count(l.w))) return true;
+    if (++e->wgrad_pass[l.w] > 1) { rc = 1; crct_set_error("engine_backward: weight gradient at offset %lld is produced twice in one pass but is listed as owned", (long long)l.w); return false; }
+    g.accumulate = 0;
+    if (c->grads_bf16) {
+      if (l.in % 8 != 0 || l.w % 8 != 0) { rc = 1; crct_set_error("engine_backward: owned weight gradient at offset %lld (in = %d) cannot be written as bf16 rows", (long long)l.w, l.in); return false; }
+      g.C = reinterpret_cast<bf16_t*>(c->grads_bf16) + l.w; g.c_is_f32 = 0;
+    }
+    return true;
+  }
   std::vector<CrctGemmArgs> pending_f8;
   std::vector<uint8_t> pending_keep;
+  std::vector<CrctGemmArgs> pending_rows;
+  std::vector<uint8_t> pending_rows_keep;
   void flush_wgrads() {
     if (!pending.empty() && std::find(pending_keep.begin(), pending_keep.end(), 1) == pending_keep.end()) { pending.clear(); pending_keep.clear(); }
-    if (rc || (pending.empty() && pending_f8.empty() && pending_fin.empty() && pending_bias.empty())) return;
+    if (!pending_rows.empty() && std::find(pending_rows_keep.begin(), pending_rows_keep.end(), 1) == pending_rows_keep.end()) { pending_rows.clear(); pending_rows_keep.clear(); }
+    if (rc || (pending.empty() && pending_rows.empty() && pending_f8.empty() && pending_fin.empty() && pending_bias.empty())) return;
     if (sw == s) ++tick;
     wgrad_after_main();
     for (const BiasJob& j : pending_bias)
@@ -483,14 +510,19 @@
     for (const FinJob& f : pending_fin)
       if (!rc) fail(crct_layernorm_bwd_finalize(f.part, f.dg, f.db, f.dlb, f.M, f.H, 1, sw));
     pending_fin.clear();
-    const int target = (sw != s && !pending.empty() && pending[0].K <= e->wgrad_target_rows && !e->one_wgrad_stream) ? e->wgrad_target : 0;
-    for (size_t i = 0; i < pending.size() && !rc; i += 8) {
-      const int ng = (int)std::min<size_t>(8, pending.size() - i);
-      const uint8_t* kp = pending_keep.data() + i;
-      fail(gemm_grouped_checked(CrctGemmGroup{pending.data() + i, nullptr, ng, std::find(kp, kp + ng, 0) == kp + ng ? nullptr : kp, target}, sw));
-    }
-    pending.clear();
-    pending_keep.clear();
+    const bool throttle = sw != s && !e->one_wgrad_stream;
+    for (int rows = 0; rows < 2; ++rows) {
+      std::vector<CrctGemmArgs>& q = rows ? pending_rows : pending;
+      std::vector<uint8_t>& qk = rows ? pending_rows_keep : pending_keep;
+      const int target = (throttle && !q.empty() && q[0].K <= e->wgrad_target_rows) ? e->wgrad_target : 0;
+      for (size_t i = 0; i < q.size() && !rc; i += 8) {
+        const int ng = (int)std::min<size_t>(8, q.size() - i);
+        const uint8_t* kp = qk.data() + i;
+        fail(gemm_grouped_checked(CrctGemmGroup{q.data() + i, nullptr, ng, std::find(kp, kp + ng, 0) == kp + ng ? nullptr : kp, target}, sw));
+      }
+      q.clear();
+      qk.clear();
+    }
     for (size_t i = 0; i < pending_f8.size() && !rc; i += 8)
       fail(crct_gemm_bf16_grouped(pending_f8.data() + i, (int)std::min<size_t>(8, pending_f8.size() - i), sw));
     pending_f8.clear();
@@ -527,14 +559,14 @@
     o.addend = A(x.x);
   }
   size_t ln_bwd(size_t dy, size_t x, size_t mean, size_t rstd, const LnP& ln, const LinearP& lin, size_t dres, size_t dlin,
-                size_t part, int M, int H, const Drop& dr, GradQ& dlq) {
+                size_t part, int M, int H, const Drop& dr, GradQ& dlq, int pitch = 1) {
     if (!f8b_lin(lin)) dlq.site = -1;
     if (rc) return dres;
     ++tick;
     CrctLnBwdArgs a = {A(dy), A(x), F(mean), F(rstd), P(ln.g), A(dres), dr.thr ? A(dlin) : nullptr, F(part), M, H,
                        0, 1.f, 0, dr.thr, dr.scale, dr.site, c->seed, nullptr, nullptr, nullptr, r32() ? 1 : 0};
     if (dlq.site >= 0) { const Q8 d8 = q8(dlq); a.q_out = d8.q; a.q_scale = d8.scale; a.q_amax = d8.amax; }
-    fail(crct_layernorm_bwd_rows_args(&a, s));
+    fail(pitch > 1 ? crct_layernorm_bwd_rows_pitch(&a, pitch, s) : crct_layernorm_bwd_rows_args(&a, s));
     if (defer_wgrad) pending_fin.push_back(FinJob{F(part), G(ln.g), G(ln.b), G(lin.b), M, H});
     else { wgrad_after_main(); if (!rc) fail(crct_layernorm_bwd_finalize(F(part), G(ln.g), G(ln.b), G(lin.b), M, H, 1, sw)); }
     return dr.thr ? dlin : dres;
@@ -574,11 +606,18 @@
     lin_fwd(ctx, p.dense.in, p.dense, M, Act{a.s}, p.dense.out, o);
     ln_fwd(a.s, p.ln, a.out(p.ln), a.mean, a.rstd, M, p.dense.out);
   }
-  void proj_bwd(const ProjP& p, const ProjA& a, const Act& ctx, size_t g, const StreamScratch& sc, int M, const Drop& dr) {
+  void proj_bwd(const ProjP& p, const ProjA& a, const Act& ctx, size_t g, const StreamScratch& sc, int M, const Drop& dr, int pitch = 1) {
     GradQ dlq{sc.dlq_b, a.g_dl};
-    const size_t dl = ln_bwd(g, a.s, a.mean, a.rstd, p.ln, p.dense, sc.dres_b, sc.dlin_b, sc.part_b, M, p.dense.out, dr, dlq);
-    lin_wgrad(A(dl), p.dense.out, A(ctx.x), p.dense.in, p.dense, M, false, WgQ8{dlq, ctx});
-    lin_dgrad(A(dl), p.dense.out, p.dense, M, A(sc.dctx), p.dense.in, Opt(), dlq);
+    if (pitch > 1 && !rc) {
+      const size_t rows = (size_t)M * pitch;
+      if (hipMemsetAsync(A(sc.dres_b), 0, rows * p.dense.out * 2, s) != hipSuccess ||
+          hipMemsetAsync(A(sc.dctx), 0, rows * p.dense.in * 2, s) != hipSuccess) { crct_set_error("engine: memset failed"); rc = 1; return; }
+      ++tick;
+    }
+    const int64_t rp = pitch;
+    const size_t dl = ln_bwd(g, a.s, a.mean, a.rstd, p.ln, p.dense, sc.dres_b, sc.dlin_b, sc.part_b, M, p.dense.out, dr, dlq, pitch);
+    lin_wgrad(A(dl), p.dense.out, A(ctx.x), p.dense.in, p.dense, M, false, WgQ8{dlq, ctx}, pitch);
+    lin_dgrad(A(dl), p.dense.out * rp, p.dense, M, A(sc.dctx), p.dense.in * rp, Opt(), dlq);
     if (e->wgrad_flush & 2) flush_wgrads();
   }
   void ffn_fwd(const FfnP& p, const FfnA& a, const Act& x, int M, const Drop& dr) {
@@ -588,18 +627,21 @@
     lin_fwd(h, p.down.in, p.down, M, Act{a.s}, p.down.out, o2);
     ln_fwd(a.s, p.ln, a.out(p.ln), a.mean, a.rstd, M, p.down.out);
   }
-  void ffn_bwd(const FfnP& p, const FfnA& a, const Act& x, size_t g, size_t gx, const StreamScratch& sc, int M, const Drop& dr) {
+  void ffn_bwd(const FfnP& p, const FfnA& a, const Act& x, size_t g, size_t gx, const StreamScratch& sc, int M, const Drop& dr, int pitch = 1) {
     const int H = p.down.out, I = p.up.out;
+    const int64_t rp = pitch;
     GradQ dlq{sc.dlq_a, a.g_dl};
-    const size_t dl = ln_bwd(g, a.s, a.mean, a.rstd, p.ln, p.down, sc.dres_a, sc.dlin_a, sc.part_a, M, H, dr, dlq);
-    lin_wgrad(A(dl), H, A(a.h), I, p.down, M, false, WgQ8{dlq, ffn_h(p, a)});
-    Opt o; o.dact_src = A(a.u); o.dact = ACT_GELU; o.ld_aux = I;
-    const GradQ duq = lin_dgrad(A(dl), H, p.down, M, A(sc.du), I, o, dlq, GradQ{sc.duq, f8b_lin(p.up) ? a.g_du : -1});
-    lin_wgrad(A(sc.du), I, A(x.x), H, p.up, M, true, WgQ8{duq, x});
-    Opt o2; o2.addend = A(sc.dres_a); o2.ld_add = H;
-    lin_dgrad(A(sc.du), I, p.up, M, A(gx), H, o2, duq);
+    const size_t dl = ln_bwd(g, a.s, a.mean, a.rstd, p.ln, p.down, sc.dres_a, sc.dlin_a, sc.part_a, M, H, dr, dlq, pitch);
+    lin_wgrad(A(dl), H, A(a.h), I, p.down, M, false, WgQ8{dlq, ffn_h(p, a)}, pitch);
+    Opt o; o.dact_src = A(a.u); o.dact = ACT_GELU; o.ld_aux = I * rp;
+    const GradQ duq = lin_dgrad(A(dl), H * rp, p.down, M, A(sc.du), I * rp, o, dlq, GradQ{sc.duq, f8b_lin(p.up) ? a.g_du : -1});
+    lin_wgrad(A(sc.du), I, A(x.x), H, p.up, M, true, WgQ8{duq, x}, pitch);
+    Opt o2; o2.addend = A(sc.dres_a); o2.ld_add = H * rp;
+    lin_dgrad(A(sc.du), I * rp, p.up, M, A(gx), H * rp, o2, duq);
     if (e->wgrad_flush & 1) flush_wgrads();
   }
+
+  int tail_pitch(bool tail, int T) const { return tail && !f8b() && T > 1 ? T : 1; }
 
   void self_fwd(const SelfLayerP& p, const SelfLayerA& a, const Act& x, const uint8_t* km, int B, int T) {
     const int M = B * T, H = p.H, d = H / p.heads;
@@ -609,14 +651,16 @@
     proj_fwd(p.proj, a.proj, ctx, x, M, drop(p.p_hid, p.site + 1));
     ffn_fwd(p.ffn, a.ffn, a.proj.out(p.proj.ln), M, drop(p.p_hid, p.site + 2));
   }
-  void self_bwd(const SelfLayerP& p, const SelfLayerA& a, const Act& x, size_t g, size_t gx, const uint8_t* km, int B, int T, bool dx = true) {
+  void self_bwd(const SelfLayerP& p, const SelfLayerA& a, const Act& x, size_t g, size_t gx, const uint8_t* km, int B, int T, bool dx = true,
+                bool tail = false) {
     const int M = B * T, H = p.H, d = H / p.heads;
     const StreamScratch& sc = layer_begin();
-    ffn_bwd(p.ffn, a.ffn, a.proj.out(p.proj.ln), g, sc.gc, sc, M, drop(p.p_hid, p.site + 2));
+    const int tp = tail_pitch(tail, T), Mb = tp > 1 ? B : M;
+    ffn_bwd(p.ffn, a.ffn, a.proj.out(p.proj.ln), g, sc.gc, sc, Mb, drop(p.p_hid, p.site + 2), tp);
     const bool aq = attn_q_ok(T, T, d);
     const bool gq = aq && f8b_lin(p.qkv) && f8_lin(p.qkv);
     const GradQ dqkvq{sc.dqkvq, gq ? a.g_dqkv : -1};
-    proj_bwd(p.proj, a.proj, ctx_act(a.ctx, a.ctxq, a.site_ctx, p.proj.dense, aq), sc.gc, sc, M, drop(p.p_hid, p.site + 1));
+    proj_bwd(p.proj, a.proj, ctx_act(a.ctx, a.ctxq, a.site_ctx, p.proj.dense, aq), sc.gc, sc, Mb, drop(p.p_hid, p.site + 1), tp);
     uint8_t* dq8 = gq ? W<uint8_t>(sc.dqkvq) : nullptr;
     attn_bwd(A(a.qkv), 3 * H, A(a.qkv) + H, A(a.qkv) + 2 * H, 3 * H, km, A(sc.dctx), H, A(sc.dqkv), 3 * H, A(sc.dqkv) + H,
              A(sc.dqkv) + 2 * H, 3 * H, B, p.heads, T, T, d, drop(p.p_attn, p.site), dq8, a.g_dqkv, gq ? dq8 + H : nullptr,
@@ -645,18 +689,20 @@
     ffn_fwd(p.ffn_t, a.ffn_t, a.proj_t.out(p.proj_t.ln), Mt, drop(D.p_hidden, p.site + 5));
   }
   void conn_bwd(Run& V, const ConnLayerP& p, const ConnLayerA& a, const StepIn& x, size_t gv, size_t gt, size_t gxv, size_t gxt,
-                bool dxv = true, bool dxt = true) {
+                bool dxv = true, bool dxt = true, bool tail_v = false, bool tail_t = false) {
     const CrctModelDims& D = e->d;
     hipEvent_t free_v = V.set_free[V.parity], free_t = set_free[parity];
     const StreamScratch& sv = V.layer_begin(); const StreamScratch& st = layer_begin();
     const int B = b->B, Mv = B * b->V, Mt = B * b->T, Hb = D.Hb, d = Hb / D.b_heads;
-    V.ffn_bwd(p.ffn_v, a.ffn_v, a.proj_v.out(p.proj_v.ln), gv, sv.gc, sv, Mv, drop(D.p_v_hidden, p.site + 4));
-    ffn_bwd(p.ffn_t, a.ffn_t, a.proj_t.out(p.proj_t.ln), gt, st.gc, st, Mt, drop(D.p_hidden, p.site + 5));
+    const int pv = V.tail_pitch(tail_v, b->V), pt = tail_pitch(tail_t, b->T);
+    const int Mbv = pv > 1 ? B : Mv, Mbt = pt > 1 ? B : Mt;
+    V.ffn_bwd(p.ffn_v, a.ffn_v, a.proj_v.out(p.proj_v.ln), gv, sv.gc, sv, Mbv, drop(D.p_v_hidden, p.site + 4), pv);
+    ffn_bwd(p.ffn_t, a.ffn_t, a.proj_t.out(p.proj_t.ln), gt, st.gc, st, Mbt, drop(D.p_hidden, p.site + 5), pt);
     const bool aq = attn_q_ok(b->T, b->V, d) && attn_q_ok(b->V, b->T, d);
     const bool gq = aq && f8b_lin(p.qkv1) && f8b_lin(p.qkv2) && f8_lin(p.qkv1) && f8_lin(p.qkv2);
     const GradQ dqkvq_v{sv.dqkvq, gq ? a.g_dqkv1 : -1}, dqkvq_t{st.dqkvq, gq ? a.g_dqkv2 : -1};
-    V.proj_bwd(p.proj_v, a.proj_v, V.ctx_act(a.ctx2, a.ctx2q, a.site_ctx2, p.proj_v.dense, aq), sv.gc, sv, Mv, drop(D.p_v_hidden, p.site + 2));
-    proj_bwd(p.proj_t, a.proj_t, ctx_act(a.ctx1, a.ctx1q, a.site_ctx1, p.proj_t.dense, aq), st.gc, st, Mt, drop(D.p_hidden, p.site + 3));
+    V.proj_bwd(p.proj_v, a.proj_v, V.ctx_act(a.ctx2, a.ctx2q, a.site_ctx2, p.proj_v.dense, aq), sv.gc, sv, Mbv, drop(D.p_v_hidden, p.site + 2), pv);
+    proj_bwd(p.proj_t, a.proj_t, ctx_act(a.ctx1, a.ctx1q, a.site_ctx1, p.proj_t.dense, aq), st.gc, st, Mbt, drop(D.p_hidden, p.site + 3), pt);
     if (sw != s && V.sw != V.s) {
       if (free_v && !rc && hipStreamWaitEvent(s, free_v, 0) != hipSuccess) { crct_set_error("engine: stream wait failed"); rc = 1; }
       if (free_t && !V.rc && hipStreamWaitEvent(V.s, free_t, 0) != hipSuccess) { crct_set_error("engine: stream wait failed"); V.rc = 1; }
@@ -872,6 +918,7 @@
     V.lin_dgrad(V.A(e->ha.d_pv), D.Hb, e->v_pool, B, V.A(gv), ldv, Opt());
     if (!has_regressor()) {
       output_grads(V, gt, gv);
+      mark_tail();
       flush_wgrads();
       V.flush_wgrads();
       return;
@@ -891,8 +938,13 @@
     V.pipe_bwd(e->vp, V.A(seq_v), ldv, e->ha.v, V.A(g[3]), 512, V.A(gv), ldv, true, B, g + 4);
     pipe_bwd(e->tp, A(seq_t), ldt, e->ha.t, A(g[3]) + 256, 512, A(gt), ldt, true, B, g + 7);
     output_grads(V, gt, gv);
+    mark_tail();
     flush_wgrads();
     V.flush_wgrads();
+  }
+  void mark_tail() {
+    e->tail_t = e->sparse_tail && !e->og.d_seq_t;
+    e->tail_v = e->sparse_tail && !e->og.d_seq_v;
   }
   void output_grads(Run& V, size_t gt, size_t gv) {
     const SegPlan& pl = e->plan[0];
@@ -1448,6 +1500,7 @@
     if (!pl.runs) {
     } else if (sgi == 0) {
       e->cur_t = 0; e->cur_v = 0;
+      e->tail_t = e->tail_v = false;
       Rt.heads_bwd(Rv, e->in.back().t.x, e->in.back().v.x, e->st.dy[0], e->sv.dy[0], logits, reg, stats);
     } else if (sgi == nseg - 1) {
       if (pl.dx_t && e->emb_own_t) Rt.embed_text_bwd(e->st.dy[e->cur_t]);
@@ -1458,11 +1511,12 @@
       const Step& st = e->sched[si];
       const StepIn& x = e->in[si];
       const size_t gt = e->st.dy[e->cur_t], gxt = e->st.dy[e->cur_t ^ 1], gv = e->sv.dy[e->cur_v], gxv = e->sv.dy[e->cur_v ^ 1];
-      if (st.kind == 't') Rt.self_bwd(e->tl[st.idx], e->tla[st.idx], x.t, gt, gxt, batch->text_keymask, batch->B, batch->T, pl.dx_t);
-      else if (st.kind == 'v') Rv.self_bwd(e->vl[st.idx], e->vla[st.idx], x.v, gv, gxv, batch->image_keymask, batch->B, batch->V, pl.dx_v);
-      else Rt.conn_bwd(Rv, e->cl[st.idx], e->cla[st.idx], x, gv, gt, gxv, gxt, pl.dx_v, pl.dx_t);
-      if (st.kind != 'v') e->cur_t ^= 1;
-      if (st.kind != 't') e->cur_v ^= 1;
+      const bool tail_t = st.kind != 'v' && e->tail_t, tail_v = st.kind != 't' && e->tail_v;
+      if (st.kind == 't') Rt.self_bwd(e->tl[st.idx], e->tla[st.idx], x.t, gt, gxt, batch->text_keymask, batch->B, batch->T, pl.dx_t, tail_t);
+      else if (st.kind == 'v') Rv.self_bwd(e->vl[st.idx], e->vla[st.idx], x.v, gv, gxv, batch->image_keymask, batch->B, batch->V, pl.dx_v, tail_v);
+      else Rt.conn_bwd(Rv, e->cl[st.idx], e->cla[st.idx], x, gv, gt, gxv, gxt, pl.dx_v, pl.dx_t, tail_v, tail_t);
+      if (st.kind != 'v') { e->cur_t ^= 1; e->tail_t = false; }
+      if (st.kind != 't') { e->cur_v ^= 1; e->tail_v = false; }
     }
     if (seg < 0 && cfg->seg_done_events && !Rt.rc && !Rv.rc) {
       Rt.flush_wgrads();
@@ -1575,6 +1629,12 @@
   if (!e) return 1;
   e->ln_addend = on != 0;
   e->ws_update();
+  return 0;
+}
+
+extern "C" int crct_engine_set_sparse_tail(crct_engine_t* e, int on) {
+  if (!e) return 1;
+  e->sparse_tail = on != 0;
   return 0;
 }
 
diff --git a/cqa-crct_amd/csrc/rowops.hip b/cqa-crct_amd/csrc/rowops.hip
--- a/cqa-crct_amd/csrc/rowops.hip
+++ b/cqa-crct_amd/csrc/rowops.hip
@@ -593,6 +593,7 @@
   float* partials; int M, H; uint32_t post_thr; float post_scale; uint32_t post_site; uint32_t lin_thr; float lin_scale;
   uint32_t lin_site; uint64_t seed;
   uint8_t* q_out; const float* q_scale; float* q_amax;
+  int pitch;
 };
 template <int NCH, bool COMBINE, bool X32>
 __device__ __forceinline__ void ln_bwd_body(const LnBwdP& a, const int blk, const int nblk) {
@@ -610,16 +611,18 @@
   const float qs = a.q_out ? a.q_scale[0] : 0.f;
   float q_amax = 0.f;
   const long stride = (long)nblk * ROWS_PER_BLOCK;
+  const long pitch = a.pitch;
   long row = (long)blk * ROWS_PER_BLOCK + wave;
   RawRow<NCH> dy_n;
   typename std::conditional<X32, RawRowF<NCH>, RawRow<NCH>>::type x_n;
   const float* __restrict__ x32_p = reinterpret_cast<const float*>(a.x);
   float mean_n = 0.f, rstd_n = 0.f;
   if (row < M) {
-    row_fetch_bf16(dy_n, dy_p + row * H, H, lane);
-    if constexpr (X32) row_fetch_f32(x_n, x32_p + row * H, H, lane);
-    else row_fetch_bf16(x_n, x_p + row * H, H, lane);
-    mean_n = mean_p[row]; rstd_n = rstd_p[row];
+    const long pr = row * pitch;
+    row_fetch_bf16(dy_n, dy_p + pr * H, H, lane);
+    if constexpr (X32) row_fetch_f32(x_n, x32_p + pr * H, H, lane);
+    else row_fetch_bf16(x_n, x_p + pr * H, H, lane);
+    mean_n = mean_p[pr]; rstd_n = rstd_p[pr];
   }
   for (; row < M; row += stride) {
     Row<NCH> dy, x;
@@ -627,20 +630,22 @@
     row_unpack_bf16(dy, dy_n, H, lane);
     if constexpr (X32) row_unpack_f32(x, x_n, H, lane);
     else row_unpack_bf16(x, x_n, H, lane);
+    const long pr = row * pitch;
     if (row + stride < M) {
-      row_fetch_bf16(dy_n, dy_p + (row + stride) * H, H, lane);
-      if constexpr (X32) row_fetch_f32(x_n, x32_p + (row + stride) * H, H, lane);
-      else row_fetch_bf16(x_n, x_p + (row + stride) * H, H, lane);
-      mean_n = mean_p[row + stride]; rstd_n = rstd_p[row + stride];
-    }
-    row_apply_dropmask(dy, H, lane, row, post_thr, post_scale, post_site, seed);
+      const long pn = (row + stride) * pitch;
+      row_fetch_bf16(dy_n, dy_p + pn * H, H, lane);
+      if constexpr (X32) row_fetch_f32(x_n, x32_p + pn * H, H, lane);
+      else row_fetch_bf16(x_n, x_p + pn * H, H, lane);
+      mean_n = mean_p[pn]; rstd_n = rstd_p[pn];
+    }
+    row_apply_dropmask(dy, H, lane, pr, post_thr, post_scale, post_site, seed);
     row_ln_bwd(dy, x, g, H, lane, mean, rstd, adg, adb);
-    row_store_bf16(dy, dx_p + row * H, H, lane);
+    row_store_bf16(dy, dx_p + pr * H, H, lane);
     if (dxl_p) {
-      row_apply_dropmask(dy, H, lane, row, lin_thr, lin_scale, lin_site, seed);
-      row_store_bf16(dy, dxl_p + row * H, H, lane);
-    }
-    if (a.q_out) q_amax = amax_join(q_amax, row_store_bf8(dy, a.q_out + row * H, H, lane, qs));
+      row_apply_dropmask(dy, H, lane, pr, lin_thr, lin_scale, lin_site, seed);
+      row_store_bf16(dy, dxl_p + pr * H, H, lane);
+    }
+    if (a.q_out) q_amax = amax_join(q_amax, row_store_bf8(dy, a.q_out + pr * H, H, lane, qs));
     row_acc(adl, dy);
   }
   if (a.q_out && a.q_amax) {
@@ -1337,16 +1342,17 @@
 static bool ln_bwd_combines(int H) {
   return (size_t)3 * ROWS_PER_BLOCK * H * 4 <= 64 * 1024;
 }
-static LnBwdP ln_bwd_problem(const CrctLnBwdArgs& a) {
+static LnBwdP ln_bwd_problem(const CrctLnBwdArgs& a, int pitch) {
   return LnBwdP{(const bf16_t*)a.dy, (const bf16_t*)a.x, a.mean, a.rstd, a.gamma, (bf16_t*)a.dx, (bf16_t*)a.dx_lin, a.partials,
                 a.M, a.H, a.post_thr, a.post_scale, a.post_site, a.lin_thr, a.lin_scale, a.lin_site, a.seed,
-                (uint8_t*)a.q_out, a.q_scale, a.q_amax};
-}
-static int ln_bwd_launch(const CrctLnBwdArgs& a, hipStream_t s) {
+                (uint8_t*)a.q_out, a.q_scale, a.q_amax, pitch};
+}
+static int ln_bwd_launch(const CrctLnBwdArgs& a, hipStream_t s, int pitch = 1) {
   CRCT_REQUIRE(a.H % 8 == 0 && a.H > 0, "layernorm_bwd: H=%d must be a positive multiple of 8", a.H);
+  CRCT_REQUIRE(pitch >= 1, "layernorm_bwd: row pitch %d must be at least 1", pitch);
   if (a.M <= 0) return 0;
   const int nb = crct_layernorm_bwd_blocks(a.M);
-  const LnBwdP p = ln_bwd_problem(a);
+  const LnBwdP p = ln_bwd_problem(a, pitch);
   if (a.x_f32) {
     if (ln_bwd_combines(a.H)) {
       DISPATCH_NCH(a.H, crct_launch((ln_bwd_kernel<NCH, true, true>), dim3(nb), dim3(256), (size_t)3 * ROWS_PER_BLOCK * a.H * 4, s, LN_BWD_HOT(p) p));
@@ -1372,6 +1378,10 @@
 int crct_layernorm_bwd_rows_args(const CrctLnBwdArgs* a, crct_stream_t stream) {
   CRCT_REQUIRE(a && (!a->q_out || a->q_scale), "layernorm_bwd_rows_args: bad arguments");
   return ln_bwd_launch(*a, (hipStream_t)stream);
+}
+extern "C++" int crct_layernorm_bwd_rows_pitch(const CrctLnBwdArgs* a, int pitch, hipStream_t stream) {
+  CRCT_REQUIRE(a && (!a->q_out || a->q_scale), "layernorm_bwd_rows_pitch: bad arguments");
+  return ln_bwd_launch(*a, stream, pitch);
 }
 int crct_layernorm_bwd_finalize(const float* partials, float* dgamma, float* dbeta, float* dbias_lin, int M, int H,
                                 int accumulate, crct_stream_t stream) {
diff --git a/include/crct_hip.h b/include/crct_hip.h
--- a/include/crct_hip.h
+++ b/include/crct_hip.h
@@ -422,6 +422,7 @@
 int crct_engine_streams(crct_engine_t*, crct_stream_t out[4]);
 int crct_engine_set_wgrad_flush(crct_engine_t* e, int mode);
 int crct_engine_set_ln_addend(crct_engine_t* e, int on);
+int crct_engine_set_sparse_tail(crct_engine_t* e, int on);
 int crct_engine_set_wgrad_workgroups(crct_engine_t* e, int target_wgs, int max_rows);
 int crct_engine_set_site_policy(crct_engine_t*, int site, int kind, int phase, int cfg, int split_k);
 int crct_engine_wgrad_owned(crct_engine_t*, int64_t* offsets, int64_t* numels, int cap);
```

Result: no change. 11430 QA-pairs/s (median of 6 runs) (+0.7%).
